# lawfuyang/ToyRenderer

Hardware: AMD Instinct MI355X
Metric: Gmeshlets/s culled (whole node), 100M meshlets (higher is better)
Workload: dtype f32

## Files before the change

### toyrenderer_amd/csrc/k_basepass_as.hip

```cpp
#include <algorithm>
#include <cstdlib>
#include <string>
#include <type_traits>

#if defined(TR_STAMPS) || defined(TR_COUNT_SLOW) || defined(TR_COUNT_PATHS)
__device__ unsigned long long g_stampSums[8];
#define g_pathCount (g_stampSums + 4)
#endif
#include <atomic>
#include <memory>
#include <mutex>
#include <unordered_map>

#include "cull_math.hip.h"
#include "instance_cache.hip.h"
#include "meshlet_exact.hip.h"
#include "trhip_internal.h"

using namespace interop;

namespace
{

constexpr uint32_t kBlock = 256;
constexpr uint32_t kWaves = kBlock / 64;
constexpr uint32_t kBatch = 64;
constexpr uint32_t kSteps = kBatch / 2;
#ifndef TR_RING_SLOTS
#define TR_RING_SLOTS 2
#endif
#ifndef TR_CULL_BATCH
#define TR_CULL_BATCH (TR_RING_SLOTS == 3 ? 30 : 32)
#endif
#ifndef TR_WINDOW_MAP
#define TR_WINDOW_MAP 0
#endif
#ifndef TR_EARLY_PREFETCH
#define TR_EARLY_PREFETCH 1
#endif
#ifndef TR_DEFER
#define TR_DEFER 1
#endif
constexpr uint32_t kCullBatch = TR_CULL_BATCH;
constexpr uint32_t kCullSteps = kCullBatch / 2;
constexpr uint32_t kRingSlots = TR_RING_SLOTS;
static_assert(kCullSteps % kRingSlots == 0 && kCullBatch <= 64, "a batch is a whole number of trips round the ring");
#ifndef TR_CULL_WAVES
#define TR_CULL_WAVES 4
#endif
constexpr uint32_t kCullWaves = TR_CULL_WAVES;
constexpr uint32_t kCullBlock = 64 * kCullWaves;
#ifndef TR_SHORT_PASS_ROUNDS
#define TR_SHORT_PASS_ROUNDS 2
#endif
constexpr uint32_t kShortPassRounds = TR_SHORT_PASS_ROUNDS;
constexpr uint32_t kSlotBytes = 1280;
constexpr uint32_t kDefWords = 5;
constexpr uint32_t kDefStage = 64;
#ifndef TR_DEF_PASS_AT
#define TR_DEF_PASS_AT 32
#endif
constexpr uint32_t kDefPassAt = TR_DEF_PASS_AT;
constexpr uint32_t kDefFromRecord = 0xFFFFFFFFu;
static_assert(kDefPassAt <= kDefStage, "deferred list sizes");

struct RecordInfo
{
    float wxy[8];
    float wz[4];
    float adjxy[6];
    float adjz[3];
    float maxScale;
    uint32_t first;
    uint32_t lastOff;
};
__device__ __forceinline__ uint32_t lastOffOf(uint32_t count) { return count ? 16u * count - 8u : 0u; }
__device__ __forceinline__ uint32_t countOf(uint32_t lastOff) { return (lastOff + 8u) >> 4; }
static_assert(sizeof(RecordInfo) == 96, "RecordInfo layout");

__device__ __forceinline__ cm::M43P worldOf(const RecordInfo& ri)
{
    return { { ri.wxy[0], ri.wxy[1] }, { ri.wxy[2], ri.wxy[3] }, { ri.wxy[4], ri.wxy[5] }, { ri.wxy[6], ri.wxy[7] },
             ri.wz[0], ri.wz[1], ri.wz[2], ri.wz[3] };
}
__device__ __forceinline__ cm::M33P adjugateOf(const RecordInfo& ri)
{
    return { { ri.adjxy[0], ri.adjxy[1] }, { ri.adjxy[2], ri.adjxy[3] }, { ri.adjxy[4], ri.adjxy[5] }, ri.adjz[0], ri.adjz[1], ri.adjz[2] };
}

__device__ __forceinline__ uint32_t listGroupCount(const MeshletCullArgs& a)
{
    return a.listGroups ? a.listGroups[0] : groupCount(a);
}

typedef float v4f __attribute__((ext_vector_type(4)));
template <bool AFTER_READS = false>
__device__ __forceinline__ void issueMeshletLoads(char* slotLds , const MeshletCullStream& stream, uint32_t firstIdx, uint32_t lastOff, uint32_t sub16 ,
                                                  v4f readA = v4f{ 0.f, 0.f, 0.f, 0.f }, uint32_t readB = 0u )
{
#ifdef TR_EXP_NOMEM
    firstIdx &= 63u;
#endif
    const uint32_t idx = firstIdx + (min(sub16, lastOff) >> 4);
    const char* pa = reinterpret_cast<const char*>(stream.sphere) + ((uint64_t)idx << 4);
    const char* pb = reinterpret_cast<const char*>(stream.cone) + ((uint64_t)idx << 2);
    const uint32_t ldsOff = (uint32_t)(uintptr_t)(__attribute__((address_space(3))) char*)slotLds;
#ifndef TR_DMA_POLICY_ID
#define TR_DMA_POLICY_ID 1
#endif
#if TR_DMA_POLICY_ID == 0
#define TR_DMA_POLICY ""
#elif TR_DMA_POLICY_ID == 1
#define TR_DMA_POLICY "nt"
#elif TR_DMA_POLICY_ID == 2
#define TR_DMA_POLICY "sc1"
#elif TR_DMA_POLICY_ID == 3
#define TR_DMA_POLICY "sc0 sc1"
#elif TR_DMA_POLICY_ID == 4
#define TR_DMA_POLICY "sc0 sc1 nt"
#elif TR_DMA_POLICY_ID == 5
#define TR_DMA_POLICY "sc0"
#else
#define TR_DMA_POLICY "sc1 nt"
#endif
    if (AFTER_READS)
        asm volatile("s_mov_b32 m0, %2\n\t"
                     "global_load_lds_dwordx4 %0, off " TR_DMA_POLICY "\n\t"
                     "s_add_u32 m0, %2, 0x400\n\t"
                     "global_load_lds_dword %1, off " TR_DMA_POLICY
                     :: "v"(pa), "v"(pb), "s"(ldsOff), "v"(readA), "v"(readB) : "memory", "m0", "scc");
    else
        asm volatile("s_mov_b32 m0, %2\n\t"
                     "global_load_lds_dwordx4 %0, off " TR_DMA_POLICY "\n\t"
                     "s_add_u32 m0, %2, 0x400\n\t"
                     "global_load_lds_dword %1, off " TR_DMA_POLICY
                     :: "v"(pa), "v"(pb), "s"(ldsOff) : "memory", "m0", "scc");
}
#define TR_WAIT_VMCNT(n) asm volatile("s_waitcnt vmcnt(" #n ")" ::: "memory")

#ifdef TR_STAMPS
#define TR_STAMP(i) do { unsigned long long _t = __builtin_amdgcn_s_memtime(); __builtin_amdgcn_s_waitcnt(0xC07F); stampSum[i] += _t - stampLast; stampLast = _t; } while (0)
#else
#define TR_STAMP(i) do {} while (0)
#endif

#ifndef TR_LK_POLICY_ID
#define TR_LK_POLICY_ID 0
#endif
#if TR_LK_POLICY_ID == 0
#define TR_LK_POLICY ""
#elif TR_LK_POLICY_ID == 1
#define TR_LK_POLICY " sc0"
#elif TR_LK_POLICY_ID == 2
#define TR_LK_POLICY " sc1"
#elif TR_LK_POLICY_ID == 3
#define TR_LK_POLICY " sc0 sc1"
#elif TR_LK_POLICY_ID == 4
#define TR_LK_POLICY " nt"
#else
#define TR_LK_POLICY " sc1 nt"
#endif
#ifndef TR_CULL_WAVES_PER_EU
#define TR_CULL_WAVES_PER_EU 5
#endif
template <bool FRUSTUM, bool OCCLUSION, bool CONE, bool TABLE>
__global__ __launch_bounds__(kCullBlock, TR_CULL_WAVES_PER_EU) void meshletCullKernel(MeshletCullArgs a)
{
#ifdef TR_STAMPS
    unsigned long long stampSum[8] = {0, 0, 0, 0, 0, 0, 0, 0};
    unsigned long long stampLast = __builtin_amdgcn_s_memtime();
    __builtin_amdgcn_s_waitcnt(0xC07F);
#endif
    __shared__ RecordInfo s_recAll[kCullWaves][kCullBatch + 2 * kRingSlots];
    __shared__ uint32_t s_gIdxAll[kCullWaves][kCullBatch];
    __shared__ uint32_t s_quadOff[16];
    __shared__ uint4 s_mipTab[17];
    __shared__ float s_coneTab[cm::kConeTabEntries];
    constexpr bool kDeferred = OCCLUSION && TABLE;
    __shared__ uint2 s_mipBand[kDeferred ? 17 : 1];
    __shared__ uint32_t s_defAll[kCullWaves][kDeferred ? kDefStage * kDefWords : 1u];
    __shared__ __attribute__((aligned(8))) uint32_t s_maskAll[kCullWaves][kCullBatch + 2];
    __shared__ __attribute__((aligned(16))) char s_ring[kCullWaves][kRingSlots][kSlotBytes];

    const uint32_t G = groupCount(a);
    const uint32_t tid = threadIdx.x, lane = tid & 63u, wave = tid >> 6;
    const uint32_t half = lane >> 5, sub = lane & 31u;
    if (a.listGroups && blockIdx.x == 0 && tid == 0) a.listGroups[0] = G;
    const cm::M43 V = cm::loadM43(a.k.m_WorldToView);
    const cm::M43P VP = cm::packM43(V);
    const cm::M33P VR = cm::rot(VP);
    const float coneSlack = cm::coneSlackFactor(V);
    if (!TABLE && G <= gridDim.x * (2u * kCullWaves) * a.shortPassRounds) {
        for (uint32_t g = (blockIdx.x * kCullWaves + wave) * 2u + half; g < G; g += gridDim.x * kCullWaves * 2u) {
            const bool vis = exactMeshletVisible<FRUSTUM, OCCLUSION, CONE>(a, VP, VR, g, sub);
            const unsigned long long b = __ballot(vis);
            if (sub == 0) a.visMask[g] = (uint32_t)(half ? b >> 32 : b);
        }
        return;
    }
    RecordInfo* s_rec = s_recAll[wave];
    uint32_t* s_gIdx = s_gIdxAll[wave];

    if (tid < 16) s_quadOff[tid] = a.hzb.mipOffset[tid];
    if (TABLE && tid >= 1 && tid <= 16) {
        const uint32_t mip = tid - 1u < a.hzb.mips ? tid - 1u : 0u;
        const uint32_t mw = (a.hzb.width >> mip) ? (a.hzb.width >> mip) : 1u, mh = (a.hzb.height >> mip) ? (a.hzb.height >> mip) : 1u;
        s_mipTab[tid] = make_uint4(a.quad.offset[mip], ((mw >> 3) + 1u) * 64u, __float_as_uint(0.5f * (float)mw), __float_as_uint(0.5f * (float)mh));
    }
    if (kDeferred && tid >= 1 && tid <= 16) { const uint32_t d = cm::projMipDelta(a.bands, tid); s_mipBand[tid] = make_uint2(d, 2u * d); }
    const bool nearInRange = a.k.m_NearPlane >= 0x1p-20f && a.k.m_NearPlane <= 0x1p20f;
    if (CONE) for (uint32_t i = tid; i < cm::kConeTabEntries; i += kCullBlock) s_coneTab[i] = cm::coneTableEntry(i);
    if (lane < 2 * kRingSlots) { s_recAll[wave][kCullBatch + lane].first = 0; s_recAll[wave][kCullBatch + lane].lastOff = 0; }
    uint32_t* s_def = s_defAll[wave];
    uint32_t* s_mask = s_maskAll[wave];
    __syncthreads();

    const bool usePerm = a.permHeader != nullptr && a.permHeader[0] == 1u && a.permHeader[1] == G;
#ifndef TR_TEAM_ALL
    const uint32_t teamWaves = kCullWaves, waveInTeam = wave, team = blockIdx.x, teams = gridDim.x;
#else
    const uint32_t teamWaves = gridDim.x * kCullWaves, waveInTeam = blockIdx.x * kCullWaves + wave, team = 0u, teams = 1u;
#endif
    const uint32_t superSize = teamWaves * kCullBatch;
    const uint32_t numSuper = (G + superSize - 1) / superSize;
    auto loadEntry = [&](uint32_t sb_) -> uint4 {
#ifdef TR_BLOCKED_MAP
        const uint64_t e64 = (uint64_t)sb_ * superSize + waveInTeam * kCullBatch + lane;
#else
        const uint64_t e64 = (uint64_t)sb_ * superSize + (lane >> 1) * 2 * teamWaves + 2 * waveInTeam + (lane & 1);
#endif
        if (lane >= kCullBatch || sb_ >= numSuper || e64 >= G) return make_uint4(0xFFFFFFFFu, 0u, 0u, 0u);
        const uint32_t e = (uint32_t)e64;
        if (usePerm) return a.perm[e];
        const MeshletAmplificationData rec = a.records[e];
        return make_uint4(e, rec.m_InstanceConstIdx, rec.m_MeshLOD, rec.m_MeshletGroupOffset);
    };
#ifndef TR_NO_SPLIT_TAIL
    const uint32_t fullRounds = numSuper / teams, left = numSuper - fullRounds * teams;
    uint32_t piecesPer = 1u, stepsPer = kCullSteps;
    if (left) {
        const uint32_t k = std::min(teams / left, kCullSteps / kRingSlots);
        if (k > 1u) {
            stepsPer = ((kCullSteps + k - 1u) / k + kRingSlots - 1u) / kRingSlots * kRingSlots;
            piecesPer = (kCullSteps + stepsPer - 1u) / stepsPer;
        }
    }
#else
    const uint32_t fullRounds = (numSuper + teams - 1u) / teams, left = 0u, piecesPer = 1u, stepsPer = kCullSteps;
#endif
    auto windowOf = [&](uint32_t it, uint32_t& s0, uint32_t& s1) -> uint32_t {
        s0 = 0u; s1 = kCullSteps;
        if (it < fullRounds) {
            uint64_t w = (uint64_t)it * teams + team;
#if TR_WINDOW_MAP
            constexpr uint32_t kCo = TR_CULL_WAVES_PER_EU;
            if (teams % kCo == 0u) {
                const uint32_t perRow = teams / kCo, c = team % perRow, j = team / perRow;
                w = TR_WINDOW_MAP == 2 ? ((uint64_t)c * fullRounds + it) * kCo + j : (uint64_t)it * teams + (uint64_t)c * kCo + j;
            }
#endif
            return w < numSuper ? (uint32_t)w : 0xFFFFFFFFu;
        }
        if (it == fullRounds && left && team < left * piecesPer) {
            s0 = (team % piecesPer) * stepsPer;
            s1 = std::min(s0 + stepsPer, kCullSteps);
            return fullRounds * teams + team / piecesPer;
// ... 276 lines not shown
            TR_STAMP(6);
        };
        if (!primed) {
#pragma unroll
            for (uint32_t k = 0; k + 1 < kRingSlots; ++k)
                issueMeshletLoads(ring + kSlotBytes * k, a.stream, s_rec[2 * (s0 + k) + half].first, s_rec[2 * (s0 + k) + half].lastOff, sub16);
            if (kDefer) {
                const void* p = TABLE ? (const void*)a.quad.base : (const void*)a.hzb.base;
                issueLookup(lk0[kRingSlots - 1u], lk1[kRingSlots - 1u], p, p, 0ull);
            }
            issueMeshletLoads(ring + kSlotBytes * (kRingSlots - 1u), a.stream, s_rec[2 * (s0 + kRingSlots - 1u) + half].first, s_rec[2 * (s0 + kRingSlots - 1u) + half].lastOff, sub16);
        }
#pragma unroll 1
        for (uint32_t s = s0; s < nSteps; s += kRingSlots) {
            step(std::integral_constant<uint32_t, 0>{}, s);
            step(std::integral_constant<uint32_t, 1>{}, s + 1);
            if (kRingSlots == 3) step(std::integral_constant<uint32_t, 2>{}, s + 2);
        }
        if (kDefer) {
            if (kEarly) asm volatile("s_waitcnt vmcnt(0)" : "+v"(lk0[kRingSlots - 1u]), "+v"(lk1[kRingSlots - 1u]) :: "memory");
            else asm volatile("s_waitcnt vmcnt(2)" : "+v"(lk0[kRingSlots - 1u]), "+v"(lk1[kRingSlots - 1u]) :: "memory");
            resolve(2u * nSteps, pVis, pAccept, pPair, pDepth, lk0[kRingSlots - 1u], lk1[kRingSlots - 1u]);
        }
        if (!kPipe) TR_WAIT_VMCNT(0);
        __builtin_amdgcn_fence(__ATOMIC_ACQ_REL, "wavefront");
        __builtin_amdgcn_wave_barrier();
        if (kDeferred && __builtin_expect(batchExact, 0)) {
            for (uint32_t s = s0; s < nSteps; ++s) {
                const uint32_t r = 2 * s + half;
                const uint32_t g = s_gIdx[r];
                const unsigned long long ballot = __ballot(g < G && exactMeshlet(g, sub));
                if (sub == 0) s_mask[r + 2u] = half ? (uint32_t)(ballot >> 32) : (uint32_t)ballot;
            }
            stCount = stAtBatch;
            batchExact = false;
#ifdef TR_COUNT_PATHS
            if (lane == 0) atomicAdd(&g_stampSums[2], 1ull);
#endif
            asm volatile("s_waitcnt vmcnt(0)" ::: "memory");
            __builtin_amdgcn_fence(__ATOMIC_ACQ_REL, "wavefront");
            __builtin_amdgcn_wave_barrier();
        }
        if (kDeferred && __builtin_expect(stAtBatch >= kDefPassAt, 0)) {
            const uint32_t n = stAtBatch < 64u ? stAtBatch : 64u;
            runPass(n);
            stAtBatch -= n;
        }
        {
            const uint32_t g = lane < kCullBatch ? s_gIdx[lane] : 0xFFFFFFFFu;
            if (g < G) a.visMask[g] = s_mask[(lane < kCullBatch ? lane : 0u) + 2u];
        }
        primed = false;
        const uint32_t nStepsN = stepsOf(sbN, s0N, s1N);
        if (nStepsN) {
            const float4* wr = blockAddr(entry);
            q0 = wr[0]; q1 = wr[1]; q2 = wr[2]; q3 = wr[3];
            if (kPipe && usePerm) {
                const bool has = entry.x < G && (lane >> 1) >= s0N && (lane >> 1) < nStepsN;
                uint32_t cnt = entry.w < 32u ? entry.w : 32u;
                if (!has || (uint64_t)entry.z + cnt > a.numMeshlets) cnt = 0u;
                const uint32_t pf = cnt ? entry.z : 0u, pl = lastOffOf(cnt);
#pragma unroll
                for (uint32_t k = 0; k < kRingSlots; ++k) {
                    const int from = (int)((2u * (s0N + k) + half) * 4u);
                    const uint32_t f = (uint32_t)__builtin_amdgcn_ds_bpermute(from, (int)pf), l = (uint32_t)__builtin_amdgcn_ds_bpermute(from, (int)pl);
                    issueMeshletLoads(ring + kSlotBytes * k, a.stream, f, l, sub16);
                }
                primed = true;
            }
        } else if (kPipe) {
            TR_WAIT_VMCNT(0);
        }
    }
    if (kDeferred && stCount) {
        asm volatile("s_waitcnt vmcnt(0)" ::: "memory");
        while (stCount) runPass(stCount < 64u ? stCount : 64u);
    }
#ifdef TR_STAMPS
    if (lane == 0)
        for (int i = 0; i < 8; ++i) atomicAdd(&g_stampSums[i], stampSum[i]);
#endif
}

__device__ __forceinline__ uint32_t waveSum(uint32_t v)
{
    v += (uint32_t)__builtin_amdgcn_update_dpp(0, (int)v, 0x111, 0xf, 0xf, true);
    v += (uint32_t)__builtin_amdgcn_update_dpp(0, (int)v, 0x112, 0xf, 0xf, true);
    v += (uint32_t)__builtin_amdgcn_update_dpp(0, (int)v, 0x114, 0xf, 0xf, true);
    v += (uint32_t)__builtin_amdgcn_update_dpp(0, (int)v, 0x118, 0xf, 0xf, true);
    v += (uint32_t)__builtin_amdgcn_update_dpp(0, (int)v, 0x142, 0xa, 0xf, false);
    v += (uint32_t)__builtin_amdgcn_update_dpp(0, (int)v, 0x143, 0xc, 0xf, false);
    return (uint32_t)__builtin_amdgcn_readlane((int)v, 63);
}

#ifndef TR_SUPER_SHIFT
#define TR_SUPER_SHIFT 8
#endif
constexpr uint32_t kSuperShift = TR_SUPER_SHIFT;
constexpr uint32_t kSuperBatches = 1u << kSuperShift;
constexpr uint32_t kCountThreads = 1024;
constexpr uint32_t kCountWaves = kCountThreads / 64;
__global__ __launch_bounds__(kCountThreads) void visCountKernel(MeshletCullArgs a)
{
    __shared__ uint32_t s_part[kCountWaves];
    const uint32_t G = listGroupCount(a);
    const uint32_t numBatches = (G + kBatch - 1) / kBatch;
    const uint32_t numSupers = (numBatches + kSuperBatches - 1) >> kSuperShift;
    const uint32_t lane = threadIdx.x & 63u, wave = threadIdx.x >> 6;
    constexpr uint32_t kPerWave = kSuperBatches / kCountWaves;
    for (uint32_t sb = blockIdx.x; sb < numSupers; sb += gridDim.x) {
        const uint32_t b0 = (sb << kSuperShift) + wave * kPerWave;
        uint32_t pc[kPerWave];
#pragma unroll
        for (uint32_t i = 0; i < kPerWave; ++i) {
            const uint32_t g = (b0 + i) * kBatch + lane;
            pc[i] = g < G ? (uint32_t)__popc(a.visMask[g]) : 0u;
        }
        uint32_t mine = 0;
#pragma unroll
        for (uint32_t i = 0; i < kPerWave; ++i) {
            pc[i] = waveSum(pc[i]);
            if (lane == 0 && b0 + i < numBatches) a.batchSum[b0 + i] = pc[i];
            mine += pc[i];
        }
        __syncthreads();
        if (lane == 0) s_part[wave] = mine;
        __syncthreads();
        if (threadIdx.x == 0) {
            uint32_t total = 0;
#pragma unroll
            for (uint32_t w = 0; w < kCountWaves; ++w) total += s_part[w];
            a.superSum[sb] = total;
        }
    }
}

__device__ __forceinline__ uint32_t waveInclusiveScan(uint32_t v, uint32_t lane)
{
#pragma unroll
    for (int d = 1; d < 64; d <<= 1) {
        uint32_t n = __shfl_up(v, d);
        if (lane >= (uint32_t)d) v += n;
    }
    return v;
}

__global__ __launch_bounds__(1024) void visSuperScanKernel(MeshletCullArgs a)
{
    __shared__ uint32_t s_wave[16];
    const uint32_t G = listGroupCount(a);
    const uint32_t numBatches = (G + kBatch - 1) / kBatch;
    const uint32_t numSupers = (numBatches + kSuperBatches - 1) >> kSuperShift;
    const uint32_t tid = threadIdx.x, lane = tid & 63u, wave = tid >> 6;
    uint32_t carry = 0;
    for (uint32_t base = 0; base < numSupers; base += 1024u) {
        const uint32_t i = base + tid;
        const uint32_t v = i < numSupers ? a.superSum[i] : 0u;
        const uint32_t inc = waveInclusiveScan(v, lane);
        __syncthreads();
        if (lane == 63) s_wave[wave] = inc;
        __syncthreads();
        uint32_t pre = 0, all = 0;
#pragma unroll
        for (uint32_t w = 0; w < 16; ++w) { if (w < wave) pre += s_wave[w]; all += s_wave[w]; }
        if (i < numSupers) a.superSum[i] = carry + pre + inc - v;
        carry += all;
    }
    if (tid == 0) { a.drawArgs[0] = carry; a.drawArgs[1] = 1; a.drawArgs[2] = 1; }
}

__global__ __launch_bounds__(kBlock) void visExpandKernel(MeshletCullArgs a)
{
    __shared__ uint2 s_mo[kWaves][kBatch];
    const uint32_t G = listGroupCount(a);
    const uint32_t numBatches = (G + kBatch - 1) / kBatch;
    const uint32_t lane = threadIdx.x & 63u, wave = threadIdx.x >> 6;
    const uint32_t half = lane >> 5, sub = lane & 31u;
    const uint32_t bit = 1u << sub, below = bit - 1u;
    uint2* mo = s_mo[wave];
    for (uint32_t batch = blockIdx.x * kWaves + wave; batch < numBatches; batch += gridDim.x * kWaves) {
        const uint32_t g0 = batch * kBatch;
        const uint32_t mask = g0 + lane < G ? a.visMask[g0 + lane] : 0u;
        const uint32_t sb = batch >> kSuperShift;
        uint32_t before = 0;
        for (uint32_t j = (sb << kSuperShift) + lane; j < batch; j += 64u) before += a.batchSum[j];
        before = waveSum(before) + a.superSum[sb];
        const uint32_t pc = (uint32_t)__popc(mask);
        const uint32_t exc = waveInclusiveScan(pc, lane) - pc + before;
        mo[lane] = make_uint2(mask, exc);
        __builtin_amdgcn_fence(__ATOMIC_RELEASE, "wavefront");
        __builtin_amdgcn_wave_barrier();
        __builtin_amdgcn_fence(__ATOMIC_ACQUIRE, "wavefront");
        uint32_t value = ((g0 + half) << 5) | sub;
#pragma unroll 8
        for (uint32_t s = 0; s < kSteps; ++s) {
            const uint2 e = mo[2 * s + half];
            if (e.x & bit) {
                const uint32_t pos = e.y + (uint32_t)__popc(e.x & below);
                if (pos < a.listCapacity) a.visibleList[pos] = value;
            }
            value += 2u << 5;
        }
        __builtin_amdgcn_fence(__ATOMIC_RELEASE, "wavefront");
        __builtin_amdgcn_wave_barrier();
        __builtin_amdgcn_fence(__ATOMIC_ACQUIRE, "wavefront");
    }
}

constexpr uint32_t kCompactTile = 2048;
constexpr uint32_t kCompactThreads = 1024;
constexpr uint32_t kCompactWaves = kCompactThreads / 64;
constexpr uint32_t kCompactMaxTiles = (1u << 19) / kCompactTile;
constexpr uint32_t kStatusStride = 16;
constexpr uint64_t kFlagA = 1ull << 62, kFlagMask = 3ull << 62, kPoison = 1ull << 48;

__global__ __launch_bounds__(kCompactThreads) void visCompactKernel(MeshletCullArgs a, unsigned long long* status, uint32_t* ticket)
{
    __shared__ uint32_t s_mask[kCompactTile];
    __shared__ uint32_t s_off[kCompactTile];
    __shared__ uint32_t s_waveTot[kCompactWaves];
    __shared__ uint32_t s_tile;
    __shared__ unsigned long long s_pre[kCompactMaxTiles / 64u];
    const uint32_t G = listGroupCount(a);
    const uint32_t numTiles = (G + kCompactTile - 1) / kCompactTile;
    const uint32_t tid = threadIdx.x, lane = tid & 63u, wave = tid >> 6;
    for (;;) {
        if (tid == 0) s_tile = atomicAdd(ticket, 1u);
        __syncthreads();
        const uint32_t tile = s_tile;
        if (tile >= numTiles) {
            if (tile == 0 && tid == 0) { a.drawArgs[0] = 0; a.drawArgs[1] = 1; a.drawArgs[2] = 1; }
            return;
        }
        const uint32_t g0 = tile * kCompactTile;
        const uint32_t b = g0 + tid * 2u;
        uint32_t m0 = 0, m1 = 0;
        if (b + 2u <= G) { const uint2 v = *reinterpret_cast<const uint2*>(a.visMask + b); m0 = v.x; m1 = v.y; }
        else if (b < G) m0 = a.visMask[b];
        const uint32_t c0 = (uint32_t)__popc(m0), mine = c0 + (uint32_t)__popc(m1);
        const uint32_t inc = waveInclusiveScan(mine, lane);
        if (lane == 63) s_waveTot[wave] = inc;
        __syncthreads();
        uint32_t pre = 0, total = 0;
#pragma unroll
        for (uint32_t w = 0; w < kCompactWaves; ++w) { const uint32_t x = s_waveTot[w]; if (w < wave) pre += x; total += x; }
        const uint32_t exc = pre + inc - mine;
        *reinterpret_cast<uint2*>(&s_mask[tid * 2u]) = make_uint2(m0, m1);
        *reinterpret_cast<uint2*>(&s_off[tid * 2u]) = make_uint2(exc, exc + c0);
        if (tid == 0) __hip_atomic_store(&status[tile * kStatusStride], kFlagA | (unsigned long long)total, __ATOMIC_RELAXED, __HIP_MEMORY_SCOPE_AGENT);
        if (wave < kCompactMaxTiles / 64u) {
            unsigned long long v = 0;
            if (tid < tile) {
                uint32_t spins = 0;
                for (;;) {
                    v = __hip_atomic_load(&status[tid * kStatusStride], __ATOMIC_RELAXED, __HIP_MEMORY_SCOPE_AGENT);
                    if (v & kFlagMask) { v &= ~kFlagMask; break; }
                    if (++spins > (1u << 22)) { v = kPoison; break; }
                    __builtin_amdgcn_s_sleep(1);
                }
            }
#pragma unroll
            for (int d = 32; d >= 1; d >>= 1) v += __shfl_xor(v, d);
            if (lane == 0) s_pre[wave] = v;
        }
        __syncthreads();
        unsigned long long base = 0;
#pragma unroll
        for (uint32_t w = 0; w < kCompactMaxTiles / 64u; ++w) base += s_pre[w];
        if (tid == 0 && tile == numTiles - 1) {
            const unsigned long long all = base + total;
            const bool bad = (all >> 40) != 0ull;
            a.drawArgs[0] = bad ? 0xFFFFFFFFu : (uint32_t)all;
            a.drawArgs[1] = bad ? 0xFFFFFFFFu : 1u;
            a.drawArgs[2] = bad ? 0xFFFFFFFFu : 1u;
        }
        const uint32_t groupsHere = G - g0 < kCompactTile ? G - g0 : kCompactTile;
#pragma unroll 4
        for (uint32_t slot = tid; slot < groupsHere * 32u; slot += kCompactThreads) {
            const uint32_t g = slot >> 5, sub = slot & 31u;
            const uint32_t mask = s_mask[g];
            if (mask & (1u << sub)) {
                const unsigned long long pos = base + s_off[g] + (uint32_t)__popc(mask & ((1u << sub) - 1u));
                if (pos < a.listCapacity) a.visibleList[pos] = ((g0 + g) << 5) | sub;
            }
        }
        __syncthreads();
    }
}

// ... 212 lines not shown
                if (inSlot > a.slotGroups || inSlot < sentG || runEnd < runBegin || runEnd > a.slotRuns) bad = true;
                if (bad) { status |= 4u; g = 0; runEnd = runBegin; }
                if (a.globalCap && a.records[s] && !bad) {
                    const unsigned long long x = a.recv[(uint64_t)p * slotWords + 2u * s + 1u];
                    if (cutDone[s]) g = 0;
                    else if (counted[s] + x >= a.globalCap) {
                        cutDone[s] = true;
                        const unsigned long long j = a.globalCap - counted[s] - 1ull;
                        if (j < g) {
                            const uint32_t* run = a.recv + (uint64_t)p * slotWords + kSlotHeaderWords + 4ull * runBegin;
                            uint32_t lo = 0, hi = runEnd - runBegin;
                            while (hi - lo > 1u) {
                                const uint32_t mid = (lo + hi) >> 1;
                                if (run[4ull * mid + 3u] <= j) lo = mid; else hi = mid;
                            }
                            g = hi > lo ? run[4ull * lo + 3u] : 0u;
                        }
                    }
                    counted[s] += x;
                }
                uint32_t runs = a.records[s] ? runEnd - runBegin : 0u;
                if (off[s] + g > a.capacity[s]) { g = a.capacity[s] - off[s]; status |= 2u; }
                const uint32_t base = p * slotWords + kSlotHeaderWords;
                s_maskStart[k] = maskRun; s_runStart[k] = runRun;
                s_maskSrc[k] = base + 4u * a.slotRuns + srcG; s_runSrc[k] = base + 4u * runBegin;
                s_dst[k] = off[s]; s_len[k] = g;
                maskRun += g; runRun += runs; ++k;
                off[s] += g;
                runBegin = runEnd;
            }
        }
        s_maskStart[k] = maskRun; s_runStart[k] = runRun;
        if (blockIdx.x == 0)
            for (uint32_t s = 0; s < kMaxPassSlots; ++s)
                if (a.args[s]) {
                    const unsigned long long X = a.globalCap ? counted[s] : off[s];
                    a.args[s][0] = X > 0xFFFFFFFFull ? 0xFFFFFFFFu : (uint32_t)X; a.args[s][1] = 1; a.args[s][2] = 1; a.args[s][3] = off[s];
                    a.args[s][7] = status;
                }
    }
    __syncthreads();
    const uint32_t numSeg = kMaxPassSlots * a.world;
    const uint32_t totalMasks = s_maskStart[numSeg];
    for (uint32_t i = blockIdx.x * 256u + tid; i < totalMasks; i += gridDim.x * 256u) {
        uint32_t lo = 0, hi = numSeg;
        while (hi - lo > 1u) {
            const uint32_t mid = (lo + hi) >> 1;
            if (s_maskStart[mid] <= i) lo = mid; else hi = mid;
        }
        a.masks[lo % kMaxPassSlots][s_dst[lo] + (i - s_maskStart[lo])] = a.recv[(uint64_t)s_maskSrc[lo] + (i - s_maskStart[lo])];
    }
    const uint32_t totalRuns = s_runStart[numSeg];
    for (uint32_t it = blockIdx.x * 256u + (tid & ~63u); it < totalRuns; it += gridDim.x * 256u) {
        const uint32_t i = it + lane;
        uint32_t id = 0, lod = 0, off0 = 0, first = 0, cnt = 0;
        uint32_t* dst = nullptr;
        if (i < totalRuns) {
            uint32_t lo = 0, hi = numSeg;
            while (hi - lo > 1u) {
                const uint32_t mid = (lo + hi) >> 1;
                if (s_runStart[mid] <= i) lo = mid; else hi = mid;
            }
            const uint32_t e = i - s_runStart[lo], runs = s_runStart[lo + 1] - s_runStart[lo], len = s_len[lo];
            const uint4 entry = *reinterpret_cast<const uint4*>(a.recv + (uint64_t)s_runSrc[lo] + 4ull * e);
            uint32_t next = e + 1u < runs ? a.recv[(uint64_t)s_runSrc[lo] + 4ull * (e + 1u) + 3u] : 0xFFFFFFFFu;
            next = next < len ? next : len;
            id = entry.x; lod = entry.y; off0 = entry.z; first = entry.w;
            cnt = first < next ? next - first : 0u;
            dst = a.records[lo % kMaxPassSlots] + 3ull * (s_dst[lo] + first);
        }
        if (cnt <= 8u)
            for (uint32_t j = 0; j < cnt; ++j) { dst[3u * j] = id; dst[3u * j + 1u] = lod; dst[3u * j + 2u] = off0 + 32u * j; }
        unsigned long long big = __ballot(cnt > 8u);
        while (big) {
            const int l = __builtin_ctzll(big);
            big &= big - 1ull;
            const uint32_t bid = __shfl(id, l), blod = __shfl(lod, l), boff = __shfl(off0, l), bcnt = __shfl(cnt, l);
            uint32_t* bdst = (uint32_t*)(((unsigned long long)__shfl((uint32_t)((unsigned long long)dst >> 32), l) << 32) | __shfl((uint32_t)(unsigned long long)dst, l));
            for (uint32_t j = lane; j < bcnt; j += 64u) { bdst[3u * j] = bid; bdst[3u * j + 1u] = blod; bdst[3u * j + 2u] = boff + 32u * j; }
        }
    }
}

void emitListBuild(const trhip::DispatchCtx& ctx, const MeshletCullArgs& a, const char* prefix, bool side, const void* argsBase)
{
    auto emit = [&](const std::string& name, std::function<int(hipStream_t)> fn) {
        if (side) ctx.emitSide(name.c_str(), std::move(fn), { { a.listGroups ? (const void*)a.listGroups : argsBase, false }, { a.visMask, false }, { a.visibleList, true }, { a.drawArgs, true } });
        else ctx.emit(name.c_str(), std::move(fn));
    };
    if (!side && a.recordCapacity <= kCompactMaxTiles * kCompactTile) {
        const uint32_t tiles = (a.recordCapacity + kCompactTile - 1) / kCompactTile;
        const size_t words = (size_t)kCompactMaxTiles * kStatusStride * 2 + 4;
        uint32_t* mem = (uint32_t*)ctx.scratch(words * 4);
        if (mem && ctx.cl->recordClearWords(mem, words, 0, true) == TRHIP_OK) {
            unsigned long long* status = (unsigned long long*)mem;
            uint32_t* ticket = mem + kCompactMaxTiles * kStatusStride * 2;
            uint32_t grid = ctx.computeUnits();
            if (grid > tiles) grid = tiles;
            if (grid == 0) grid = 1;
            emit(std::string(prefix) + "compact", [a, status, ticket, grid](hipStream_t s) {
                TRHIP_LAUNCH(visCompactKernel, dim3(grid), dim3(kCompactThreads), 0, s, a, status, ticket);
                return trhip::launchStatus("visCompactKernel"); });
            return;
        }
    }
    const uint32_t needBlocks = (a.maxBatches + kWaves - 1) / kWaves;
    uint32_t gridSmall = ctx.computeUnits() * 8u;
    if (gridSmall > needBlocks) gridSmall = needBlocks;
    if (gridSmall == 0) gridSmall = 1;
    const std::string p = prefix;
    const uint32_t supers = (a.maxBatches >> kSuperShift) + 1u;
    emit(p + "count", [a, supers](hipStream_t s) {
        TRHIP_LAUNCH(visCountKernel, dim3(supers), dim3(kCountThreads), 0, s, a);
        return trhip::launchStatus("visCountKernel"); });
    emit(p + "scan", [a](hipStream_t s) {
        TRHIP_LAUNCH(visSuperScanKernel, dim3(1), dim3(1024), 0, s, a);
        return trhip::launchStatus("visSuperScanKernel"); });
    emit(p + "expand", [a, gridSmall](hipStream_t s) {
        TRHIP_LAUNCH(visExpandKernel, dim3(gridSmall), dim3(kBlock), 0, s, a);
        return trhip::launchStatus("visExpandKernel"); });
}

template <bool F, bool O, bool C>
void launchCull(const MeshletCullArgs& a, uint32_t grid, bool table, hipStream_t s)
{
    if (O && table) TRHIP_LAUNCH((meshletCullKernel<F, O, C, true>), dim3(grid), dim3(kCullBlock), 0, s, a);
    else TRHIP_LAUNCH((meshletCullKernel<F, O, C, false>), dim3(grid), dim3(kCullBlock), 0, s, a);
}

constexpr uint64_t kStreamBytesPerMeshlet = 20;
__host__ __device__ inline MeshletCullStream meshletStreamLayout(void* mem, uint64_t numMeshlets)
{
    const uint64_t coneAt = (numMeshlets * 16u + 255u) & ~255ull;
    return { reinterpret_cast<const float4*>(mem), reinterpret_cast<const uint32_t*>(reinterpret_cast<char*>(mem) + coneAt) };
}
inline uint64_t meshletStreamBytes(uint64_t numMeshlets) { return ((numMeshlets * 16u + 255u) & ~255ull) + numMeshlets * 4u; }

__global__ __launch_bounds__(256) void meshletStreamKernel(const MeshletData* __restrict__ meshlets, uint64_t n, MeshletCullStream out)
{
    const uint64_t stride = (uint64_t)gridDim.x * 256u;
    for (uint64_t i = (uint64_t)blockIdx.x * 256u + threadIdx.x; i < n; i += stride) {
        const float4* p = reinterpret_cast<const float4*>(meshlets + i);
        const float4 sphere = p[0];
        const uint32_t cone = __float_as_uint(p[1].x);
        const_cast<float4*>(out.sphere)[i] = sphere;
        const_cast<uint32_t*>(out.cone)[i] = cone;
    }
}

int meshletStreamLaunchBuild(trhip_buffer_t* meshlets, hipStream_t s)
{
    const trhip::Stamp from = { meshlets->version };
    if (meshlets->cullStream.current(from)) return TRHIP_OK;
    const uint64_t n = meshlets->byteSize / sizeof(MeshletData);
    const uint64_t blocks = (n + 255u) / 256u;
    TRHIP_LAUNCH(meshletStreamKernel, dim3((uint32_t)(blocks < 65536u ? (blocks ? blocks : 1u) : 65536u)), dim3(256), 0, s,
                       (const MeshletData*)meshlets->ptr, n, meshletStreamLayout(meshlets->cullStream.ptr, n));
    meshlets->cullStream.markBuilt(from);
    return trhip::launchStatus("meshletStreamKernel");
}

int recordASMain(trhip::DispatchCtx& ctx)
{
    const BasePassConstants* k = (const BasePassConstants*)ctx.constants(0, sizeof(BasePassConstants));
    TRHIP_REQUIRE(k, "%s: constant buffer b0 (BasePassConstants, 256 bytes) missing", ctx.shaderName);
    trhip_buffer_t* instances = ctx.buffer(TRHIP_BIND_STRUCTURED_SRV, 0);
    trhip_buffer_t* meshData = ctx.buffer(TRHIP_BIND_STRUCTURED_SRV, 2);
    trhip_buffer_t* meshlets = ctx.buffer(TRHIP_BIND_STRUCTURED_SRV, 4);
    trhip_buffer_t* records = ctx.buffer(TRHIP_BIND_STRUCTURED_SRV, 7);
    trhip_texture_t* hzb = ctx.texture(TRHIP_BIND_TEXTURE_SRV, 8);
    trhip_buffer_t* visMask = ctx.buffer(TRHIP_BIND_STRUCTURED_UAV, 0);
    trhip_buffer_t* visList = ctx.buffer(TRHIP_BIND_STRUCTURED_UAV, 1);
    trhip_buffer_t* drawArgs = ctx.buffer(TRHIP_BIND_STRUCTURED_UAV, 2);
    TRHIP_REQUIRE(instances && meshData && meshlets && records, "%s: needs SRVs t0, t2, t4, t7 (BasePassRenderers.cpp:463-479)", ctx.shaderName);
    TRHIP_REQUIRE(visMask && visList && drawArgs, "%s: needs UAVs u0 (visMask), u1 (visibleList), u2 (drawArgs)", ctx.shaderName);
    TRHIP_REQUIRE(ctx.indirect, "%s: launched by dispatchMeshIndirect (BasePassRenderers.cpp:497-502): use dispatch_indirect", ctx.shaderName);
    TRHIP_REQUIRE(instances->byteSize % sizeof(BasePassInstanceConstants) == 0, "%s: instance buffer size is not a multiple of 144", ctx.shaderName);
    TRHIP_REQUIRE(meshlets->byteSize % sizeof(MeshletData) == 0, "%s: meshlet buffer size is not a multiple of 32", ctx.shaderName);
    TRHIP_REQUIRE(drawArgs->byteSize >= 12, "%s: drawArgs buffer smaller than 12 bytes", ctx.shaderName);

    MeshletCullArgs a;
    memset(&a, 0, sizeof a);
    a.k = *k;
    const bool occlusion = (k->m_CullingFlags & kCullingFlagOcclusionCullingEnable) != 0;
    const bool useTable = occlusion && ctx.variant == 0 && records->byteSize / sizeof(MeshletAmplificationData) >= trhip::tableMinGroups();
    int rc = TRHIP_OK;
    {
        memset(&a.hzb, 0, sizeof a.hzb);
        if (occlusion) {
            TRHIP_REQUIRE(hzb, "%s: occlusion culling enabled but no HZB texture bound at t8", ctx.shaderName);
            TRHIP_REQUIRE(hzb->format == TRHIP_FORMAT_R16_FLOAT, "%s: HZB is not R16_FLOAT", ctx.shaderName);
            TRHIP_REQUIRE(hzb->width == k->m_HZBDimensions.x && hzb->height == k->m_HZBDimensions.y,
                          "%s: m_HZBDimensions %ux%u does not match the HZB texture %ux%u", ctx.shaderName,
                          k->m_HZBDimensions.x, k->m_HZBDimensions.y, hzb->width, hzb->height);
            a.hzb.base = (const _Float16*)hzb->ptr;
            a.hzb.width = hzb->width; a.hzb.height = hzb->height; a.hzb.mips = hzb->mips;
            for (uint32_t m = 0; m < hzb->mips; ++m) a.hzb.mipOffset[m] = (uint32_t)(hzb->mipOffset[m] / 2);
            if (useTable) {
                rc = trhip::hzbQuadEnsure(hzb);
                if (rc != TRHIP_OK) return rc;
                a.quad.base = (const _Float16*)hzb->quad.ptr;
                a.quad.total = hzb->quadTotal;
                for (uint32_t m = 0; m < hzb->mips; ++m) a.quad.offset[m] = hzb->quadOffset[m];
            }
        }
    }
    if (rc != TRHIP_OK) return rc;
    a.meshlets = (const MeshletData*)meshlets->ptr;
    TRHIP_REQUIRE(meshlets->byteSize >= sizeof(MeshletData), "%s: empty meshlet buffer", ctx.shaderName);
    rc = meshlets->cullStream.allocate(meshlets->dev, meshletStreamBytes(meshlets->byteSize / sizeof(MeshletData)));
    if (rc != TRHIP_OK) return rc;
    a.stream = meshletStreamLayout(meshlets->cullStream.ptr, meshlets->byteSize / sizeof(MeshletData));
    a.records = (const MeshletAmplificationData*)records->ptr;
    a.dispatchArgs = (const uint32_t*)((const char*)ctx.argsBuffer->ptr + ctx.argsOffset);
    a.argsWords = (ctx.argsBuffer->byteSize - ctx.argsOffset) >= 16 ? 4u : 3u;
    const uint64_t cap = records->byteSize / sizeof(MeshletAmplificationData);
    a.recordCapacity = cap > 0xFFFFFFFFull ? 0xFFFFFFFFu : (uint32_t)cap;
    TRHIP_REQUIRE(a.recordCapacity <= (1u << 27), "%s: more than 2^27 records cannot be encoded as (g<<5)|lane", ctx.shaderName);
    TRHIP_REQUIRE(visMask->byteSize / 4 >= a.recordCapacity, "%s: visMask holds %llu groups, records buffer %u", ctx.shaderName,
                  (unsigned long long)(visMask->byteSize / 4), a.recordCapacity);
    a.numMeshlets = meshlets->byteSize / sizeof(MeshletData);
    TRHIP_REQUIRE(a.numMeshlets <= (1ull << 32), "%s: more than 2^32 meshlets (m_MeshletDataBufferIdx is 32 bits wide)", ctx.shaderName);
    a.visMask = (uint32_t*)visMask->ptr;
    a.visibleList = (uint32_t*)visList->ptr;
    const uint64_t lcap = visList->byteSize / 4;
    a.listCapacity = lcap > 0xFFFFFFFFull ? 0xFFFFFFFFu : (uint32_t)lcap;
    a.drawArgs = (uint32_t*)drawArgs->ptr;
    if (records->order.ptr && records->order.bytes >= 256 + (uint64_t)a.recordCapacity * 16) {
        a.permHeader = (const uint32_t*)records->order.ptr;
        a.perm = (const uint4*)(a.permHeader + 64);
    }
    rc = trhip::instanceCacheEnsure(instances);
    if (rc != TRHIP_OK) return rc;
    a.numInstances = (uint32_t)(instances->byteSize / sizeof(BasePassInstanceConstants));
    a.cache = instanceCacheLayout(instances->cullCache.ptr, a.numInstances);
    a.maxBatches = (a.recordCapacity + kBatch - 1) / kBatch;
    a.batchSum = (uint32_t*)(a.recordCapacity >= (1u << 19) ? ctx.scratchSide((size_t)a.maxBatches * 4)
                                                            : ctx.scratch((size_t)a.maxBatches * 4));
    TRHIP_REQUIRE(a.batchSum, "%s: scratch allocation failed", ctx.shaderName);
    {
        const size_t supers = (a.maxBatches >> kSuperShift) + 1u;
        a.superSum = (uint32_t*)(a.recordCapacity >= (1u << 19) ? ctx.scratchSide(supers * 4) : ctx.scratch(supers * 4));
        TRHIP_REQUIRE(a.superSum, "%s: scratch allocation failed", ctx.shaderName);
    }

    const uint32_t blocksPerCU = TR_CULL_WAVES_PER_EU;
    uint32_t grid = ctx.computeUnits() * blocksPerCU;
    const uint32_t needBlocks = (a.recordCapacity + kCullBatch * kCullWaves - 1) / (kCullBatch * kCullWaves);
    if (grid > needBlocks) grid = needBlocks;
    if (grid == 0) grid = 1;
    rc = visMask->listCount.allocate(visMask->dev, 256);
    if (rc != TRHIP_OK) return rc;
    a.listGroups = (uint32_t*)visMask->listCount.ptr;
    ctx.cl->use(a.listGroups, ctx.cl->ops.size(), true);
    if (useTable) a.bands = cm::projBands(k->m_P00, k->m_P11, hzb->width, hzb->height);
    static const bool noShortPass = getenv("TRHIP_NO_SHORT_PASS") != nullptr;
    a.shortPassRounds = noShortPass ? 0u : kShortPassRounds;
    const uint32_t flags = k->m_CullingFlags & 7u;
    trhip_texture_t* quadOwner = useTable ? hzb : nullptr;
    const bool table = useTable;
    if (quadOwner) ctx.cl->use(quadOwner->quad.ptr, ctx.cl->ops.size(), false);
    ctx.emit("cull", [a, grid, flags, quadOwner, table, instances, meshData, meshlets](hipStream_t s) {
        if ((const void*)a.meshlets != meshlets->ptr)
            return trhip::fail(TRHIP_ERR_STATE, "basepass_AS_Main: the meshlet buffer was bound to other memory after this command list was recorded: record it again");
        {
            int crc = trhip::instanceCacheLaunchBuild(instances, meshData, s);
            if (crc != TRHIP_OK) return crc;
            crc = meshletStreamLaunchBuild(meshlets, s);
            if (crc != TRHIP_OK) return crc;
        }
        if (quadOwner) {
            int brc = trhip::hzbQuadLaunchBuild(quadOwner, s);
            if (brc != TRHIP_OK) return brc;
        }
        switch (flags) {
        case 0: launchCull<false, false, false>(a, grid, table, s); break;
        case 1: launchCull<true, false, false>(a, grid, table, s); break;
        case 2: launchCull<false, true, false>(a, grid, table, s); break;
        case 3: launchCull<true, true, false>(a, grid, table, s); break;
        case 4: launchCull<false, false, true>(a, grid, table, s); break;
        case 5: launchCull<true, false, true>(a, grid, table, s); break;
        case 6: launchCull<false, true, true>(a, grid, table, s); break;
        default: launchCull<true, true, true>(a, grid, table, s); break;
        }
        return trhip::launchStatus("meshletCullKernel"); });
    emitListBuild(ctx, a, "", a.recordCapacity >= (1u << 19), ctx.argsBuffer->ptr);
    if (ctx.cl->openStats)
        return trhip::statsEmitAS(ctx, a, meshlets, records, instances, meshData, a.recordCapacity >= (1u << 19));
    return TRHIP_OK;
}

int recordPackShard(trhip::DispatchCtx& ctx)
{
    const uint32_t* push = (const uint32_t*)ctx.constants(0, 8);
    trhip_buffer_t* slot = ctx.buffer(TRHIP_BIND_STRUCTURED_UAV, 0);
    trhip_buffer_t* state = ctx.buffer(TRHIP_BIND_STRUCTURED_UAV, 1);
    TRHIP_REQUIRE(push && slot && state, "%s: needs push constants {slotGroups, slotRuns}, UAV u0 (shard slot) and UAV u1 (state words, zeroed once)", ctx.shaderName);
    ShardPackArgs a;
    memset(&a, 0, sizeof a);
    a.slotGroups = push[0];
    a.slotRuns = push[1];
    const uint64_t slotWords = (uint64_t)kSlotHeaderWords + 4ull * a.slotRuns + a.slotGroups;
    TRHIP_REQUIRE(slot->byteSize >= slotWords * 4, "%s: shard slot buffer smaller than 16 + 4 * %u + %u words", ctx.shaderName, a.slotRuns, a.slotGroups);
    const uint64_t maxTiles = (uint64_t)a.slotGroups / kPackTile + kMaxPassSlots + 1u;
    TRHIP_REQUIRE(maxTiles < (1u << 30) && state->byteSize >= maxTiles * 16u, "%s: state buffer u1 smaller than %llu bytes", ctx.shaderName, (unsigned long long)(maxTiles * 16u));
    TRHIP_REQUIRE(((uintptr_t)slot->ptr & 15u) == 0 && ((uintptr_t)state->ptr & 7u) == 0, "%s: u0 / u1 not 16 / 8-byte aligned", ctx.shaderName);
    a.slot = (uint32_t*)slot->ptr;
    a.maxTiles = (uint32_t)maxTiles;
    unsigned long long* halves = (unsigned long long*)state->ptr;
    for (uint32_t s = 0; s < kMaxPassSlots; ++s) {
        trhip_buffer_t* rec = ctx.buffer(TRHIP_BIND_STRUCTURED_SRV, 4 * s);
        trhip_buffer_t* mask = ctx.buffer(TRHIP_BIND_STRUCTURED_SRV, 4 * s + 1);
        trhip_buffer_t* args = ctx.buffer(TRHIP_BIND_STRUCTURED_SRV, 4 * s + 2);
        trhip_buffer_t* draw = ctx.buffer(TRHIP_BIND_STRUCTURED_SRV, 4 * s + 3);
        if (!rec && !mask && !args && !draw) continue;
        TRHIP_REQUIRE(rec && mask && args && draw, "%s: pass slot %u needs t%u..t%u (records, visMask, dispatch args, draw args)", ctx.shaderName, s, 4 * s, 4 * s + 3);
        TRHIP_REQUIRE(args->byteSize >= 12 && draw->byteSize >= 12, "%s: argument buffers smaller than 12 bytes", ctx.shaderName);
        const uint64_t cap = std::min<uint64_t>(rec->byteSize / sizeof(MeshletAmplificationData), mask->byteSize / 4);
        a.records[s] = (const uint32_t*)rec->ptr;
        a.masks[s] = (const uint32_t*)mask->ptr;
        a.dispatchArgs[s] = (const uint32_t*)args->ptr;
        a.drawArgs[s] = (const uint32_t*)draw->ptr;
        a.argsWords[s] = args->byteSize >= 16 ? 4u : 3u;
        a.recordCapacity[s] = cap > 0xFFFFFFFFull ? 0xFFFFFFFFu : (uint32_t)cap;
    }
    a.tileBlocks = (uint32_t)std::min<uint64_t>(maxTiles, (uint64_t)ctx.computeUnits() * 3u);
    const uint32_t maskBlocks = (uint32_t)std::min<uint64_t>(std::max<uint64_t>(((uint64_t)a.slotGroups + 4u * kPackThreads - 1u) / (4u * kPackThreads), 1u), ctx.computeUnits());
    const uint32_t grid = a.tileBlocks + maskBlocks;
    static std::mutex mu;
    static std::unordered_map<void*, std::shared_ptr<std::atomic<uint32_t>>> launches;
    std::shared_ptr<std::atomic<uint32_t>> count;
    {
        std::lock_guard<std::mutex> lock(mu);
        std::shared_ptr<std::atomic<uint32_t>>& c = launches[(void*)halves];
        if (!c) c = std::make_shared<std::atomic<uint32_t>>(0u);
        count = c;
    }
    ctx.emit("main", [a, grid, halves, count](hipStream_t s) {
        ShardPackArgs l = a;
        const uint32_t half = count->fetch_add(1u) & 1u;
        l.status = halves + (size_t)half * a.maxTiles;
        l.statusNext = halves + (size_t)(half ^ 1u) * a.maxTiles;
        TRHIP_LAUNCH(shardPackKernel, dim3(grid), dim3(kPackThreads), 0, s, l);
        return trhip::launchStatus("shardPackKernel"); });
    return TRHIP_OK;
}

int recordUnpackShards(trhip::DispatchCtx& ctx)
{
    const uint32_t* push = (const uint32_t*)ctx.constants(0, 12);
    trhip_buffer_t* recv = ctx.buffer(TRHIP_BIND_STRUCTURED_SRV, 0);
    TRHIP_REQUIRE(push && recv, "%s: needs push constants {world, slotGroups, slotRuns[, globalGroupCapacity]} and SRV t0 (gathered slots)", ctx.shaderName);
    ShardUnpackArgs a;
    memset(&a, 0, sizeof a);
    a.world = push[0];
    a.slotGroups = push[1];
    a.slotRuns = push[2];
    if (const uint32_t* push4 = (const uint32_t*)ctx.constants(0, 16)) a.globalCap = push4[3];
    TRHIP_REQUIRE(a.world >= 1 && a.world <= kMaxRanks, "%s: world size %u outside [1, %u]", ctx.shaderName, a.world, kMaxRanks);
    const uint64_t words = (uint64_t)a.world * (kSlotHeaderWords + 4ull * a.slotRuns + a.slotGroups);
    TRHIP_REQUIRE(words < (1ull << 32), "%s: %u slots of %u groups / %u runs exceed 2^32 words", ctx.shaderName, a.world, a.slotGroups, a.slotRuns);
    TRHIP_REQUIRE(recv->byteSize >= words * 4, "%s: gathered buffer smaller than world x slot", ctx.shaderName);
    TRHIP_REQUIRE(((uintptr_t)recv->ptr & 15u) == 0, "%s: t0 not 16-byte aligned", ctx.shaderName);
    a.recv = (const uint32_t*)recv->ptr;
    MeshletCullArgs lists[kMaxPassSlots];
    uint64_t copyWords = 0;
    for (uint32_t s = 0; s < kMaxPassSlots; ++s) {
        trhip_buffer_t* rec = ctx.buffer(TRHIP_BIND_STRUCTURED_UAV, 4 * s);
        trhip_buffer_t* mask = ctx.buffer(TRHIP_BIND_STRUCTURED_UAV, 4 * s + 1);
// ... 64 lines not shown
```

### toyrenderer_amd/csrc/k_gpuculling.hip

```cpp
#include "cull_math.hip.h"
#include "hzb_quad.hip.h"
#include "instance_cache.hip.h"
#include "trhip_internal.h"

using namespace interop;

namespace
{

constexpr uint32_t kBlock = 256;
constexpr uint32_t kWordSubmit = 1u << 30;
constexpr uint32_t kWordLate = 1u << 31;
constexpr uint32_t kGroupMask = (1u << 27) - 1u;

struct InstanceCullArgs
{
    GPUCullingPassConstants k;
    const BasePassInstanceConstants* instances;
    const uint32_t* ids;
    const MeshData* meshData;
    cm::Hzb hzb;
    MeshletAmplificationData* records;
    uint32_t* dispatchArgs;
    uint32_t* lateCount;
    uint32_t* lateIds;
    const uint32_t* indirectArgs;
    InstanceCullCache cache;
    uint32_t numInstances;
    const uint32_t* shardLate;
    uint32_t directThreads;
    uint32_t maxGroups;
    uint32_t argsWords;
    uint32_t* word;
    uint32_t* localOff;
    uint32_t* blockGroups;
    uint64_t* blockLateSubmit;
    uint32_t* bases;
    uint32_t numBlocks;
    uint32_t* tileHist;
    uint32_t* tileTotal;
    uint16_t* tileOf;
    uint2* lodSel;
    uint32_t* permHeader;
    uint4* perm;
    uint32_t permCapacity;
    uint32_t* lateArgsOut;
    unsigned long long* fusedStatus;
    uint32_t* fusedTicket;
};

struct QuadShare { bool stale = false; };
struct EarlyCullNote { InstanceCullArgs a; size_t scanOp; bool fused; trhip_texture_t* quadOwner = nullptr; std::shared_ptr<QuadShare> share; };

__global__ __launch_bounds__(256) void instanceCacheKernel(const BasePassInstanceConstants* instances, uint32_t n,
                                                           const MeshData* meshData, uint32_t numMeshes, InstanceCullCache c)
{
    const uint32_t i = blockIdx.x * 256u + threadIdx.x;
    if (i >= n) return;
    const BasePassInstanceConstants& inst = instances[i];
    const float4 w0 = *reinterpret_cast<const float4*>(inst.m_WorldMatrix.m[0]);
    const float4 w1 = *reinterpret_cast<const float4*>(inst.m_WorldMatrix.m[1]);
    const float4 w2 = *reinterpret_cast<const float4*>(inst.m_WorldMatrix.m[2]);
    const float4 w3 = *reinterpret_cast<const float4*>(inst.m_WorldMatrix.m[3]);
    const uint32_t meshIdx = inst.m_MeshDataIdx;
    float4 sph = make_float4(0.f, 0.f, 0.f, 0.f);
    uint32_t numLODs = 0;
    uint32_t nm[kMaxNumMeshLODs], mb[kMaxNumMeshLODs];
    float err[kMaxNumMeshLODs];
#pragma unroll
    for (uint32_t l = 0; l < kMaxNumMeshLODs; ++l) { nm[l] = 0; mb[l] = 0; err[l] = 0.f; }
    if (meshIdx < numMeshes) {
        const MeshData& mesh = meshData[meshIdx];
        sph = *reinterpret_cast<const float4*>(&mesh.m_BoundingSphere);
        numLODs = mesh.m_NumLODs;
#pragma unroll
        for (uint32_t l = 0; l < kMaxNumMeshLODs; ++l) {
            nm[l] = mesh.m_MeshLODDatas[l].m_NumMeshlets; mb[l] = mesh.m_MeshLODDatas[l].m_MeshletDataBufferIdx; err[l] = mesh.m_MeshLODDatas[l].m_Error;
        }
    }
    instanceCacheWriteTransformPart(c, i, w0, w1, w2, w3, sph);
    const_cast<float4*>(c.localSphere)[i] = sph;
    const_cast<uint32_t*>(c.numLODs)[i] = numLODs;
#pragma unroll
    for (uint32_t l = 0; l < kMaxNumMeshLODs; ++l) {
        const_cast<uint2&>(c.lod(i, l)) = make_uint2(nm[l], mb[l]);
// ... 308 lines not shown
    const uint32_t tid = threadIdx.x, lane = tid & 63u, wave = tid >> 6;
    const bool binned = n >= kMinBinnedEntries;
    if (binned) {
        uint32_t carry = 0;
        for (uint32_t base = 0; base < kNumTiles; base += kBigThreads) {
            const bool inRange = base + tid < kNumTiles;
            const uint32_t tot = inRange ? a.tileTotal[base + tid] : 0u;
            const uint32_t inc = waveInclusiveScan(tot, lane);
            if (lane == 63) s_wave[wave] = inc;
            __syncthreads();
            uint32_t pre = 0, all = 0;
            for (uint32_t w = 0; w < kBigWaves; ++w) { if (w < wave) pre += s_wave[w]; all += s_wave[w]; }
            if (inRange) s_cursor[base + tid] = carry + pre + inc - tot + a.tileHist[(uint64_t)blockIdx.x * kNumTiles + base + tid];
            carry += all;
            __syncthreads();
        }
    }
    const uint32_t baseG = a.bases[0] + a.blockGroups[blockIdx.x];
    const uint32_t baseL = a.bases[1] + (uint32_t)a.blockLateSubmit[blockIdx.x];
    for (uint32_t e = 0; e < kBigPerThread; ++e) {
        const uint32_t t = blockIdx.x * kBigChunk + e * kBigThreads + tid;
        const uint32_t word = t < n ? a.word[t] : 0u;
        if (word & kWordLate) a.lateIds[baseL + a.localOff[t]] = a.ids[t];
        const bool submit = (word & kWordSubmit) != 0 && !(word & kWordLate);
        const uint32_t groups = word & kGroupMask;
        const uint32_t lod = (word >> 27) & 7u;
        const uint32_t off = submit ? baseG + a.localOff[t] : 0u;
        const bool dropped = submit && off + groups >= a.maxGroups;
        if (dropped && groups != 0 && off < a.maxGroups && a.argsWords > 3) a.dispatchArgs[3] = off;
        const bool emitRec = submit && !dropped;
        const uint32_t id = emitRec ? a.ids[t] : 0u;
        if (emitRec) {
            struct __attribute__((packed, aligned(4))) Quad { uint32_t x, y, z, w; };
            uint32_t* dst = reinterpret_cast<uint32_t*>(a.records + off);
            uint32_t i = 0;
            for (; i + 4u <= groups; i += 4u) {
                const uint32_t o = i * kNumThreadsPerWave;
                *reinterpret_cast<Quad*>(dst + 3u * i) = Quad{ id, lod, o, id };
                *reinterpret_cast<Quad*>(dst + 3u * i + 4u) = Quad{ lod, o + kNumThreadsPerWave, id, lod };
                *reinterpret_cast<Quad*>(dst + 3u * i + 8u) = Quad{ o + 2u * kNumThreadsPerWave, id, lod, o + 3u * kNumThreadsPerWave };
            }
            for (; i < groups; ++i) {
                MeshletAmplificationData rec = { id, lod, i * kNumThreadsPerWave };
                a.records[off + i] = rec;
            }
        }
        const bool place = emitRec && groups != 0 && binned;
        uint32_t p = 0, numMeshlets = 0, mbase = 0;
        if (place) {
            p = atomicAdd(&s_cursor[a.tileOf[t]], groups);
            const uint2 li = a.lodSel[t];
            numMeshlets = li.x; mbase = li.y;
        }
        const uint32_t head = place ? (groups < 4u ? groups : 4u) : 0u;
        const uint32_t j = lane & 3u;
#pragma unroll
        for (uint32_t it = 0; it < 4; ++it) {
            const int src = (int)(it * 16u + (lane >> 2));
            const uint32_t sp = __shfl(p, src), soff = __shfl(off, src), sid = __shfl(id, src);
            const uint32_t sbase = __shfl(mbase, src), snm = __shfl(numMeshlets, src), shead = __shfl(head, src);
            if (j < shead) {
                const uint32_t first = j * kNumThreadsPerWave;
                const uint32_t cnt = snm > first ? (snm - first < kNumThreadsPerWave ? snm - first : kNumThreadsPerWave) : 0u;
                if (sp + j < a.permCapacity) a.perm[sp + j] = make_uint4(soff + j, sid, sbase + first, cnt);
            }
        }
        if (place)
            for (uint32_t i = 4; i < groups; ++i) {
                const uint32_t first = i * kNumThreadsPerWave;
                const uint32_t cnt = numMeshlets > first ? (numMeshlets - first < kNumThreadsPerWave ? numMeshlets - first : kNumThreadsPerWave) : 0u;
                if (p + i < a.permCapacity) a.perm[p + i] = make_uint4(off + i, id, mbase + first, cnt);
            }
    }
}


constexpr uint32_t kFusedMaxEntries = 1u << 17;
constexpr uint32_t kFusedMaxTiles = kFusedMaxEntries / kBlock;
constexpr uint32_t kFusedLateMaxTiles = 4096;
constexpr uint32_t kFusedStatusStride = 16;
constexpr unsigned long long kFusedFlag = 1ull << 63, kFusedPoison = 1ull << 60;

template <int LATE>
__global__ __launch_bounds__(kBlock) void instanceFusedKernel(InstanceCullArgs a, trhip::QuadArgs q)
{
    if (!LATE && blockIdx.x >= a.numBlocks) {
        __shared__ float s_t[9][trhip::kQuadStripCols + 1];
        trhip::hzbQuadStrip(q, blockIdx.x - a.numBlocks, s_t);
        return;
    }
    __shared__ uint32_t s_waveG[kBlock / 64], s_waveL[kBlock / 64], s_waveS[kBlock / 64];
    __shared__ unsigned long long s_preG[kBlock / 64], s_preLS[kBlock / 64];
    __shared__ uint32_t s_tile;
    const uint32_t n = threadCount<LATE>(a);
    const uint32_t numTiles = (n + kBlock - 1) / kBlock < a.numBlocks ? (n + kBlock - 1) / kBlock : a.numBlocks;
    const uint32_t tid = threadIdx.x, lane = tid & 63u, wave = tid >> 6;
    const uint32_t baseX = __hip_atomic_load(&a.dispatchArgs[0], __ATOMIC_RELAXED, __HIP_MEMORY_SCOPE_AGENT);
    const uint32_t baseLate = LATE ? 0u : __hip_atomic_load(a.lateCount, __ATOMIC_RELAXED, __HIP_MEMORY_SCOPE_AGENT);
    if (blockIdx.x >= (numTiles ? numTiles : 1u)) return;
    {
        if (tid == 0) s_tile = atomicAdd(a.fusedTicket, 1u);
        __syncthreads();
        const uint32_t tile = s_tile;
        const uint32_t t = tile * kBlock + tid;
        uint32_t word = 0, tileUnused = 0;
        uint2 lodUnused;
        if (t < n) word = classify<LATE>(a, a.ids[t], &tileUnused, &lodUnused);
        const uint32_t g = (word & kWordSubmit) ? (word & kGroupMask) : 0u;
        const uint32_t late = word >> 31;
        const uint32_t submit = (word >> 30) & 1u;
        const uint32_t incG = waveInclusiveScan(g, lane);
        const uint32_t incL = waveInclusiveScan(late, lane);
        const uint32_t cntS = (uint32_t)__popcll(__ballot(submit != 0));
        if (lane == 63) { s_waveG[wave] = incG; s_waveL[wave] = incL; s_waveS[wave] = cntS; }
        __syncthreads();
        uint32_t baseG = 0, baseL = 0, totG = 0, totL = 0, totS = 0;
#pragma unroll
        for (uint32_t w = 0; w < kBlock / 64; ++w) {
            if (w < wave) { baseG += s_waveG[w]; baseL += s_waveL[w]; }
            totG += s_waveG[w]; totL += s_waveL[w]; totS += s_waveS[w];
        }
        const uint32_t localOff = late ? (baseL + incL - late) : (baseG + incG - g);
        unsigned long long* line = a.fusedStatus + (uint64_t)tile * kFusedStatusStride;
        if (tid == 0 && numTiles != 0) {
            __hip_atomic_store(&line[0], kFusedFlag | (unsigned long long)totG, __ATOMIC_RELAXED, __HIP_MEMORY_SCOPE_AGENT);
            __hip_atomic_store(&line[1], kFusedFlag | ((unsigned long long)totS << 32) | (unsigned long long)totL, __ATOMIC_RELAXED, __HIP_MEMORY_SCOPE_AGENT);
        }
        unsigned long long sumG = 0, sumLS = 0;
        for (uint32_t j = tid; j < tile; j += kBlock) {
            const unsigned long long* pl = a.fusedStatus + (uint64_t)j * kFusedStatusStride;
            unsigned long long v0 = 0, v1 = 0;
            uint32_t spins = 0;
            for (;;) {
                v0 = __hip_atomic_load(&pl[0], __ATOMIC_RELAXED, __HIP_MEMORY_SCOPE_AGENT);
                v1 = __hip_atomic_load(&pl[1], __ATOMIC_RELAXED, __HIP_MEMORY_SCOPE_AGENT);
                if ((v0 & v1 & kFusedFlag) != 0ull) { v0 &= ~kFusedFlag; v1 &= ~kFusedFlag; break; }
                if (++spins > (1u << 22)) { v0 = kFusedPoison; v1 = 0; break; }
                __builtin_amdgcn_s_sleep(1);
            }
            sumG += v0; sumLS += v1;
        }
#pragma unroll
        for (int d = 32; d >= 1; d >>= 1) { sumG += __shfl_xor(sumG, d); sumLS += __shfl_xor(sumLS, d); }
        if (lane == 0) { s_preG[wave] = sumG; s_preLS[wave] = sumLS; }
        __syncthreads();
        unsigned long long preG = 0, preLS = 0;
#pragma unroll
        for (uint32_t w = 0; w < kBlock / 64; ++w) { preG += s_preG[w]; preLS += s_preLS[w]; }
        const uint32_t prefixG = (uint32_t)preG, prefixL = (uint32_t)preLS;
        if (t < n) {
            if (word & kWordLate) {
                a.lateIds[baseLate + prefixL + localOff] = a.ids[t];
            } else if (word & kWordSubmit) {
                const uint32_t groups = word & kGroupMask;
                const uint32_t lod = (word >> 27) & 7u;
                const uint32_t off = baseX + prefixG + localOff;
                if (off + groups >= a.maxGroups) {
                    if (groups != 0 && off < a.maxGroups && a.argsWords > 3) a.dispatchArgs[3] = off;
                } else {
                    const uint32_t id = a.ids[t];
                    for (uint32_t i = 0; i < groups; ++i) {
                        MeshletAmplificationData rec = { id, lod, i * kNumThreadsPerWave };
                        a.records[off + i] = rec;
                    }
                }
            }
        }
        if (tid == 0 && (tile == numTiles - 1u || numTiles == 0)) {
            const unsigned long long allG = preG + totG;
            const uint32_t allL = prefixL + totL, allS = (uint32_t)(preLS >> 32) + totS;
            const uint32_t X = (allG >> 40) ? 0xFFFFFFFFu : baseX + (uint32_t)allG;
            a.bases[0] = baseX;
            a.bases[1] = baseLate;
            a.dispatchArgs[0] = X;
            if (allS != 0) { a.dispatchArgs[1] = 1; a.dispatchArgs[2] = 1; }
            if (a.argsWords > 3 && (X < a.maxGroups || baseX >= a.maxGroups)) a.dispatchArgs[3] = X;
            if (!LATE) {
                const uint32_t lateTotal = baseLate + allL;
                *a.lateCount = lateTotal;
                if (a.lateArgsOut) { a.lateArgsOut[0] = (lateTotal + 63u) / 64u; a.lateArgsOut[1] = 1; a.lateArgsOut[2] = 1; }
            }
            a.permHeader[0] = 0u;
            a.permHeader[1] = X;
        }
    }
}

__global__ void buildLateCullIndirectArgsKernel(const uint32_t* count, uint32_t* args)
{
    args[0] = (count[0] + 63u) / 64u;
    args[1] = 1;
    args[2] = 1;
}

__global__ void shardLateInfoKernel(const uint32_t* counts, uint32_t world, uint32_t rank, uint32_t* info)
{
    uint32_t below = 0, all = 0;
    for (uint32_t p = 0; p < world; ++p) {
        const uint32_t c = counts[p];
        if (p < rank) below += c;
        all += c;
    }
    info[0] = below;
    info[1] = all;
}

int fillHzb(const trhip::DispatchCtx& ctx, trhip_texture_t* tex, const Vector2U& dims, bool occlusion, cm::Hzb* out)
{
    memset(out, 0, sizeof *out);
    if (!occlusion) return TRHIP_OK;
    TRHIP_REQUIRE(tex, "%s: occlusion culling enabled but no HZB texture bound", ctx.shaderName);
    TRHIP_REQUIRE(tex->format == TRHIP_FORMAT_R16_FLOAT, "%s: HZB '%s' is not R16_FLOAT", ctx.shaderName, tex->name.c_str());
    TRHIP_REQUIRE(tex->width == dims.x && tex->height == dims.y,
                  "%s: m_HZBDimensions %ux%u does not match HZB texture %ux%u", ctx.shaderName, dims.x, dims.y, tex->width, tex->height);
    out->base = (const _Float16*)tex->ptr;
    out->width = tex->width; out->height = tex->height; out->mips = tex->mips;
    for (uint32_t k = 0; k < tex->mips; ++k) out->mipOffset[k] = (uint32_t)(tex->mipOffset[k] / 2);
    return TRHIP_OK;
}

std::function<int(hipStream_t)> fusedEarlyLaunch(const InstanceCullArgs& a, trhip_texture_t* quadOwner)
{
    return [a, quadOwner](hipStream_t s) {
        trhip::QuadArgs q;
        memset(&q, 0, sizeof q);
        uint32_t strips = 0;
        if (quadOwner && !quadOwner->quad.current({ quadOwner->version })) {
            q = trhip::quadArgs(quadOwner);
            strips = q.firstStrip[q.mips];
            quadOwner->quad.markBuilt({ quadOwner->version });
        }
        TRHIP_LAUNCH(instanceFusedKernel<0>, dim3(a.numBlocks + strips), dim3(kBlock), 0, s, a, q);
        return trhip::launchStatus("instanceFusedKernel"); };
}

inline uint32_t quadScanStrips(uint32_t all)
{
    static const uint32_t pct = [] { const char* e = getenv("TRHIP_QUAD_SCAN_PERCENT"); const int v = e ? atoi(e) : 50; return (uint32_t)(v < 0 ? 0 : v > 100 ? 100 : v); }();
    return (uint32_t)((uint64_t)all * pct / 100u);
}

std::function<int(hipStream_t)> scanEarlyLaunch(const InstanceCullArgs& a, trhip_texture_t* quadOwner, std::shared_ptr<QuadShare> share)
{
    return [a, quadOwner, share](hipStream_t s) {
        trhip::QuadArgs q;
        memset(&q, 0, sizeof q);
        uint32_t extra = 0, stripEnd = 0;
        if (share) share->stale = false;
        if (quadOwner && !quadOwner->quad.current({ quadOwner->version })) {
            q = trhip::quadArgs(quadOwner);
            stripEnd = share ? quadScanStrips(q.firstStrip[q.mips]) : q.firstStrip[q.mips];
            extra = (stripEnd + kScanStripsPerGroup - 1u) / kScanStripsPerGroup;
            quadOwner->quad.markBuilt({ quadOwner->version });
            if (share) share->stale = true;
        }
        TRHIP_LAUNCH(instanceScanKernel<0>, dim3(1 + kScanTileGroups + extra), dim3(kScanThreads), 0, s, a, q, stripEnd);
        return trhip::launchStatus("instanceScanKernel"); };
}

template <int LATE>
int recordGPUCulling(trhip::DispatchCtx& ctx)
{
    const GPUCullingPassConstants* k = (const GPUCullingPassConstants*)ctx.constants(0, sizeof(GPUCullingPassConstants));
    TRHIP_REQUIRE(k, "%s: constant buffer b0 (GPUCullingPassConstants, 180 bytes) missing", ctx.shaderName);
    trhip_buffer_t* instances = ctx.buffer(TRHIP_BIND_STRUCTURED_SRV, 0);
    trhip_buffer_t* ids = ctx.buffer(TRHIP_BIND_STRUCTURED_SRV, 1);
    trhip_buffer_t* meshData = ctx.buffer(TRHIP_BIND_STRUCTURED_SRV, 2);
    trhip_texture_t* hzb = ctx.texture(TRHIP_BIND_TEXTURE_SRV, 3);
    trhip_buffer_t* records = ctx.buffer(TRHIP_BIND_STRUCTURED_UAV, 0);
    trhip_buffer_t* args = ctx.buffer(TRHIP_BIND_STRUCTURED_UAV, 1);
    trhip_buffer_t* lateCount = ctx.buffer(TRHIP_BIND_STRUCTURED_UAV, 2);
    trhip_buffer_t* lateIds = ctx.buffer(TRHIP_BIND_STRUCTURED_UAV, 3);
    trhip_buffer_t* shardLate = LATE ? ctx.buffer(TRHIP_BIND_STRUCTURED_SRV, 4) : nullptr;
    TRHIP_REQUIRE(!shardLate || shardLate->byteSize >= 8, "%s: shard late info (t4) smaller than 8 bytes", ctx.shaderName);
    TRHIP_REQUIRE(instances && ids && meshData && records && args && lateCount && lateIds,
                  "%s: needs SRVs t0..t2 and UAVs u0..u3 (BasePassRenderers.cpp:351-362)", ctx.shaderName);
    const bool occlusion = (k->m_CullingFlags & kCullingFlagOcclusionCullingEnable) != 0;
    TRHIP_REQUIRE(instances->byteSize % sizeof(BasePassInstanceConstants) == 0, "%s: instance buffer size is not a multiple of 144", ctx.shaderName);
    TRHIP_REQUIRE(meshData->byteSize % sizeof(MeshData) == 0, "%s: mesh data buffer size is not a multiple of 156", ctx.shaderName);
    TRHIP_REQUIRE(records->byteSize >= sizeof(MeshletAmplificationData), "%s: amplification buffer too small", ctx.shaderName);
    TRHIP_REQUIRE(args->byteSize >= 12, "%s: dispatch-arguments buffer smaller than 12 bytes", ctx.shaderName);
    if (LATE) {
        TRHIP_REQUIRE(ctx.indirect, "%s: LATE_CULL=1 is dispatched indirectly (BasePassRenderers.cpp:399)", ctx.shaderName);
        TRHIP_REQUIRE(occlusion, "%s: LATE_CULL=1 without occlusion culling", ctx.shaderName);
        TRHIP_REQUIRE((uint64_t)k->m_NbInstances * 4 <= lateIds->byteSize, "%s: late id buffer smaller than m_NbInstances", ctx.shaderName);
    } else {
        TRHIP_REQUIRE(!ctx.indirect, "%s: LATE_CULL=0 is dispatched directly", ctx.shaderName);
        TRHIP_REQUIRE((uint64_t)k->m_NbInstances * 4 <= ids->byteSize, "%s: m_NbInstances %u exceeds the id buffer", ctx.shaderName, k->m_NbInstances);
        if (occlusion)
            TRHIP_REQUIRE((uint64_t)k->m_NbInstances * 4 <= lateIds->byteSize, "%s: late id buffer smaller than m_NbInstances", ctx.shaderName);
    }
    TRHIP_REQUIRE(lateCount->byteSize >= 4, "%s: late counter buffer too small", ctx.shaderName);

    InstanceCullArgs a;
    memset(&a, 0, sizeof a);
    a.k = *k;
    int rc = fillHzb(ctx, hzb, k->m_HZBDimensions, occlusion, &a.hzb);
    if (rc != TRHIP_OK) return rc;
    a.instances = (const BasePassInstanceConstants*)instances->ptr;
    a.ids = LATE ? (const uint32_t*)lateIds->ptr : (const uint32_t*)ids->ptr;
    a.meshData = (const MeshData*)meshData->ptr;
    a.records = (MeshletAmplificationData*)records->ptr;
    a.dispatchArgs = (uint32_t*)args->ptr;
    a.lateCount = (uint32_t*)lateCount->ptr;
    a.lateIds = (uint32_t*)lateIds->ptr;
    a.indirectArgs = LATE ? (const uint32_t*)((const char*)ctx.argsBuffer->ptr + ctx.argsOffset) : nullptr;
    a.shardLate = shardLate ? (const uint32_t*)shardLate->ptr : nullptr;
    const uint64_t direct = (uint64_t)ctx.gx * kNumThreadsPerWave;
    a.directThreads = direct > 0xFFFFFFFFull ? 0xFFFFFFFFu : (uint32_t)direct;
    const uint64_t cap = records->byteSize / sizeof(MeshletAmplificationData);
    a.maxGroups = cap > 0xFFFFFFFFull ? 0xFFFFFFFFu : (uint32_t)cap;
    a.argsWords = args->byteSize >= 16 ? 4u : 3u;

    const uint32_t nMax = k->m_NbInstances;
    if (nMax == 0) return TRHIP_OK;

    rc = trhip::instanceCacheEnsure(instances);
    if (rc != TRHIP_OK) return rc;
    a.cache = instanceCacheLayout(instances->cullCache.ptr, instances->byteSize / sizeof(BasePassInstanceConstants));
    a.numInstances = (uint32_t)(instances->byteSize / sizeof(BasePassInstanceConstants));
    ctx.emit("instance_cache", [instances, meshData](hipStream_t s) { return trhip::instanceCacheLaunchBuild(instances, meshData, s); });
    static const bool noFused = getenv("TRHIP_NO_FUSED_INSTANCE") != nullptr;
    const bool fusedPath = (nMax <= kFusedMaxEntries || (LATE && (nMax + kBlock - 1) / kBlock <= kFusedLateMaxTiles)) && !noFused;
    a.numBlocks = fusedPath ? (nMax + kBlock - 1) / kBlock : (nMax + kBigChunk - 1) / kBigChunk;
    a.word = (uint32_t*)ctx.scratch((size_t)nMax * 4);
    a.localOff = (uint32_t*)ctx.scratch((size_t)nMax * 4);
    a.blockGroups = (uint32_t*)ctx.scratch((size_t)a.numBlocks * 4);
    a.blockLateSubmit = (uint64_t*)ctx.scratch((size_t)a.numBlocks * 8);
    a.bases = (uint32_t*)ctx.scratch(16);
    a.tileHist = (uint32_t*)ctx.scratch(fusedPath ? 16 : (size_t)a.numBlocks * kNumTiles * 4);
    a.tileTotal = (uint32_t*)ctx.scratch(kNumTiles * 4);
    a.tileOf = (uint16_t*)ctx.scratch((size_t)nMax * 2);
    a.lodSel = (uint2*)ctx.scratch((size_t)nMax * 8);
    TRHIP_REQUIRE(a.word && a.localOff && a.blockGroups && a.blockLateSubmit && a.bases && a.tileHist && a.tileTotal && a.tileOf && a.lodSel, "%s: scratch allocation failed", ctx.shaderName);
    rc = records->order.allocate(records->dev, (uint64_t)kPermHeaderWords * 4 + (uint64_t)a.maxGroups * 16);
    if (rc != TRHIP_OK) return rc;
    a.permHeader = (uint32_t*)records->order.ptr;
    a.perm = (uint4*)(a.permHeader + kPermHeaderWords);
    a.permCapacity = a.maxGroups;
    const bool wantTable = !LATE && occlusion && a.maxGroups >= trhip::tableMinGroups();
    if (wantTable) {
        rc = trhip::hzbQuadEnsure(hzb);
        if (rc != TRHIP_OK) return rc;
    }

    if (fusedPath) {
        const size_t words = (size_t)a.numBlocks * kFusedStatusStride * 2 + 4;
        uint32_t* mem = (uint32_t*)ctx.scratch(words * 4);
        TRHIP_REQUIRE(mem, "%s: scratch allocation failed", ctx.shaderName);
        rc = ctx.cl->recordClearWords(mem, words, 0, true);
        if (rc != TRHIP_OK) return rc;
        a.fusedStatus = (unsigned long long*)mem;
        a.fusedTicket = mem + (size_t)a.numBlocks * kFusedStatusStride * 2;
        trhip_texture_t* quadOwner = wantTable ? hzb : nullptr;
        if (quadOwner) ctx.cl->use(quadOwner->quad.ptr, ctx.cl->ops.size(), true);
        if (LATE) ctx.emit("fused", [a](hipStream_t s) {
            trhip::QuadArgs q;
            memset(&q, 0, sizeof q);
            TRHIP_LAUNCH(instanceFusedKernel<LATE>, dim3(a.numBlocks), dim3(kBlock), 0, s, a, q);
            return trhip::launchStatus("instanceFusedKernel"); });
        else ctx.emit("fused", fusedEarlyLaunch(a, quadOwner));
        if (!LATE && occlusion) ctx.cl->peephole = { ctx.cl->ops.size() - 1, "gpuculling_early", std::make_shared<EarlyCullNote>(EarlyCullNote{ a, ctx.cl->ops.size() - 1, true, quadOwner }) };
        return TRHIP_OK;
    }

    ctx.emit("classify", [a](hipStream_t s) {
        TRHIP_LAUNCH(instanceClassifyKernel<LATE>, dim3(a.numBlocks), dim3(kBigThreads), 0, s, a);
        return trhip::launchStatus("instanceClassifyKernel"); });
    trhip_texture_t* quadOwner = wantTable ? hzb : nullptr;
    std::shared_ptr<QuadShare> share = quadOwner ? std::make_shared<QuadShare>() : nullptr;
    if (quadOwner) ctx.cl->use(quadOwner->quad.ptr, ctx.cl->ops.size(), true);
    if (LATE) ctx.emit("scan", [a](hipStream_t s) {
        trhip::QuadArgs q;
        memset(&q, 0, sizeof q);
        TRHIP_LAUNCH(instanceScanKernel<LATE>, dim3(1 + kScanTileGroups), dim3(kScanThreads), 0, s, a, q, 0u);
        return trhip::launchStatus("instanceScanKernel"); });
    else ctx.emit("scan", scanEarlyLaunch(a, quadOwner, share));
    const size_t scanOp = ctx.cl->ops.size() - 1;
    if (quadOwner) ctx.cl->use(quadOwner->quad.ptr, ctx.cl->ops.size(), true);
    ctx.emit("emit", [a, quadOwner, share](hipStream_t s) {
        trhip::QuadArgs q;
        memset(&q, 0, sizeof q);
        uint32_t extra = 0, stripBegin = 0;
        if (!LATE && quadOwner && share && share->stale) {
            q = trhip::quadArgs(quadOwner);
            stripBegin = quadScanStrips(q.firstStrip[q.mips]);
            extra = (q.firstStrip[q.mips] - stripBegin + kEmitStripsPerGroup - 1u) / kEmitStripsPerGroup;
        }
        TRHIP_LAUNCH(instanceEmitKernel<LATE>, dim3(a.numBlocks + extra), dim3(kBigThreads), 0, s, a, q, stripBegin);
        return trhip::launchStatus("instanceEmitKernel"); });
    if (!LATE && occlusion) ctx.cl->peephole = { ctx.cl->ops.size() - 1, "gpuculling_early", std::make_shared<EarlyCullNote>(EarlyCullNote{ a, scanOp, false, quadOwner, share }) };
    return TRHIP_OK;
}

int recordBuildLateArgs(trhip::DispatchCtx& ctx)
{
    trhip_buffer_t* count = ctx.buffer(TRHIP_BIND_STRUCTURED_SRV, 0);
    trhip_buffer_t* args = ctx.buffer(TRHIP_BIND_STRUCTURED_UAV, 0);
    TRHIP_REQUIRE(count && args, "%s: needs SRV t0 (late count) and UAV u0 (indirect args)", ctx.shaderName);
    TRHIP_REQUIRE(count->byteSize >= 4 && args->byteSize >= 12, "%s: buffers too small", ctx.shaderName);
    TRHIP_REQUIRE(!ctx.indirect && ctx.gx == 1 && ctx.gy == 1 && ctx.gz == 1, "%s: dispatched as 1x1x1", ctx.shaderName);
    const uint32_t* c = (const uint32_t*)count->ptr;
    uint32_t* a = (uint32_t*)args->ptr;
    const trhip_cmdlist_t::Peephole ph = ctx.cl->peephole;
    if (ph.kind && !strcmp(ph.kind, "gpuculling_early") && ph.op != SIZE_MAX && ph.op == ctx.cl->ops.size() - 1) {
        const EarlyCullNote* note = (const EarlyCullNote*)ph.data.get();
        if (note->a.lateCount == c && note->scanOp < ctx.cl->ops.size() && ctx.cl->ops[note->scanOp].lane == 0) {
            InstanceCullArgs fused = note->a;
            fused.lateArgsOut = a;
            const size_t scanOp = note->scanOp;
            if (note->fused) ctx.cl->ops[scanOp].fn = fusedEarlyLaunch(fused, note->quadOwner);
            else ctx.cl->ops[scanOp].fn = scanEarlyLaunch(fused, note->quadOwner, note->share);
            for (size_t i = ctx.cl->useMarks.size(); i-- > 0 && ctx.cl->useMarks[i].op >= ctx.cl->ops.size();) ctx.cl->useMarks[i].op = scanOp;
            ctx.cl->peephole = trhip_cmdlist_t::Peephole();
            return TRHIP_OK;
        }
    }
    ctx.emit("main", [c, a](hipStream_t s) {
        TRHIP_LAUNCH(buildLateCullIndirectArgsKernel, dim3(1), dim3(1), 0, s, c, a);
        return trhip::launchStatus("buildLateCullIndirectArgsKernel"); });
    return TRHIP_OK;
}

trhip::ShaderRegistrar r0("gpuculling_CS_GPUCulling LATE_CULL=0", recordGPUCulling<0>, 0);
trhip::ShaderRegistrar r1("gpuculling_CS_GPUCulling LATE_CULL=1", recordGPUCulling<1>, 1);
trhip::ShaderRegistrar r2("gpuculling_CS_BuildLateCullIndirectArgs", recordBuildLateArgs, 0);

}

namespace trhip
{

int instanceCacheEnsure(trhip_buffer_t* instances)
{
    const uint64_t n = instances->byteSize / sizeof(BasePassInstanceConstants);
    TRHIP_REQUIRE(n >= 1 && n <= 0xFFFFFFFFull, "instance cull cache: instance buffer '%s' size out of range", instances->name.c_str());
    return instances->cullCache.allocate(instances->dev, n * kInstanceCacheBytesPerInstance);
}

int instanceCacheLaunchBuild(trhip_buffer_t* instances, trhip_buffer_t* meshData, hipStream_t s)
{
    const Stamp from = { instances->version, meshData->ptr, meshData->version };
    if (instances->cullCache.current(from)) return TRHIP_OK;
// ... 19 lines not shown
```

### toyrenderer_amd/csrc/k_hzb.hip

```cpp
#include "cull_math.hip.h"
#include "hzb_quad.hip.h"
#include "trhip_internal.h"

using namespace interop;

namespace
{

template <bool MAX>
__global__ __launch_bounds__(256) void minMaxDownsampleKernel(const float* __restrict__ depth, uint32_t W, uint32_t H,
                                                              _Float16* __restrict__ out, uint32_t ow, uint32_t oh)
{
    const uint32_t x = blockIdx.x * 32 + (threadIdx.x & 31), y = blockIdx.y * 8 + (threadIdx.x >> 5);
    if (x >= ow || y >= oh) return;
    const float u = ((float)x + 0.5f) / (float)ow, v = ((float)y + 0.5f) / (float)oh;
    const float fx = cm::fma_(u, (float)W, -0.5f), fy = cm::fma_(v, (float)H, -0.5f);
    int x0 = (int)__builtin_floorf(fx), y0 = (int)__builtin_floorf(fy);
    int x1 = min(max(x0 + 1, 0), (int)W - 1), y1 = min(max(y0 + 1, 0), (int)H - 1);
    x0 = min(max(x0, 0), (int)W - 1);
    y0 = min(max(y0, 0), (int)H - 1);
    const float a = depth[(uint64_t)y0 * W + x0], b = depth[(uint64_t)y0 * W + x1];
    const float c = depth[(uint64_t)y1 * W + x0], d = depth[(uint64_t)y1 * W + x1];
    const float r = MAX ? cm::max_(cm::max_(a, b), cm::max_(c, d))
                        : cm::min_(cm::min_(a, b), cm::min_(c, d));
    out[(uint64_t)y * ow + x] = (_Float16)r;
}

struct SpdArgs
{
    _Float16* base;
    uint32_t width, height, mips;
    uint32_t mipOffset[16];
};

template <bool MAX>
__device__ __forceinline__ float red4(float a, float b, float c, float d)
{
    return MAX ? cm::max_(cm::max_(a, b), cm::max_(c, d)) : cm::min_(cm::min_(a, b), cm::min_(c, d));
}

template <bool MAX>
__global__ __launch_bounds__(256) void spdTileKernel(SpdArgs a, uint32_t lastMip)
{
    __shared__ float s[2][32 * 32];
    const uint32_t tid = threadIdx.x;
    const uint32_t tx = blockIdx.x, ty = blockIdx.y;
    const _Float16* m0 = a.base + a.mipOffset[0];
    {
        const uint32_t px = (tid & 15) * 2, py = (tid >> 4) * 2;
        for (uint32_t dy = 0; dy < 2; ++dy)
            for (uint32_t dx = 0; dx < 2; ++dx) {
                const uint32_t ox = px + dx, oy = py + dy;
                const uint32_t sx = tx * 64 + ox * 2, sy = ty * 64 + oy * 2;
                const float v = red4<MAX>((float)m0[(uint64_t)sy * a.width + sx], (float)m0[(uint64_t)sy * a.width + sx + 1],
                                          (float)m0[(uint64_t)(sy + 1) * a.width + sx], (float)m0[(uint64_t)(sy + 1) * a.width + sx + 1]);
                s[0][oy * 32 + ox] = v;
                if (lastMip >= 1) {
                    const uint32_t mw = a.width >> 1;
                    a.base[a.mipOffset[1] + (uint64_t)(ty * 32 + oy) * mw + tx * 32 + ox] = (_Float16)v;
                }
            }
    }
    __syncthreads();
    uint32_t cur = 0, dim = 32;
    for (uint32_t mip = 2; mip <= 6 && mip <= lastMip; ++mip) {
        const uint32_t od = dim >> 1;
        if (tid < od * od) {
            const uint32_t ox = tid % od, oy = tid / od;
            const float* p = s[cur];
            const float v = red4<MAX>(p[(2 * oy) * dim + 2 * ox], p[(2 * oy) * dim + 2 * ox + 1],
                                      p[(2 * oy + 1) * dim + 2 * ox], p[(2 * oy + 1) * dim + 2 * ox + 1]);
            s[cur ^ 1][oy * od + ox] = v;
            const uint32_t mw = a.width >> mip;
            a.base[a.mipOffset[mip] + (uint64_t)(ty * od + oy) * mw + tx * od + ox] = (_Float16)v;
        }
        __syncthreads();
        cur ^= 1;
        dim = od;
    }
}

template <bool MAX>
__global__ __launch_bounds__(256) void hzbDepthTileKernel(const float* __restrict__ depth, uint32_t W, uint32_t H, SpdArgs a, uint32_t lastMip)
{
    __shared__ float s0[64 * 64];
    __shared__ float s[2][32 * 32];
    const uint32_t tid = threadIdx.x;
    const uint32_t tx = blockIdx.x, ty = blockIdx.y;
    _Float16* m0 = a.base + a.mipOffset[0];
    const uint32_t ow = a.width, oh = a.height;
    {
        const uint32_t lx = tid & 63u, x = tx * 64 + lx;
        const float u = ((float)x + 0.5f) / (float)ow;
        const float fx = cm::fma_(u, (float)W, -0.5f);
        int x0 = (int)__builtin_floorf(fx);
        const int x1 = min(max(x0 + 1, 0), (int)W - 1);
        x0 = min(max(x0, 0), (int)W - 1);
        const int xl = min(x0, (int)W - 2);
        struct __attribute__((packed, aligned(4))) Pair { float a, b; };
        const bool wide = W >= 2u;
        Pair v0[16], v1[16];
        int rowY0, rowY1;
        {
            const uint32_t ly = (tid & 15u) * 4 + (tid >> 6), y = ty * 64 + ly;
            const float v = ((float)y + 0.5f) / (float)oh;
            const float fy = cm::fma_(v, (float)H, -0.5f);
            const int f0 = (int)__builtin_floorf(fy);
            rowY1 = min(max(f0 + 1, 0), (int)H - 1);
            rowY0 = min(max(f0, 0), (int)H - 1);
        }
#pragma unroll
        for (uint32_t it = 0; it < 16; ++it) {
            const int y0 = __builtin_amdgcn_readlane(rowY0, (int)it), y1 = __builtin_amdgcn_readlane(rowY1, (int)it);
            if (wide) {
                v0[it] = *reinterpret_cast<const Pair*>(depth + (uint64_t)y0 * W + xl);
                v1[it] = *reinterpret_cast<const Pair*>(depth + (uint64_t)y1 * W + xl);
            } else {
                v0[it] = { depth[(uint64_t)y0 * W + x0], depth[(uint64_t)y0 * W + x1] };
                v1[it] = { depth[(uint64_t)y1 * W + x0], depth[(uint64_t)y1 * W + x1] };
            }
        }
#pragma unroll
        for (uint32_t it = 0; it < 16; ++it) {
            const uint32_t ly = it * 4 + (tid >> 6), y = ty * 64 + ly;
            const float p = !wide || x0 == xl ? v0[it].a : v0[it].b, q = wide && x1 == xl ? v0[it].a : v0[it].b;
            const float r = !wide || x0 == xl ? v1[it].a : v1[it].b, t = wide && x1 == xl ? v1[it].a : v1[it].b;
            const _Float16 h = (_Float16)red4<MAX>(p, q, r, t);
            m0[(uint64_t)y * ow + x] = h;
            s0[ly * 64 + lx] = (float)h;
        }
    }
    __syncthreads();
    {
        const uint32_t px = (tid & 15) * 2, py = (tid >> 4) * 2;
        for (uint32_t dy = 0; dy < 2; ++dy)
            for (uint32_t dx = 0; dx < 2; ++dx) {
                const uint32_t ox = px + dx, oy = py + dy;
                const float v = red4<MAX>(s0[(2 * oy) * 64 + 2 * ox], s0[(2 * oy) * 64 + 2 * ox + 1],
                                          s0[(2 * oy + 1) * 64 + 2 * ox], s0[(2 * oy + 1) * 64 + 2 * ox + 1]);
                s[0][oy * 32 + ox] = v;
                if (lastMip >= 1) {
                    const uint32_t mw = a.width >> 1;
                    a.base[a.mipOffset[1] + (uint64_t)(ty * 32 + oy) * mw + tx * 32 + ox] = (_Float16)v;
                }
            }
    }
    __syncthreads();
    uint32_t cur = 0, dim = 32;
    for (uint32_t mip = 2; mip <= 6 && mip <= lastMip; ++mip) {
        const uint32_t od = dim >> 1;
        if (tid < od * od) {
            const uint32_t ox = tid % od, oy = tid / od;
            const float* p = s[cur];
            const float v = red4<MAX>(p[(2 * oy) * dim + 2 * ox], p[(2 * oy) * dim + 2 * ox + 1],
                                      p[(2 * oy + 1) * dim + 2 * ox], p[(2 * oy + 1) * dim + 2 * ox + 1]);
            s[cur ^ 1][oy * od + ox] = v;
            const uint32_t mw = a.width >> mip;
            a.base[a.mipOffset[mip] + (uint64_t)(ty * od + oy) * mw + tx * od + ox] = (_Float16)v;
        }
        __syncthreads();
        cur ^= 1;
        dim = od;
    }
}

template <bool MAX>
__global__ __launch_bounds__(256) void spdMipKernel(SpdArgs a, uint32_t mip)
{
    const uint32_t pw = (a.width >> (mip - 1)) ? (a.width >> (mip - 1)) : 1u, ph = (a.height >> (mip - 1)) ? (a.height >> (mip - 1)) : 1u;
    const uint32_t mw = (a.width >> mip) ? (a.width >> mip) : 1u, mh = (a.height >> mip) ? (a.height >> mip) : 1u;
    const uint32_t i = blockIdx.x * 256u + threadIdx.x;
    if (i >= mw * mh) return;
    const uint32_t x = i % mw, y = i / mw;
    const uint32_t x0 = min(2 * x, pw - 1), x1 = min(2 * x + 1, pw - 1);
    const uint32_t y0 = min(2 * y, ph - 1), y1 = min(2 * y + 1, ph - 1);
    const _Float16* p = a.base + a.mipOffset[mip - 1];
    a.base[a.mipOffset[mip] + i] = (_Float16)red4<MAX>((float)p[y0 * pw + x0], (float)p[y0 * pw + x1], (float)p[y1 * pw + x0], (float)p[y1 * pw + x1]);
}

struct MinMaxNote { const float* depth; uint32_t W, H; _Float16* out; uint32_t ow, oh; bool mx; };

template <bool MAX>
__global__ __launch_bounds__(1024) void spdTailKernel(SpdArgs a, uint32_t first)
{
    __shared__ float s[2][64 * 64];
    const uint32_t tid = threadIdx.x;
    uint32_t pw = (a.width >> first) ? (a.width >> first) : 1u, ph = (a.height >> first) ? (a.height >> first) : 1u;
    for (uint32_t i = tid; i < pw * ph; i += 1024) s[0][i] = (float)a.base[a.mipOffset[first] + i];
    __syncthreads();
    uint32_t cur = 0;
    for (uint32_t mip = first + 1; mip < a.mips; ++mip) {
        const uint32_t mw = (a.width >> mip) ? (a.width >> mip) : 1u, mh = (a.height >> mip) ? (a.height >> mip) : 1u;
        const float* p = s[cur];
        for (uint32_t i = tid; i < mw * mh; i += 1024) {
            const uint32_t x = i % mw, y = i / mw;
            const uint32_t x0 = min(2 * x, pw - 1), x1 = min(2 * x + 1, pw - 1);
            const uint32_t y0 = min(2 * y, ph - 1), y1 = min(2 * y + 1, ph - 1);
            const float v = red4<MAX>(p[y0 * pw + x0], p[y0 * pw + x1], p[y1 * pw + x0], p[y1 * pw + x1]);
            s[cur ^ 1][i] = v;
            a.base[a.mipOffset[mip] + i] = (_Float16)v;
        }
        __syncthreads();
        cur ^= 1;
        pw = mw; ph = mh;
    }
}

__global__ __launch_bounds__(256) void hzbQuadBuildKernel(trhip::QuadArgs a)
{
    __shared__ float s_t[9][trhip::kQuadStripCols + 1];
    trhip::hzbQuadStrip(a, blockIdx.x, s_t);
}


int recordMinMaxDownsample(trhip::DispatchCtx& ctx)
{
    const MinMaxDownsampleConsts* k = (const MinMaxDownsampleConsts*)ctx.constants(0, sizeof(MinMaxDownsampleConsts));
    TRHIP_REQUIRE(k, "%s: push constants (MinMaxDownsampleConsts, 12 bytes) missing", ctx.shaderName);
    trhip_texture_t* src = ctx.texture(TRHIP_BIND_TEXTURE_SRV, 0);
    uint32_t mip = 0;
    trhip_texture_t* dst = ctx.texture(TRHIP_BIND_TEXTURE_UAV, 0, &mip);
    TRHIP_REQUIRE(src && dst, "%s: needs Texture_SRV t0 (depth) and Texture_UAV u0 (HZB)", ctx.shaderName);
    TRHIP_REQUIRE(src->format == TRHIP_FORMAT_R32_FLOAT, "%s: depth source must be R32_FLOAT", ctx.shaderName);
    TRHIP_REQUIRE(dst->format == TRHIP_FORMAT_R16_FLOAT, "%s: HZB must be R16_FLOAT", ctx.shaderName);
    TRHIP_REQUIRE(k->m_OutputDimensions.x == dst->mipW(mip) && k->m_OutputDimensions.y == dst->mipH(mip),
                  "%s: m_OutputDimensions %ux%u does not match HZB mip %u (%ux%u)", ctx.shaderName,
                  k->m_OutputDimensions.x, k->m_OutputDimensions.y, mip, dst->mipW(mip), dst->mipH(mip));
    TRHIP_REQUIRE(!ctx.indirect, "%s: dispatched directly", ctx.shaderName);
    TRHIP_REQUIRE(ctx.gx >= (dst->mipW(mip) + 7) / 8 && ctx.gy >= (dst->mipH(mip) + 7) / 8,
                  "%s: dispatch %ux%u groups of 8x8 does not cover %ux%u (BasePassRenderers.cpp:533)", ctx.shaderName,
                  ctx.gx, ctx.gy, dst->mipW(mip), dst->mipH(mip));
    const float* depth = (const float*)src->mipPtr(0);
    _Float16* out = (_Float16*)dst->mipPtr(mip);
    const uint32_t W = src->width, H = src->height, ow = dst->mipW(mip), oh = dst->mipH(mip);
    const bool mx = k->m_bDownsampleMax != 0;
    ctx.emit("main", [=](hipStream_t s) {
        dim3 grid((ow + 31) / 32, (oh + 7) / 8);
        if (mx) TRHIP_LAUNCH(minMaxDownsampleKernel<true>, grid, dim3(256), 0, s, depth, W, H, out, ow, oh);
        else TRHIP_LAUNCH(minMaxDownsampleKernel<false>, grid, dim3(256), 0, s, depth, W, H, out, ow, oh);
        return trhip::launchStatus("minMaxDownsampleKernel"); });
    ctx.cl->peephole = { ctx.cl->ops.size() - 1, "minmaxdownsample", std::make_shared<MinMaxNote>(MinMaxNote{ depth, W, H, out, ow, oh, mx }) };
    return TRHIP_OK;
}

int recordSPD(trhip::DispatchCtx& ctx)
{
    const SPDConstants* k = (const SPDConstants*)ctx.constants(0, sizeof(SPDConstants));
    TRHIP_REQUIRE(k, "%s: push constants (SPDConstants, 32 bytes) missing", ctx.shaderName);
    uint32_t mip0 = 0;
    trhip_texture_t* tex = ctx.texture(TRHIP_BIND_TEXTURE_UAV, 2, &mip0);
    TRHIP_REQUIRE(tex, "%s: needs Texture_UAV u2 = HZB mip 0 (FFXHelpers.cpp:71)", ctx.shaderName);
    TRHIP_REQUIRE(mip0 == 0, "%s: u2 must be mip 0", ctx.shaderName);
    TRHIP_REQUIRE(tex->format == TRHIP_FORMAT_R16_FLOAT, "%s: HZB must be R16_FLOAT", ctx.shaderName);
    TRHIP_REQUIRE(k->mips == tex->mips - 1, "%s: SPDConstants.mips %u != HZB mips-1 %u (FFXHelpers.cpp:63-64)", ctx.shaderName, k->mips, tex->mips - 1);
    for (uint32_t i = 1; i < tex->mips; ++i) {
        uint32_t m = 0;
        trhip_texture_t* t = ctx.texture(TRHIP_BIND_TEXTURE_UAV, 2 + i, &m);
        TRHIP_REQUIRE(t == tex && m == i, "%s: UAV u%u must be HZB mip %u (FFXHelpers.cpp:76-81)", ctx.shaderName, 2 + i, i);
    }
    TRHIP_REQUIRE(!ctx.indirect, "%s: dispatched directly", ctx.shaderName);
    if (trhip_buffer_t* counter = ctx.buffer(TRHIP_BIND_STRUCTURED_UAV, 0)) ctx.cl->forgetUse(counter->ptr, ctx.cl->ops.size());
    const bool mx = ctx.variant == 2;
    SpdArgs a;
    memset(&a, 0, sizeof a);
    a.base = (_Float16*)tex->ptr;
    a.width = tex->width; a.height = tex->height; a.mips = tex->mips;
    for (uint32_t i = 0; i < tex->mips; ++i) a.mipOffset[i] = (uint32_t)(tex->mipOffset[i] / 2);
    if (tex->mips <= 1) return TRHIP_OK;

    uint32_t first = 0;
    const bool tiled = (tex->width % 64 == 0) && (tex->height % 64 == 0);
    const trhip_cmdlist_t::Peephole ph = ctx.cl->peephole;
    const MinMaxNote* note = (ph.kind && !strcmp(ph.kind, "minmaxdownsample") && ph.op == ctx.cl->ops.size() - 1 && ph.op != SIZE_MAX) ? (const MinMaxNote*)ph.data.get() : nullptr;
    const bool fuse = tiled && note && note->out == a.base + a.mipOffset[0] && note->ow == tex->width && note->oh == tex->height && note->mx == mx
                      && ctx.cl->ops.back().lane == 0;
    if (fuse) {
        const MinMaxNote n = *note;
        const uint32_t lastMip = tex->mips - 1 < 6 ? tex->mips - 1 : 6;
        ctx.cl->ops.pop_back();
        ctx.emit("depth_tile", [a, n, lastMip, mx](hipStream_t s) {
            dim3 grid(a.width / 64, a.height / 64);
            if (mx) TRHIP_LAUNCH(hzbDepthTileKernel<true>, grid, dim3(256), 0, s, n.depth, n.W, n.H, a, lastMip);
            else TRHIP_LAUNCH(hzbDepthTileKernel<false>, grid, dim3(256), 0, s, n.depth, n.W, n.H, a, lastMip);
            return trhip::launchStatus("hzbDepthTileKernel"); });
        first = lastMip;
    } else if (tiled) {
        const uint32_t lastMip = tex->mips - 1 < 6 ? tex->mips - 1 : 6;
        ctx.emit("tile", [a, lastMip, mx](hipStream_t s) {
            dim3 grid(a.width / 64, a.height / 64);
            if (mx) TRHIP_LAUNCH(spdTileKernel<true>, grid, dim3(256), 0, s, a, lastMip);
            else TRHIP_LAUNCH(spdTileKernel<false>, grid, dim3(256), 0, s, a, lastMip);
            return trhip::launchStatus("spdTileKernel"); });
        first = lastMip;
    }
    while ((uint64_t)tex->mipW(first) * tex->mipH(first) > 64 * 64 && first + 1 < tex->mips) {
        const uint32_t mip = first + 1;
        const uint32_t texels = tex->mipW(mip) * tex->mipH(mip);
        ctx.emit("mip", [a, mip, texels, mx](hipStream_t s) {
            if (mx) TRHIP_LAUNCH(spdMipKernel<true>, dim3((texels + 255u) / 256u), dim3(256), 0, s, a, mip);
            else TRHIP_LAUNCH(spdMipKernel<false>, dim3((texels + 255u) / 256u), dim3(256), 0, s, a, mip);
            return trhip::launchStatus("spdMipKernel"); });
        first = mip;
    }
    if (first + 1 < tex->mips) {
        ctx.emit("tail", [a, first, mx](hipStream_t s) {
            if (mx) TRHIP_LAUNCH(spdTailKernel<true>, dim3(1), dim3(1024), 0, s, a, first);
            else TRHIP_LAUNCH(spdTailKernel<false>, dim3(1), dim3(1024), 0, s, a, first);
            return trhip::launchStatus("spdTailKernel"); });
    }
    return TRHIP_OK;
}

}

namespace trhip
{

int hzbQuadEnsure(trhip_texture_t* tex)
{
    TRHIP_REQUIRE(tex && tex->ptr && tex->format == TRHIP_FORMAT_R16_FLOAT && tex->mips <= 16, "footprint-min table: needs a bound R16_FLOAT texture");
    uint64_t total = 0;
    for (uint32_t k = 0; k < tex->mips; ++k) {
        tex->quadOffset[k] = (uint32_t)total;
        total += (uint64_t)((tex->mipW(k) >> 3) + 1) * ((tex->mipH(k) >> 3) + 1) * 64u;
    }
    TRHIP_REQUIRE(total < (1ull << 31), "footprint-min table: HZB %ux%u too large", tex->width, tex->height);
    tex->quadTotal = (uint32_t)total;
    return tex->quad.allocate(tex->dev, total * 2);
}

int hzbQuadLaunchBuild(trhip_texture_t* tex, hipStream_t s)
{
    const Stamp from = { tex->version };
    if (tex->quad.current(from)) return TRHIP_OK;
    const QuadArgs a = quadArgs(tex);
    TRHIP_LAUNCH(hzbQuadBuildKernel, dim3(a.firstStrip[a.mips]), dim3(256), 0, s, a);
    tex->quad.markBuilt(from);
    return launchStatus("hzbQuadBuildKernel");
}

}

namespace
{

trhip::ShaderRegistrar r0("minmaxdownsample_CS_Main", recordMinMaxDownsample, 0);
trhip::ShaderRegistrar r1("ffx_spd_downsample_pass_CS FFX_SPD_OPTION_DOWNSAMPLE_FILTER=1", recordSPD, 1);
trhip::ShaderRegistrar r2("ffx_spd_downsample_pass_CS FFX_SPD_OPTION_DOWNSAMPLE_FILTER=2", recordSPD, 2);

}
```

### toyrenderer_amd/csrc/trhip_core.cpp

```cpp
#include "trhip_internal.h"
#include "r11g11b10.hip.h"

#include <chrono>
#include <cmath>
#include <cstdlib>

#include <algorithm>
#include <memory>

namespace trhip
{

static thread_local char tl_error[1024] = "";

int fail(int code, const char* fmt, ...)
{
    va_list ap;
    va_start(ap, fmt);
    vsnprintf(tl_error, sizeof tl_error, fmt, ap);
    va_end(ap);
    return code;
}

int hipfail(hipError_t e, const char* what)
{
    return fail(TRHIP_ERR_HIP, "HIP error %d (%s) in %s", (int)e, hipGetErrorString(e), what);
}

struct ShaderEntry { std::string name; RecordFn fn; int variant; };
static std::vector<ShaderEntry>& shaders()
{
    static std::vector<ShaderEntry> s;
    return s;
}

void registerShader(const char* name, RecordFn fn, int variant)
{
    shaders().push_back({ name, fn, variant });
}

static const ShaderEntry* findShader(const char* name)
{
    for (const ShaderEntry& e : shaders())
        if (e.name == name) return &e;
    return nullptr;
}

trhip_buffer_t* DispatchCtx::buffer(uint32_t type, uint32_t slot) const
{
    for (uint32_t i = 0; i < numBindings; ++i)
        if (bindings[i].type == type && bindings[i].slot == slot)
            return (trhip_buffer_t*)bindings[i].resource;
    return nullptr;
}

trhip_texture_t* DispatchCtx::texture(uint32_t type, uint32_t slot, uint32_t* baseMip) const
{
    for (uint32_t i = 0; i < numBindings; ++i)
        if (bindings[i].type == type && bindings[i].slot == slot) {
            if (baseMip) *baseMip = bindings[i].baseMip;
            return (trhip_texture_t*)bindings[i].resource;
        }
    return nullptr;
}

const void* DispatchCtx::constants(uint32_t slot, size_t bytes) const
{
    for (uint32_t i = 0; i < numBindings; ++i) {
        if (bindings[i].slot != slot) continue;
        if (bindings[i].type == TRHIP_BIND_CONSTANT_BUFFER) {
            trhip_buffer_t* b = (trhip_buffer_t*)bindings[i].resource;
            if (!b || !b->isVolatileConstant || b->shadow.size() < bytes) return nullptr;
            return b->shadow.data();
        }
        if (bindings[i].type == TRHIP_BIND_PUSH_CONSTANTS) {
            if (!push || pushBytes < bytes) return nullptr;
            return push;
        }
    }
    return nullptr;
}

void DispatchCtx::emit(const char* kernelName, std::function<int(hipStream_t)> fn) const
{
    std::string n = std::string(shaderName) + "#" + kernelName;
    cl->ops.push_back({ std::move(n), std::move(fn) });
}

void DispatchCtx::emitSide(const char* kernelName, std::function<int(hipStream_t)> fn, std::initializer_list<Op::Access> touched) const
{
// ... 39 lines not shown
    (void)hipEventCreate(&e);
    return e;
}

int trhip_device_t::drainProfile()
{
    for (ProfilePending& p : pending) {
        float ms = 0;
        TRHIP_HIP(hipEventSynchronize(p.e1));
        TRHIP_HIP(hipEventElapsedTime(&ms, p.e0, p.e1));
        auto it = accum.find(p.name);
        if (it == accum.end()) { accumOrder.push_back(p.name); it = accum.emplace(p.name, ProfileAccum{}).first; }
        it->second.launches += 1;
        it->second.totalMs += ms;
        eventPool.push_back(p.e0);
        eventPool.push_back(p.e1);
    }
    pending.clear();
    return TRHIP_OK;
}

static void* arenaAlloc(std::vector<trhip_cmdlist_t::ScratchBlock>& arena, int deviceIndex, size_t bytes)
{
    bytes = (bytes + 255) & ~size_t(255);
    if (bytes == 0) bytes = 256;
    for (trhip_cmdlist_t::ScratchBlock& b : arena)
        if (b.bytes - b.used >= bytes) { void* p = (char*)b.ptr + b.used; b.used += bytes; return p; }
    size_t blockBytes = std::max(bytes, size_t(1) << 20);
    void* p = nullptr;
    if (hipSetDevice(deviceIndex) != hipSuccess || hipMalloc(&p, blockBytes) != hipSuccess) return nullptr;
    arena.push_back({ p, blockBytes, bytes });
    return p;
}

void* trhip_cmdlist_t::scratchAlloc(size_t bytes) { return arenaAlloc(scratch, dev->index, bytes); }
void* trhip_cmdlist_t::scratchAllocSide(size_t bytes) { return arenaAlloc(sideScratch, dev->index, bytes); }

int trhip_device_t::syncAll()
{
    TRHIP_HIP(hipStreamSynchronize(stream));
    if (sideStream) TRHIP_HIP(hipStreamSynchronize(sideStream));
    return TRHIP_OK;
}

int trhip::DerivedData::allocate(const trhip_device_t* dev, uint64_t size)
{
    if (ptr) return size <= bytes ? TRHIP_OK : fail(TRHIP_ERR_STATE, "derived data of %llu bytes asked to grow to %llu", (unsigned long long)bytes, (unsigned long long)size);
    TRHIP_HIP(hipSetDevice(dev->index));
    void* p = nullptr;
    TRHIP_HIP(hipMalloc(&p, (size_t)size));
    ptr = p;
    bytes = size;
    return TRHIP_OK;
}

void trhip::freeDerived(trhip_device_t* dev, std::initializer_list<DerivedData*> all)
{
    bool any = false;
    for (const DerivedData* d : all) any |= d->ptr != nullptr;
    if (!any) return;
    (void)hipSetDevice(dev->index);
    (void)dev->syncAll();
    for (const DerivedData* d : all)
        if (d->ptr) (void)hipFree(d->ptr);
}

void trhip_cmdlist_t::resetRecording()
{
    ops.clear();
    for (trhip_buffer_t* b : heldBuffers) trhip_buffer_release(b);
    for (trhip_texture_t* t : heldTextures) trhip_texture_release(t);
    heldBuffers.clear();
    heldTextures.clear();
    markers.clear();
    openStats = nullptr;
    statsHostCS = 0;
    useMarks.clear();
    openClearBatch.reset();
    openClearOp = SIZE_MAX;
    firstClearBatch.reset();
    firstClearOp = SIZE_MAX;
    clearedTo.clear();
    peephole = Peephole();
    for (ScratchBlock& b : scratch) b.used = 0;
    for (ScratchBlock& b : sideScratch) b.used = 0;
}

namespace
{
struct ClearKernelArgs { void* ptr[trhip_cmdlist_t::ClearBatch::kMax]; uint64_t words[trhip_cmdlist_t::ClearBatch::kMax]; uint32_t value[trhip_cmdlist_t::ClearBatch::kMax]; uint32_t count; };

__global__ __launch_bounds__(256) void multiClearKernel(ClearKernelArgs a)
{
    const uint64_t stride = (uint64_t)gridDim.x * 256u;
    for (uint32_t k = 0; k < a.count; ++k) {
        uint32_t* p = (uint32_t*)a.ptr[k];
        const uint32_t v = a.value[k];
        for (uint64_t i = (uint64_t)blockIdx.x * 256u + threadIdx.x; i < a.words[k]; i += stride) p[i] = v;
    }
}
}

int trhip_cmdlist_t::recordClearWords(void* ptr, uint64_t words, uint32_t value, bool fresh)
{
    if (words == 0) return TRHIP_OK;
    if (fresh && firstClearBatch && firstClearBatch->count < ClearBatch::kMax) {
        ClearBatch& f = *firstClearBatch;
        f.ptr[f.count] = ptr; f.words[f.count] = words; f.value[f.count] = value;
        ++f.count;
        return TRHIP_OK;
    }
    if (!(openClearBatch && openClearOp == ops.size() - 1 && openClearBatch->count < ClearBatch::kMax)) {
        openClearBatch = std::make_shared<ClearBatch>();
        std::shared_ptr<ClearBatch> b = openClearBatch;
        const uint32_t cus = dev->computeUnits;
        ops.push_back({ "", [b, cus](hipStream_t s) {
            ClearKernelArgs a;
            uint64_t most = 0;
            a.count = b->count;
            for (uint32_t k = 0; k < b->count; ++k) { a.ptr[k] = b->ptr[k]; a.words[k] = b->words[k]; a.value[k] = b->value[k]; most = std::max(most, b->words[k]); }
            uint64_t grid = (most + 1023u) / 1024u;
            if (grid > (uint64_t)cus * 8u) grid = (uint64_t)cus * 8u;
            if (grid == 0) grid = 1;
            TRHIP_LAUNCH(multiClearKernel, dim3((uint32_t)grid), dim3(256), 0, s, a);
            return trhip::launchStatus("multiClearKernel"); } });
        ops.back().kind = "clear_buffer";
        openClearOp = ops.size() - 1;
        if (!firstClearBatch) { firstClearBatch = openClearBatch; firstClearOp = openClearOp; }
    }
    ClearBatch& b = *openClearBatch;
    b.ptr[b.count] = ptr; b.words[b.count] = words; b.value[b.count] = value;
    ++b.count;
    return TRHIP_OK;
}

void trhip_cmdlist_t::hold(trhip_buffer_t* b, bool write, size_t op) { if (b) { use(b->ptr, op == SIZE_MAX ? ops.size() : op, write, &b->version); trhip_buffer_retain(b); heldBuffers.push_back(b); } }
void trhip_cmdlist_t::hold(trhip_texture_t* t, bool write) { if (t) { use(t->ptr, ops.size(), write, &t->version); trhip_texture_retain(t); heldTextures.push_back(t); } }

extern "C" {

const char* trhip_last_error(void) { return tl_error; }
uint32_t trhip_abi_version(void) { return TRHIP_ABI_VERSION; }
uint32_t trhip_shader_count(void) { return (uint32_t)shaders().size(); }
const char* trhip_shader_name(uint32_t i) { return i < shaders().size() ? shaders()[i].name.c_str() : nullptr; }
int trhip_shader_exists(const char* name) { return name && findShader(name) ? 1 : 0; }

static int deviceCreate(int index, void* stream, bool external, trhip_device* out)
{
    if (!out) return fail(TRHIP_ERR_INVALID, "out is null");
    int n = 0;
    if (hipGetDeviceCount(&n) != hipSuccess || n <= 0)
        return fail(TRHIP_ERR_NO_DEVICE, "no HIP device visible (this back end has no CPU fallback)");
    if (index < 0 || index >= n) return fail(TRHIP_ERR_INVALID, "device index %d out of range (%d devices)", index, n);
    TRHIP_HIP(hipSetDevice(index));
    hipDeviceProp_t props;
    TRHIP_HIP(hipGetDeviceProperties(&props, index));
    auto dev = std::make_unique<trhip_device_t>();
    dev->index = index;
    dev->computeUnits = (uint32_t)props.multiProcessorCount;
    dev->waveSize = (uint32_t)props.warpSize;
    dev->totalMem = (uint64_t)props.totalGlobalMem;
    if (dev->waveSize != 64)
        return fail(TRHIP_ERR_INVALID, "wave size %u: the kernels are written for wave64 (gfx950)", dev->waveSize);
    if (external) {
        dev->stream = (hipStream_t)stream;
        dev->ownsStream = false;
    } else {
        TRHIP_HIP(hipStreamCreateWithFlags(&dev->stream, hipStreamNonBlocking));
        dev->ownsStream = true;
    }
    if (!getenv("TRHIP_NO_SIDE_STREAM")) {
        int lowest = 0, highest = 0;
        TRHIP_HIP(hipDeviceGetStreamPriorityRange(&lowest, &highest));
        TRHIP_HIP(hipStreamCreateWithPriority(&dev->sideStream, hipStreamNonBlocking, highest));
        TRHIP_HIP(hipEventCreateWithFlags(&dev->evFork, hipEventDisableTiming));
        for (hipEvent_t& e : dev->runDone) TRHIP_HIP(hipEventCreateWithFlags(&e, hipEventDisableTiming));
    }
    *out = dev.release();
    return TRHIP_OK;
}

int trhip_device_create(int device_index, trhip_device* out) { return deviceCreate(device_index, nullptr, false, out); }
int trhip_device_create_on_stream(int device_index, void* s, trhip_device* out) { return deviceCreate(device_index, s, true, out); }

void trhip_device_destroy(trhip_device dev)
{
    if (!dev) return;
    (void)hipSetDevice(dev->index);
    (void)dev->syncAll();
    (void)dev->drainProfile();
    for (hipEvent_t e : dev->eventPool) (void)hipEventDestroy(e);
    if (dev->sideStream) { (void)hipStreamSynchronize(dev->sideStream); (void)hipStreamDestroy(dev->sideStream); }
    if (dev->evFork) (void)hipEventDestroy(dev->evFork);
    for (hipEvent_t e : dev->runDone) if (e) (void)hipEventDestroy(e);
    if (dev->ownsStream) (void)hipStreamDestroy(dev->stream);
    delete dev;
}

int trhip_device_wait_idle(trhip_device dev)
{
    if (!dev) return fail(TRHIP_ERR_INVALID, "device is null");
    TRHIP_HIP(hipSetDevice(dev->index));
    return dev->syncAll();
}

int trhip_device_join_side_stream(trhip_device dev)
{
    if (!dev) return fail(TRHIP_ERR_INVALID, "device is null");
    TRHIP_HIP(hipSetDevice(dev->index));
    std::lock_guard<std::mutex> lock(dev->mutex);
    if (dev->sideStream && dev->sideRunCounter > dev->mainWaitedUpTo) {
        TRHIP_HIP(hipStreamWaitEvent(dev->stream, dev->runDone[dev->sideRunCounter % trhip_device_t::kSideRuns], 0));
        dev->mainWaitedUpTo = dev->sideRunCounter;
    }
    return TRHIP_OK;
}
// ... 207 lines not shown
    if (off + bytes > b->byteSize) return fail(TRHIP_ERR_INVALID, "buffer_upload(%s): range exceeds the buffer", b->name.c_str());
    int rc = syncCopy(b->dev, (char*)b->ptr + off, src, bytes, hipMemcpyHostToDevice);
    b->version.fetch_add(1);
    return rc;
}

int trhip_buffer_mark_written(trhip_buffer b)
{
    if (!b) return fail(TRHIP_ERR_INVALID, "buffer_mark_written: null argument");
    b->version.fetch_add(1);
    return TRHIP_OK;
}

int trhip_texture_mark_written(trhip_texture t)
{
    if (!t) return fail(TRHIP_ERR_INVALID, "texture_mark_written: null argument");
    t->version.fetch_add(1);
    return TRHIP_OK;
}

int trhip_buffer_download(trhip_buffer b, uint64_t off, void* dst, uint64_t bytes)
{
    if (!b || !dst) return fail(TRHIP_ERR_INVALID, "buffer_download: null argument");
    if (!b->ptr) return fail(TRHIP_ERR_STATE, "buffer_download(%s): no memory bound", b->name.c_str());
    if (off + bytes > b->byteSize) return fail(TRHIP_ERR_INVALID, "buffer_download(%s): range exceeds the buffer", b->name.c_str());
    return syncCopy(b->dev, dst, (char*)b->ptr + off, bytes, hipMemcpyDeviceToHost);
}

int trhip_texture_upload(trhip_texture t, uint32_t mip, const void* src, uint64_t bytes)
{
    if (!t || !src || mip >= t->mips) return fail(TRHIP_ERR_INVALID, "texture_upload: bad argument");
    if (!t->ptr) return fail(TRHIP_ERR_STATE, "texture_upload(%s): no memory bound", t->name.c_str());
    uint64_t need = (uint64_t)t->mipW(mip) * t->mipH(mip) * t->texelBytes;
    if (bytes != need) return fail(TRHIP_ERR_INVALID, "texture_upload(%s): mip %u is %llu bytes, got %llu", t->name.c_str(), mip, (unsigned long long)need, (unsigned long long)bytes);
    int rc = syncCopy(t->dev, t->mipPtr(mip), src, bytes, hipMemcpyHostToDevice);
    t->version.fetch_add(1);
    return rc;
}

int trhip_texture_download(trhip_texture t, uint32_t mip, void* dst, uint64_t bytes)
{
    if (!t || !dst || mip >= t->mips) return fail(TRHIP_ERR_INVALID, "texture_download: bad argument");
    if (!t->ptr) return fail(TRHIP_ERR_STATE, "texture_download(%s): no memory bound", t->name.c_str());
    uint64_t need = (uint64_t)t->mipW(mip) * t->mipH(mip) * t->texelBytes;
    if (bytes != need) return fail(TRHIP_ERR_INVALID, "texture_download(%s): mip %u is %llu bytes, got %llu", t->name.c_str(), mip, (unsigned long long)need, (unsigned long long)bytes);
    return syncCopy(t->dev, dst, t->mipPtr(mip), bytes, hipMemcpyDeviceToHost);
}

int trhip_cmd_create(trhip_device dev, trhip_cmdlist* out)
{
    if (!dev || !out) return fail(TRHIP_ERR_INVALID, "cmd_create: null argument");
    auto cl = std::make_unique<trhip_cmdlist_t>();
    cl->dev = dev;
    *out = cl.release();
    return TRHIP_OK;
}

void trhip_cmd_release(trhip_cmdlist cl)
{
    if (!cl) return;
    (void)hipSetDevice(cl->dev->index);
    (void)cl->dev->syncAll();
    cl->resetRecording();
    for (auto& b : cl->scratch) (void)hipFree(b.ptr);
    for (auto& b : cl->sideScratch) (void)hipFree(b.ptr);
    delete cl;
}

int trhip_cmd_open(trhip_cmdlist cl)
{
    if (!cl) return fail(TRHIP_ERR_INVALID, "cmdlist is null");
    if (cl->open) return fail(TRHIP_ERR_STATE, "cmd_open: already open");
    cl->resetRecording();
    cl->open = true;
    return TRHIP_OK;
}

int trhip_cmd_close(trhip_cmdlist cl)
{
    if (!cl) return fail(TRHIP_ERR_INVALID, "cmdlist is null");
    if (!cl->open) return fail(TRHIP_ERR_STATE, "cmd_close: not open");
    if (!cl->markers.empty()) return fail(TRHIP_ERR_STATE, "cmd_close: %zu marker(s) still open", cl->markers.size());
    if (cl->openStats) return fail(TRHIP_ERR_STATE, "cmd_close: a pipeline statistics query is still open");
    cl->open = false;
    std::stable_sort(cl->useMarks.begin(), cl->useMarks.end(), [](const trhip_cmdlist_t::UseMark& a, const trhip_cmdlist_t::UseMark& b) { return a.op < b.op; });
    return TRHIP_OK;
}

#define TRHIP_RECORDING(cl)                                                                  \
    do {                                                                                     \
        if (!(cl)) return fail(TRHIP_ERR_INVALID, "cmdlist is null");                        \
        if (!(cl)->open) return fail(TRHIP_ERR_STATE, "command list is not open");           \
    } while (0)

int trhip_cmd_write_buffer(trhip_cmdlist cl, trhip_buffer buf, uint64_t off, const void* src, uint64_t bytes)
{
    TRHIP_RECORDING(cl);
    if (!buf || !src) return fail(TRHIP_ERR_INVALID, "write_buffer: null argument");
    if (off + bytes > buf->byteSize) return fail(TRHIP_ERR_INVALID, "write_buffer(%s): %llu+%llu exceeds %llu bytes", buf->name.c_str(), (unsigned long long)off, (unsigned long long)bytes, (unsigned long long)buf->byteSize);
    if (buf->isVolatileConstant) {
        memcpy(buf->shadow.data() + off, src, (size_t)bytes);
        return TRHIP_OK;
    }
    if (!buf->ptr) return fail(TRHIP_ERR_STATE, "write_buffer(%s): no memory bound", buf->name.c_str());
    auto staged = std::make_shared<std::vector<uint8_t>>((const uint8_t*)src, (const uint8_t*)src + bytes);
    void* dst = (char*)buf->ptr + off;
    cl->hold(buf, true);
    cl->ops.push_back({ "", [staged, dst](hipStream_t s) {
        TRHIP_HIP(hipMemcpyAsync(dst, staged->data(), staged->size(), hipMemcpyHostToDevice, s));
        return (int)TRHIP_OK; } });
    cl->ops.back().kind = "write_buffer";
    return TRHIP_OK;
}

int trhip_cmd_clear_buffer_u32(trhip_cmdlist cl, trhip_buffer buf, uint32_t value)
{
    TRHIP_RECORDING(cl);
    if (!buf) return fail(TRHIP_ERR_INVALID, "clear_buffer: null buffer");
    if (!buf->ptr) return fail(TRHIP_ERR_STATE, "clear_buffer(%s): no memory bound", buf->name.c_str());
    if (buf->byteSize % 4) return fail(TRHIP_ERR_INVALID, "clear_buffer(%s): size not a multiple of 4", buf->name.c_str());
    if (cl->stillClearedTo(buf->ptr, value)) return TRHIP_OK;
    const bool hoist = !cl->usedSoFar(buf->ptr) && cl->firstClearBatch && cl->firstClearBatch->count < trhip_cmdlist_t::ClearBatch::kMax;
    const bool merges = cl->openClearBatch && cl->openClearOp == cl->ops.size() - 1 && cl->openClearBatch->count < trhip_cmdlist_t::ClearBatch::kMax;
    cl->hold(buf, true, hoist ? cl->firstClearOp : merges ? cl->openClearOp : cl->ops.size());
    int rc = cl->recordClearWords(buf->ptr, buf->byteSize / 4, value, hoist);
    if (rc == TRHIP_OK) cl->clearedTo[buf->ptr] = { value, cl->useMarks.size() };
    return rc;
}

int trhip_cmd_clear_texture_f32(trhip_cmdlist cl, trhip_texture tex, float value)
{
    TRHIP_RECORDING(cl);
    if (!tex) return fail(TRHIP_ERR_INVALID, "clear_texture: null texture");
    if (!tex->ptr) return fail(TRHIP_ERR_STATE, "clear_texture(%s): no memory bound", tex->name.c_str());
    if (tex->format == TRHIP_FORMAT_RG32_UINT || tex->format == TRHIP_FORMAT_RGBA32_UINT || tex->format == TRHIP_FORMAT_R8_UINT)
        return fail(TRHIP_ERR_INVALID, "clear_texture_f32(%s): RG32_UINT / RGBA32_UINT / R8_UINT are cleared with clear_texture_u32", tex->name.c_str());
    if (tex->format == TRHIP_FORMAT_RGBA8_UNORM)
        return fail(TRHIP_ERR_INVALID, "clear_texture_f32(%s): an RGBA8_UNORM texture has no clear: postprocess_PS_PostProcess writes every texel", tex->name.c_str());
    void* p = tex->ptr;
    cl->hold(tex, true);
    if (tex->format == TRHIP_FORMAT_R32_FLOAT || tex->format == TRHIP_FORMAT_R11G11B10_FLOAT) {
        uint32_t bits;
        memcpy(&bits, &value, 4);
        if (tex->format == TRHIP_FORMAT_R11G11B10_FLOAT) bits = trhip::packR11G11B10(value, value, value);
        size_t n = (size_t)(tex->totalBytes / 4);
        cl->ops.push_back({ "", [p, n, bits](hipStream_t s) { TRHIP_HIP(hipMemsetD32Async((hipDeviceptr_t)p, (int)bits, n, s)); return (int)TRHIP_OK; } });
        cl->ops.back().kind = "clear_texture";
    } else if (tex->format == TRHIP_FORMAT_R8_UNORM) {
        const float sat = value != value ? 0.0f : value < 0.0f ? 0.0f : value > 1.0f ? 1.0f : value;
        const int byte = (int)std::nearbyint(sat * 255.0f);
        size_t n = (size_t)tex->totalBytes;
        cl->ops.push_back({ "", [p, n, byte](hipStream_t s) { TRHIP_HIP(hipMemsetAsync(p, byte, n, s)); return (int)TRHIP_OK; } });
        cl->ops.back().kind = "clear_texture";
    } else {
        _Float16 h = (_Float16)value;
        uint16_t bits;
        memcpy(&bits, &h, 2);
        size_t n = (size_t)(tex->totalBytes / 2);
        cl->ops.push_back({ "", [p, n, bits](hipStream_t s) { TRHIP_HIP(hipMemsetD16Async((hipDeviceptr_t)p, bits, n, s)); return (int)TRHIP_OK; } });
        cl->ops.back().kind = "clear_texture";
    }
    return TRHIP_OK;
}

int trhip_cmd_clear_texture_u32(trhip_cmdlist cl, trhip_texture tex, uint32_t value)
{
    TRHIP_RECORDING(cl);
    if (!tex) return fail(TRHIP_ERR_INVALID, "clear_texture: null texture");
    if (!tex->ptr) return fail(TRHIP_ERR_STATE, "clear_texture(%s): no memory bound", tex->name.c_str());
    if (tex->format == TRHIP_FORMAT_RGBA8_UNORM)
        return fail(TRHIP_ERR_INVALID, "clear_texture_u32(%s): an RGBA8_UNORM texture has no clear: postprocess_PS_PostProcess writes every texel", tex->name.c_str());
    if (tex->format != TRHIP_FORMAT_RG32_UINT && tex->format != TRHIP_FORMAT_RGBA32_UINT && tex->format != TRHIP_FORMAT_R8_UINT)
        return fail(TRHIP_ERR_INVALID, "clear_texture_u32(%s): needs an RG32_UINT, RGBA32_UINT or R8_UINT texture", tex->name.c_str());
    void* p = tex->ptr;
    cl->hold(tex, true);
    if (tex->format == TRHIP_FORMAT_R8_UINT) {
        const int byte = (int)(value & 0xFFu);
        const size_t bytes = (size_t)tex->totalBytes;
        cl->ops.push_back({ "", [p, bytes, byte](hipStream_t s) { TRHIP_HIP(hipMemsetAsync(p, byte, bytes, s)); return (int)TRHIP_OK; } });
        cl->ops.back().kind = "clear_texture";
        return TRHIP_OK;
    }
    const size_t n = (size_t)(tex->totalBytes / 4);
    cl->ops.push_back({ "", [p, n, value](hipStream_t s) { TRHIP_HIP(hipMemsetD32Async((hipDeviceptr_t)p, (int)value, n, s)); return (int)TRHIP_OK; } });
    cl->ops.back().kind = "clear_texture";
    return TRHIP_OK;
}

int trhip_cmd_copy_buffer(trhip_cmdlist cl, trhip_buffer dst, uint64_t dstOff, trhip_buffer src, uint64_t srcOff, uint64_t bytes)
{
    TRHIP_RECORDING(cl);
    if (!dst || !src) return fail(TRHIP_ERR_INVALID, "copy_buffer: null buffer");
    if (!dst->ptr || !src->ptr) return fail(TRHIP_ERR_STATE, "copy_buffer: a buffer has no memory bound");
    if (dstOff + bytes > dst->byteSize || srcOff + bytes > src->byteSize) return fail(TRHIP_ERR_INVALID, "copy_buffer(%s <- %s): range exceeds a buffer", dst->name.c_str(), src->name.c_str());
    void* d = (char*)dst->ptr + dstOff;
    const void* sp = (const char*)src->ptr + srcOff;
    cl->hold(dst, true); cl->hold(src, false);
    cl->ops.push_back({ "", [d, sp, bytes](hipStream_t s) { TRHIP_HIP(hipMemcpyAsync(d, sp, (size_t)bytes, hipMemcpyDeviceToDevice, s)); return (int)TRHIP_OK; } });
    cl->ops.back().kind = "copy_buffer";
    return TRHIP_OK;
}

int trhip_cmd_host_callback(trhip_cmdlist cl, trhip_host_fn fn, void* user)
{
    TRHIP_RECORDING(cl);
    if (!fn) return fail(TRHIP_ERR_INVALID, "host_callback: null function");
    cl->ops.push_back({ "", [fn, user](hipStream_t s) { fn(user, (void*)s); return (int)TRHIP_OK; } });
    cl->ops.back().kind = "host_callback";
    return TRHIP_OK;
}

int trhip_cmd_copy_texture(trhip_cmdlist cl, trhip_texture dst, trhip_texture src)
{
    TRHIP_RECORDING(cl);
    if (!dst || !src) return fail(TRHIP_ERR_INVALID, "copy_texture: null texture");
    if (!dst->ptr || !src->ptr) return fail(TRHIP_ERR_STATE, "copy_texture: a texture has no memory bound");
    if (dst->width != src->width || dst->height != src->height || dst->mips != src->mips || dst->format != src->format)
        return fail(TRHIP_ERR_INVALID, "copy_texture(%s <- %s): descriptions differ", dst->name.c_str(), src->name.c_str());
    void* d = dst->ptr;
    const void* sp = src->ptr;
    const uint64_t bytes = src->totalBytes;
    cl->hold(dst, true); cl->hold(src, false);
    cl->ops.push_back({ "", [d, sp, bytes](hipStream_t s) { TRHIP_HIP(hipMemcpyAsync(d, sp, (size_t)bytes, hipMemcpyDeviceToDevice, s)); return (int)TRHIP_OK; } });
    cl->ops.back().kind = "copy_texture";
    return TRHIP_OK;
}

static int recordDispatch(trhip_cmdlist cl, const char* name, const trhip_binding* b, uint32_t nb, const void* push, uint32_t pushBytes,
                          bool indirect, trhip_buffer args, uint32_t argsOff, uint32_t gx, uint32_t gy, uint32_t gz)
{
    TRHIP_RECORDING(cl);
    if (!name) return fail(TRHIP_ERR_INVALID, "dispatch: shader name is null");
    const ShaderEntry* e = findShader(name);
    if (!e) return fail(TRHIP_ERR_UNKNOWN_SHADER, "dispatch: unknown shader '%s'", name);
    if (nb && !b) return fail(TRHIP_ERR_INVALID, "dispatch(%s): bindings is null", name);
    if (indirect) {
        if (!args || !args->ptr) return fail(TRHIP_ERR_INVALID, "dispatch_indirect(%s): no argument buffer", name);
        if (argsOff % 4 || argsOff + 12 > args->byteSize) return fail(TRHIP_ERR_INVALID, "dispatch_indirect(%s): bad argument offset %u", name, argsOff);
        cl->hold(args, false);
    } else if (gx == 0 || gy == 0 || gz == 0) {
        return fail(TRHIP_ERR_INVALID, "dispatch(%s): zero group count (Graphic.cpp:944)", name);
    }
    for (uint32_t i = 0; i < nb; ++i) {
        switch (b[i].type) {
        case TRHIP_BIND_CONSTANT_BUFFER: case TRHIP_BIND_STRUCTURED_SRV: case TRHIP_BIND_STRUCTURED_UAV: {
            trhip_buffer_t* r = (trhip_buffer_t*)b[i].resource;
            if (!r) return fail(TRHIP_ERR_INVALID, "dispatch(%s): binding %u has no buffer", name, i);
            if (b[i].type != TRHIP_BIND_CONSTANT_BUFFER && !r->ptr) return fail(TRHIP_ERR_STATE, "dispatch(%s): buffer '%s' has no memory bound", name, r->name.c_str());
            if (b[i].type == TRHIP_BIND_STRUCTURED_UAV && !r->canHaveUAVs) return fail(TRHIP_ERR_INVALID, "dispatch(%s): buffer '%s' bound as UAV without canHaveUAVs", name, r->name.c_str());
            cl->hold(r, b[i].type == TRHIP_BIND_STRUCTURED_UAV);
            break; }
        case TRHIP_BIND_TEXTURE_SRV: case TRHIP_BIND_TEXTURE_UAV: {
            trhip_texture_t* t = (trhip_texture_t*)b[i].resource;
            if (!t) return fail(TRHIP_ERR_INVALID, "dispatch(%s): binding %u has no texture", name, i);
            if (!t->ptr) return fail(TRHIP_ERR_STATE, "dispatch(%s): texture '%s' has no memory bound", name, t->name.c_str());
            if (b[i].type == TRHIP_BIND_TEXTURE_UAV && b[i].baseMip >= t->mips) return fail(TRHIP_ERR_INVALID, "dispatch(%s): UAV mip %u out of range", name, b[i].baseMip);
            cl->hold(t, b[i].type == TRHIP_BIND_TEXTURE_UAV);
            break; }
        case TRHIP_BIND_PUSH_CONSTANTS: case TRHIP_BIND_SAMPLER: break;
        default: return fail(TRHIP_ERR_INVALID, "dispatch(%s): binding %u has unknown type %u", name, i, b[i].type);
        }
    }
    DispatchCtx ctx{ cl, e->name.c_str(), e->variant, b, nb, push, pushBytes, indirect, args, argsOff, gx, gy, gz };
    int rc = e->fn(ctx);
    if (rc != TRHIP_OK || !cl->openStats) return rc;
    const uint32_t threads = statsCSThreads(name);
    if (!threads) return TRHIP_OK;
    if (!indirect) { cl->statsHostCS += (uint64_t)gx * gy * gz * threads; return TRHIP_OK; }
    return statsEmitIndirectCS(cl, args, argsOff, threads);
}

int trhip_cmd_dispatch(trhip_cmdlist cl, const char* name, const trhip_binding* b, uint32_t nb, const void* push, uint32_t pushBytes,
                       uint32_t gx, uint32_t gy, uint32_t gz)
{
    return recordDispatch(cl, name, b, nb, push, pushBytes, false, nullptr, 0, gx, gy, gz);
}

int trhip_cmd_dispatch_indirect(trhip_cmdlist cl, const char* name, const trhip_binding* b, uint32_t nb, const void* push, uint32_t pushBytes,
                                trhip_buffer args, uint32_t argsOff)
{
    return recordDispatch(cl, name, b, nb, push, pushBytes, true, args, argsOff, 0, 0, 0);
}

int trhip_cmd_begin_timer(trhip_cmdlist cl, trhip_timer t)
{
    TRHIP_RECORDING(cl);
    if (!t) return fail(TRHIP_ERR_INVALID, "timer is null");
    cl->ops.push_back({ "", [t](hipStream_t s) { TRHIP_HIP(hipEventRecord(t->e0, s)); t->began = true; t->ended = false; return (int)TRHIP_OK; } });
    cl->ops.back().kind = "timer";
    return TRHIP_OK;
}

int trhip_cmd_end_timer(trhip_cmdlist cl, trhip_timer t)
{
    TRHIP_RECORDING(cl);
    if (!t) return fail(TRHIP_ERR_INVALID, "timer is null");
    cl->ops.push_back({ "", [t](hipStream_t s) { TRHIP_HIP(hipEventRecord(t->e1, s)); t->ended = true; return (int)TRHIP_OK; } });
    cl->ops.back().kind = "timer";
    return TRHIP_OK;
}

int trhip_cmd_begin_pipeline_stats(trhip_cmdlist cl, trhip_pipeline_stats q)
{
    TRHIP_RECORDING(cl);
    if (!q) return fail(TRHIP_ERR_INVALID, "pipeline statistics query is null");
    if (q->dev != cl->dev) return fail(TRHIP_ERR_INVALID, "begin_pipeline_stats: the query belongs to another device");
    if (cl->openStats) return fail(TRHIP_ERR_STATE, "begin_pipeline_stats: this command list already has a query open");
    cl->openStats = q;
    cl->statsHostCS = 0;
    cl->peephole = trhip_cmdlist_t::Peephole();
    cl->use(q->counters, cl->ops.size(), true);
    cl->ops.push_back({ "", [q](hipStream_t s) {
        TRHIP_HIP(hipMemsetAsync(q->counters, 0, sizeof(trhip_pipeline_statistics), s));
        q->began = true; q->ended = false;
        return (int)TRHIP_OK; } });
    cl->ops.back().kind = "pipeline_stats";
    return TRHIP_OK;
}

int trhip_cmd_end_pipeline_stats(trhip_cmdlist cl, trhip_pipeline_stats q)
{
    TRHIP_RECORDING(cl);
    if (!q) return fail(TRHIP_ERR_INVALID, "pipeline statistics query is null");
    if (cl->openStats != q) return fail(TRHIP_ERR_STATE, "end_pipeline_stats: the query is not open in this command list");
    const uint64_t hostCS = cl->statsHostCS;
    cl->openStats = nullptr;
    cl->statsHostCS = 0;
    cl->peephole = trhip_cmdlist_t::Peephole();
    cl->use(q->counters, cl->ops.size(), true);
    cl->ops.push_back({ "", [q, hostCS](hipStream_t s) {
        if (hostCS) {
            int rc = statsLaunchAdd(q->counters + kStatCS, hostCS, s);
            if (rc != TRHIP_OK) return rc;
        }
        TRHIP_HIP(hipEventRecord(q->done, s));
        q->ended = true;
        return (int)TRHIP_OK; } });
    cl->ops.back().kind = "pipeline_stats";
    return TRHIP_OK;
}

int trhip_cmd_begin_marker(trhip_cmdlist cl, const char* name)
{
    TRHIP_RECORDING(cl);
    cl->markers.push_back(name ? name : "");
    return TRHIP_OK;
}

int trhip_cmd_end_marker(trhip_cmdlist cl)
{
    TRHIP_RECORDING(cl);
    if (cl->markers.empty()) return fail(TRHIP_ERR_STATE, "end_marker without begin_marker");
    cl->markers.pop_back();
    return TRHIP_OK;
}

int trhip_queue_execute(trhip_device dev, const trhip_cmdlist* lists, uint32_t n)
{
    if (!dev || (n && !lists)) return fail(TRHIP_ERR_INVALID, "queue_execute: null argument");
    TRHIP_HIP(hipSetDevice(dev->index));
    std::lock_guard<std::mutex> lock(dev->mutex);
    bool inRun = false;
    std::vector<Op::Access> runTouched;
    auto endRun = [&]() -> int {
        if (!inRun) return TRHIP_OK;
        inRun = false;
        const uint64_t id = ++dev->sideRunCounter;
        const uint32_t slot = (uint32_t)(id % trhip_device_t::kSideRuns);
        if (id > trhip_device_t::kSideRuns && id - trhip_device_t::kSideRuns > dev->mainWaitedUpTo) {
            TRHIP_HIP(hipStreamWaitEvent(dev->stream, dev->runDone[slot], 0));
            dev->mainWaitedUpTo = id - trhip_device_t::kSideRuns;
        }
        TRHIP_HIP(hipEventRecord(dev->runDone[slot], dev->sideStream));
        for (const Op::Access& t : runTouched) (t.write ? dev->sideWriter : dev->sideReader)[t.ptr] = id;
        runTouched.clear();
        return TRHIP_OK;
    };
    auto ownerOf = [&](const void* ptr, bool write) -> uint64_t {
        uint64_t need = 0;
        auto w = dev->sideWriter.find(ptr);
        if (w != dev->sideWriter.end()) need = w->second;
        if (write) {
            auto r = dev->sideReader.find(ptr);
            if (r != dev->sideReader.end() && r->second > need) need = r->second;
        }
        return need;
    };
    auto waitForRun = [&](uint64_t need) -> int {
        if (need <= dev->mainWaitedUpTo) return TRHIP_OK;
        TRHIP_HIP(hipStreamWaitEvent(dev->stream, dev->runDone[need % trhip_device_t::kSideRuns], 0));
        dev->mainWaitedUpTo = need;
        return TRHIP_OK;
    };
    auto nextIsSide = [&](uint32_t li, size_t oi) -> bool {
        if (!dev->sideStream) return false;
        for (++oi; li < n; ++li, oi = 0)
            if (lists[li] && oi < lists[li]->ops.size()) return lists[li]->ops[oi].lane == 1;
        return false;
    };
    for (uint32_t i = 0; i < n; ++i) {
        trhip_cmdlist_t* cl = lists[i];
        if (!cl) return fail(TRHIP_ERR_INVALID, "queue_execute: list %u is null", i);
        if (cl->open) return fail(TRHIP_ERR_STATE, "queue_execute: list %u is still open", i);
        if (cl->dev != dev) return fail(TRHIP_ERR_INVALID, "queue_execute: list %u belongs to another device", i);
        size_t mark = 0;
// ... 212 lines not shown
```

### toyrenderer_amd/csrc/trhip_internal.h

```cpp
#pragma once

#include <hip/hip_runtime.h>

#include <atomic>
#include <cstdarg>
#include <cstdint>
#include <cstdio>
#include <cstdlib>
#include <cstring>
#include <functional>
#include <map>
#include <memory>
#include <mutex>
#include <string>
#include <unordered_map>
#include <vector>

#include <hip/hip_ext.h>

#include "../../include/trhip.h"
#include "ShaderInterop.h"

namespace trhip
{

int fail(int code, const char* fmt, ...) __attribute__((format(printf, 2, 3)));
int hipfail(hipError_t e, const char* what);

#define TRHIP_HIP(expr)                                                        \
    do {                                                                       \
        hipError_t _e = (expr);                                                \
        if (_e != hipSuccess) return ::trhip::hipfail(_e, #expr);              \
    } while (0)

#define TRHIP_REQUIRE(cond, ...)                                               \
    do {                                                                       \
        if (!(cond)) return ::trhip::fail(TRHIP_ERR_INVALID, __VA_ARGS__);     \
    } while (0)

struct ProfilePending { std::string name; hipEvent_t e0, e1; };
struct ProfileAccum { uint64_t launches = 0; double totalMs = 0; };

}

struct trhip_device_t
{
    int index = 0;
    hipStream_t stream = nullptr;
    bool ownsStream = false;
    uint32_t computeUnits = 0;
    uint32_t waveSize = 0;
    uint64_t totalMem = 0;

    static constexpr uint32_t kSideRuns = 16;
    hipStream_t sideStream = nullptr;
    hipEvent_t evFork = nullptr;
    bool forkSignalled = false;
    hipEvent_t runDone[kSideRuns] = {};
    uint64_t sideRunCounter = 0;
    uint64_t mainWaitedUpTo = 0;
    std::unordered_map<const void*, uint64_t> sideWriter;
    std::unordered_map<const void*, uint64_t> sideReader;
    int syncAll();

    std::mutex mutex;
    bool profiling = false;
    std::string profileFilter;
    std::vector<trhip::ProfilePending> pending;
    std::vector<hipEvent_t> eventPool;
    std::map<std::string, trhip::ProfileAccum> accum;
    std::vector<std::string> accumOrder;

    hipEvent_t acquireEvent();
    int drainProfile();
};

struct trhip_heap_t
{
    trhip_device_t* dev = nullptr;
    void* base = nullptr;
    uint64_t bytes = 0;
    std::atomic<int> rc{1};
};

namespace trhip
{

struct Stamp
{
    uint64_t version = 0;
    const void* other = nullptr;
    uint64_t otherVersion = 0;
    bool operator==(const Stamp& s) const { return version == s.version && other == s.other && otherVersion == s.otherVersion; }
};

struct DerivedData
{
    void* ptr = nullptr;
    uint64_t bytes = 0;
    Stamp built;

    int allocate(const trhip_device_t* dev, uint64_t size);
    bool current(const Stamp& s) const { return built == s; }
    void markBuilt(const Stamp& s) { built = s; }
// ... 47 lines not shown
};

struct trhip_timer_t
{
    trhip_device_t* dev = nullptr;
    hipEvent_t e0 = nullptr, e1 = nullptr;
    bool began = false, ended = false;
};

struct MeshletCullArgs;

struct trhip_pipeline_stats_t
{
    trhip_device_t* dev = nullptr;
    unsigned long long* counters = nullptr;
    hipEvent_t done = nullptr;
    bool began = false, ended = false;
};

namespace trhip
{

enum : uint32_t { kStatCS = 10, kStatAS = 11, kStatMS = 12, kStatMSPrim = 13, kStatWords = 14 };

struct Op
{
    std::string name;
    std::function<int(hipStream_t)> fn;
    const char* kind = "dispatch";
    uint8_t lane = 0;
    struct Access { const void* ptr; bool write; };
    std::vector<Access> touched;
};

}

struct trhip_cmdlist_t
{
    trhip_device_t* dev = nullptr;
    bool open = false;
    std::vector<trhip::Op> ops;
    std::vector<trhip_buffer_t*> heldBuffers;
    std::vector<trhip_texture_t*> heldTextures;
    std::vector<std::string> markers;
    trhip_pipeline_stats_t* openStats = nullptr;
    uint64_t statsHostCS = 0;

    struct ScratchBlock { void* ptr; size_t bytes; size_t used; };
    std::vector<ScratchBlock> scratch;

    struct ClearBatch { static constexpr uint32_t kMax = 32; void* ptr[kMax]; uint64_t words[kMax]; uint32_t value[kMax]; uint32_t count = 0; };
    std::shared_ptr<ClearBatch> openClearBatch;
    size_t openClearOp = SIZE_MAX;
    std::shared_ptr<ClearBatch> firstClearBatch;
    size_t firstClearOp = SIZE_MAX;
    struct ClearedTo { uint32_t value; size_t marks; };
    std::unordered_map<const void*, ClearedTo> clearedTo;
    bool stillClearedTo(const void* ptr, uint32_t value) const
    {
        auto it = clearedTo.find(ptr);
        if (it == clearedTo.end() || it->second.value != value) return false;
        for (size_t i = it->second.marks; i < useMarks.size(); ++i)
            if (useMarks[i].ptr == ptr && useMarks[i].write) return false;
        return true;
    }
    int recordClearWords(void* ptr, uint64_t words, uint32_t value, bool fresh = false);
    bool usedSoFar(const void* ptr) const { for (const UseMark& m : useMarks) if (m.ptr == ptr) return true; return false; }

    struct UseMark { size_t op; const void* ptr; bool write; std::atomic<uint64_t>* version; };
    std::vector<UseMark> useMarks;
    void use(const void* ptr, size_t op, bool write, std::atomic<uint64_t>* version = nullptr)
    {
        if (!ptr) return;
        useMarks.push_back({ op, ptr, write, version });
    }
    void forgetUse(const void* ptr, size_t op)
    {
        for (size_t i = useMarks.size(); i-- > 0 && useMarks[i].op >= op;)
            if (useMarks[i].op == op && useMarks[i].ptr == ptr) useMarks.erase(useMarks.begin() + (ptrdiff_t)i);
    }

    struct Peephole { size_t op = SIZE_MAX; const char* kind = nullptr; std::shared_ptr<void> data; } peephole;

    void* scratchAlloc(size_t bytes);
    void* scratchAllocSide(size_t bytes);
    std::vector<ScratchBlock> sideScratch;
    void resetRecording();
    void hold(trhip_buffer_t* b, bool write, size_t op = SIZE_MAX);
    void hold(trhip_texture_t* t, bool write);
};

namespace trhip
{

struct DispatchCtx
{
    trhip_cmdlist_t* cl;
    const char* shaderName;
    int variant;
    const trhip_binding* bindings; uint32_t numBindings;
    const void* push; uint32_t pushBytes;
    bool indirect; trhip_buffer_t* argsBuffer; uint32_t argsOffset;
    uint32_t gx, gy, gz;

    trhip_buffer_t* buffer(uint32_t type, uint32_t slot) const;
    trhip_texture_t* texture(uint32_t type, uint32_t slot, uint32_t* baseMip = nullptr) const;
    const void* constants(uint32_t slot, size_t bytes) const;
    uint32_t computeUnits() const { return cl->dev->computeUnits; }
    void* scratch(size_t bytes) const { return cl->scratchAlloc(bytes); }
    void* scratchSide(size_t bytes) const { return cl->dev->sideStream ? cl->scratchAllocSide(bytes) : cl->scratchAlloc(bytes); }
    void emit(const char* kernelName, std::function<int(hipStream_t)> fn) const;
    void emitSide(const char* kernelName, std::function<int(hipStream_t)> fn, std::initializer_list<Op::Access> touched) const;
};

int hzbQuadEnsure(trhip_texture_t* tex);
int hzbQuadLaunchBuild(trhip_texture_t* tex, hipStream_t s);

int instanceCacheEnsure(trhip_buffer_t* instances);
int instanceCacheLaunchBuild(trhip_buffer_t* instances, trhip_buffer_t* meshData, hipStream_t s);

inline uint32_t tableMinGroups()
{
    static const uint32_t v = [] { const char* e = getenv("TRHIP_TABLE_MIN_GROUPS"); return e ? (uint32_t)strtoul(e, nullptr, 0) : (1u << 17); }();
    return v;
}

uint32_t statsCSThreads(const char* shaderName);
int statsLaunchAdd(unsigned long long* counter, uint64_t value, hipStream_t s);
int statsEmitIndirectCS(trhip_cmdlist_t* cl, trhip_buffer_t* args, uint32_t argsOffset, uint32_t threads);
int statsEmitAS(const DispatchCtx& ctx, const ::MeshletCullArgs& a, trhip_buffer_t* meshlets, trhip_buffer_t* records,
                trhip_buffer_t* instances, trhip_buffer_t* meshData, bool side);

using RecordFn = int (*)(DispatchCtx&);
void registerShader(const char* name, RecordFn fn, int variant);

struct ShaderRegistrar
{
    ShaderRegistrar(const char* name, RecordFn fn, int variant = 0) { registerShader(name, fn, variant); }
};

struct LaunchTap { hipStream_t onStream = nullptr; hipEvent_t stopEvent = nullptr; int launches = 0; };
extern thread_local LaunchTap* g_launchTap;
#define TRHIP_LAUNCH(kernel, grid, block, shmem, stream, ...)                                                       \
    do {                                                                                                            \
        trhip::LaunchTap* tap_ = trhip::g_launchTap;                                                                \
        if (tap_ && tap_->onStream == (stream) && ++tap_->launches)                                              \
            hipExtLaunchKernelGGL(kernel, grid, block, shmem, stream, nullptr, tap_->stopEvent, 0, __VA_ARGS__);    \
        else                                                                                                        \
            hipLaunchKernelGGL(kernel, grid, block, shmem, stream, __VA_ARGS__);                                    \
    } while (0)

inline int launchStatus(const char* what)
{
    hipError_t e = hipGetLastError();
    return e == hipSuccess ? TRHIP_OK : hipfail(e, what);
}

}
```

Before: 123.3.

## Carry meshlet list build into later dispatches and host it in spare blocks

Instead of emitting the count/scan/expand list-build kernels right after the meshlet cull, the command list now carries the pending list build forward. Later dispatches (HZB downsample, late culling, late AS) run its stages inside extra grid rows of their own kernels, and any other command flushes the carried work first. The list-build device code moves into a shared header so several kernels can call it. This is meant to remove separate small kernel launches and let the list build overlap with independent work, at the cost of more complex recording logic and dependency hazards.

```diff
diff --git a/toyrenderer_amd/csrc/k_basepass_as.hip b/toyrenderer_amd/csrc/k_basepass_as.hip
--- a/toyrenderer_amd/csrc/k_basepass_as.hip
+++ b/toyrenderer_amd/csrc/k_basepass_as.hip
@@ -1,6 +1,7 @@
 #include <algorithm>
 #include <cstdlib>
 #include <string>
+#include <tuple>
 #include <type_traits>
 
 #if defined(TR_STAMPS) || defined(TR_COUNT_SLOW) || defined(TR_COUNT_PATHS)
@@ -163,9 +164,11 @@
 #ifndef TR_CULL_WAVES_PER_EU
 #define TR_CULL_WAVES_PER_EU 5
 #endif
-template <bool FRUSTUM, bool OCCLUSION, bool CONE, bool TABLE>
-__global__ __launch_bounds__(kCullBlock, TR_CULL_WAVES_PER_EU) void meshletCullKernel(MeshletCullArgs a)
-{
+template <bool FRUSTUM, bool OCCLUSION, bool CONE, bool TABLE, typename... Host>
+__global__ __launch_bounds__(kCullBlock, TR_CULL_WAVES_PER_EU) void meshletCullKernel(MeshletCullArgs a, Host... host)
+{
+    constexpr bool HOST = sizeof...(Host) != 0;
+    static_assert(!HOST || !TABLE, "the deferred mode never hosts");
 #ifdef TR_STAMPS
     unsigned long long stampSum[8] = {0, 0, 0, 0, 0, 0, 0, 0};
     unsigned long long stampLast = __builtin_amdgcn_s_memtime();
@@ -182,6 +185,12 @@
     __shared__ __attribute__((aligned(8))) uint32_t s_maskAll[kCullWaves][kCullBatch + 2];
     __shared__ __attribute__((aligned(16))) char s_ring[kCullWaves][kRingSlots][kSlotBytes];
 
+    if constexpr (HOST) {
+        if (blockIdx.y != 0) {
+            trhip::listWorkRun<kCullBlock, trhip::kListExpand>(std::get<0>(std::tie(host...)), (blockIdx.y - 1u) * gridDim.x + blockIdx.x, (gridDim.y - 1u) * gridDim.x, s_ring);
+            return;
+        }
+    }
     const uint32_t G = groupCount(a);
     const uint32_t tid = threadIdx.x, lane = tid & 63u, wave = tid >> 6;
     const uint32_t half = lane >> 5, sub = lane & 31u;
@@ -624,129 +633,39 @@
 #endif
 }
 
-__device__ __forceinline__ uint32_t waveSum(uint32_t v)
-{
-    v += (uint32_t)__builtin_amdgcn_update_dpp(0, (int)v, 0x111, 0xf, 0xf, true);
-    v += (uint32_t)__builtin_amdgcn_update_dpp(0, (int)v, 0x112, 0xf, 0xf, true);
-    v += (uint32_t)__builtin_amdgcn_update_dpp(0, (int)v, 0x114, 0xf, 0xf, true);
-    v += (uint32_t)__builtin_amdgcn_update_dpp(0, (int)v, 0x118, 0xf, 0xf, true);
-    v += (uint32_t)__builtin_amdgcn_update_dpp(0, (int)v, 0x142, 0xa, 0xf, false);
-    v += (uint32_t)__builtin_amdgcn_update_dpp(0, (int)v, 0x143, 0xc, 0xf, false);
-    return (uint32_t)__builtin_amdgcn_readlane((int)v, 63);
-}
-
+using trhip::waveSum;
+using trhip::waveInclusiveScan;
 #ifndef TR_SUPER_SHIFT
 #define TR_SUPER_SHIFT 8
 #endif
-constexpr uint32_t kSuperShift = TR_SUPER_SHIFT;
-constexpr uint32_t kSuperBatches = 1u << kSuperShift;
+static_assert(trhip::kSuperShift == TR_SUPER_SHIFT, "one super size for the list build");
+using trhip::kSuperShift;
+using trhip::kSuperBatches;
+static_assert(kBatch == trhip::kListBatch && kSteps == trhip::kListSteps, "one batch size for the cull's list build");
 constexpr uint32_t kCountThreads = 1024;
 constexpr uint32_t kCountWaves = kCountThreads / 64;
+
+__device__ __forceinline__ trhip::ListBuildArgs listArgsOf(const MeshletCullArgs& a)
+{
+    return { a.visMask, a.listGroups, a.batchSum, a.superSum, a.visibleList, a.listCapacity, a.drawArgs };
+}
+
 __global__ __launch_bounds__(kCountThreads) void visCountKernel(MeshletCullArgs a)
 {
     __shared__ uint32_t s_part[kCountWaves];
-    const uint32_t G = listGroupCount(a);
-    const uint32_t numBatches = (G + kBatch - 1) / kBatch;
-    const uint32_t numSupers = (numBatches + kSuperBatches - 1) >> kSuperShift;
-    const uint32_t lane = threadIdx.x & 63u, wave = threadIdx.x >> 6;
-    constexpr uint32_t kPerWave = kSuperBatches / kCountWaves;
-    for (uint32_t sb = blockIdx.x; sb < numSupers; sb += gridDim.x) {
-        const uint32_t b0 = (sb << kSuperShift) + wave * kPerWave;
-        uint32_t pc[kPerWave];
-#pragma unroll
-        for (uint32_t i = 0; i < kPerWave; ++i) {
-            const uint32_t g = (b0 + i) * kBatch + lane;
-            pc[i] = g < G ? (uint32_t)__popc(a.visMask[g]) : 0u;
-        }
-        uint32_t mine = 0;
-#pragma unroll
-        for (uint32_t i = 0; i < kPerWave; ++i) {
-            pc[i] = waveSum(pc[i]);
-            if (lane == 0 && b0 + i < numBatches) a.batchSum[b0 + i] = pc[i];
-            mine += pc[i];
-        }
-        __syncthreads();
-        if (lane == 0) s_part[wave] = mine;
-        __syncthreads();
-        if (threadIdx.x == 0) {
-            uint32_t total = 0;
-#pragma unroll
-            for (uint32_t w = 0; w < kCountWaves; ++w) total += s_part[w];
-            a.superSum[sb] = total;
-        }
-    }
-}
-
-__device__ __forceinline__ uint32_t waveInclusiveScan(uint32_t v, uint32_t lane)
-{
-#pragma unroll
-    for (int d = 1; d < 64; d <<= 1) {
-        uint32_t n = __shfl_up(v, d);
-        if (lane >= (uint32_t)d) v += n;
-    }
-    return v;
+    trhip::visCountBlocks<kCountThreads>(listArgsOf(a), listGroupCount(a), blockIdx.x, gridDim.x, s_part);
 }
 
 __global__ __launch_bounds__(1024) void visSuperScanKernel(MeshletCullArgs a)
 {
     __shared__ uint32_t s_wave[16];
-    const uint32_t G = listGroupCount(a);
-    const uint32_t numBatches = (G + kBatch - 1) / kBatch;
-    const uint32_t numSupers = (numBatches + kSuperBatches - 1) >> kSuperShift;
-    const uint32_t tid = threadIdx.x, lane = tid & 63u, wave = tid >> 6;
-    uint32_t carry = 0;
-    for (uint32_t base = 0; base < numSupers; base += 1024u) {
-        const uint32_t i = base + tid;
-        const uint32_t v = i < numSupers ? a.superSum[i] : 0u;
-        const uint32_t inc = waveInclusiveScan(v, lane);
-        __syncthreads();
-        if (lane == 63) s_wave[wave] = inc;
-        __syncthreads();
-        uint32_t pre = 0, all = 0;
-#pragma unroll
-        for (uint32_t w = 0; w < 16; ++w) { if (w < wave) pre += s_wave[w]; all += s_wave[w]; }
-        if (i < numSupers) a.superSum[i] = carry + pre + inc - v;
-        carry += all;
-    }
-    if (tid == 0) { a.drawArgs[0] = carry; a.drawArgs[1] = 1; a.drawArgs[2] = 1; }
-}
-
-__global__ __launch_bounds__(kBlock) void visExpandKernel(MeshletCullArgs a)
-{
-    __shared__ uint2 s_mo[kWaves][kBatch];
-    const uint32_t G = listGroupCount(a);
-    const uint32_t numBatches = (G + kBatch - 1) / kBatch;
-    const uint32_t lane = threadIdx.x & 63u, wave = threadIdx.x >> 6;
-    const uint32_t half = lane >> 5, sub = lane & 31u;
-    const uint32_t bit = 1u << sub, below = bit - 1u;
-    uint2* mo = s_mo[wave];
-    for (uint32_t batch = blockIdx.x * kWaves + wave; batch < numBatches; batch += gridDim.x * kWaves) {
-        const uint32_t g0 = batch * kBatch;
-        const uint32_t mask = g0 + lane < G ? a.visMask[g0 + lane] : 0u;
-        const uint32_t sb = batch >> kSuperShift;
-        uint32_t before = 0;
-        for (uint32_t j = (sb << kSuperShift) + lane; j < batch; j += 64u) before += a.batchSum[j];
-        before = waveSum(before) + a.superSum[sb];
-        const uint32_t pc = (uint32_t)__popc(mask);
-        const uint32_t exc = waveInclusiveScan(pc, lane) - pc + before;
-        mo[lane] = make_uint2(mask, exc);
-        __builtin_amdgcn_fence(__ATOMIC_RELEASE, "wavefront");
-        __builtin_amdgcn_wave_barrier();
-        __builtin_amdgcn_fence(__ATOMIC_ACQUIRE, "wavefront");
-        uint32_t value = ((g0 + half) << 5) | sub;
-#pragma unroll 8
-        for (uint32_t s = 0; s < kSteps; ++s) {
-            const uint2 e = mo[2 * s + half];
-            if (e.x & bit) {
-                const uint32_t pos = e.y + (uint32_t)__popc(e.x & below);
-                if (pos < a.listCapacity) a.visibleList[pos] = value;
-            }
-            value += 2u << 5;
-        }
-        __builtin_amdgcn_fence(__ATOMIC_RELEASE, "wavefront");
-        __builtin_amdgcn_wave_barrier();
-        __builtin_amdgcn_fence(__ATOMIC_ACQUIRE, "wavefront");
-    }
+    trhip::visSuperScanBlock(listArgsOf(a), listGroupCount(a), s_wave);
+}
+
+__global__ __launch_bounds__(kBlock) void visExpandKernel(MeshletCullArgs a, uint32_t first16, uint32_t end16)
+{
+    __shared__ uint2 s_mo[kWaves * kBatch];
+    trhip::visExpandBlocks<kBlock>(listArgsOf(a), listGroupCount(a), first16, end16, blockIdx.x, gridDim.x, s_mo);
 }
 
 constexpr uint32_t kCompactTile = 2048;
@@ -1125,6 +1044,41 @@
     }
 }
 
+template <typename Emit>
+void emitListKernels(Emit&& emit, const MeshletCullArgs& a, uint32_t computeUnits, const std::string& p, uint32_t stage, uint32_t first16)
+{
+    const uint32_t needBlocks = (a.maxBatches + kWaves - 1) / kWaves;
+    uint32_t gridSmall = computeUnits * 8u;
+    if (gridSmall > needBlocks) gridSmall = needBlocks;
+    if (gridSmall == 0) gridSmall = 1;
+    const uint32_t supers = (a.maxBatches >> kSuperShift) + 1u;
+    if (stage == 0) emit(p + "count", [a, supers](hipStream_t s) {
+        TRHIP_LAUNCH(visCountKernel, dim3(supers), dim3(kCountThreads), 0, s, a);
+        return trhip::launchStatus("visCountKernel"); });
+    if (stage <= 1) emit(p + "scan", [a](hipStream_t s) {
+        TRHIP_LAUNCH(visSuperScanKernel, dim3(1), dim3(1024), 0, s, a);
+        return trhip::launchStatus("visSuperScanKernel"); });
+    if (first16 < 65536u) emit(p + "expand", [a, gridSmall, first16](hipStream_t s) {
+        TRHIP_LAUNCH(visExpandKernel, dim3(gridSmall), dim3(kBlock), 0, s, a, first16, 65536u);
+        return trhip::launchStatus("visExpandKernel"); });
+}
+
+int flushCarriedList(trhip_cmdlist_t* cl, const trhip_cmdlist_t::ListCarry& c)
+{
+    MeshletCullArgs a;
+    memset(&a, 0, sizeof a);
+    a.visMask = const_cast<uint32_t*>(c.l.visMask);
+    a.listGroups = const_cast<uint32_t*>(c.l.groups);
+    a.batchSum = c.l.batchSum; a.superSum = c.l.superSum;
+    a.visibleList = c.l.visibleList; a.listCapacity = c.l.listCapacity;
+    a.drawArgs = c.l.drawArgs;
+    a.maxBatches = c.maxBatches;
+    const trhip::DispatchCtx ctx{ cl, c.shader.c_str(), 0, nullptr, 0, nullptr, 0, false, nullptr, 0, 0, 0, 0 };
+    emitListKernels([&](const std::string& name, std::function<int(hipStream_t)> fn) { ctx.emit(name.c_str(), std::move(fn)); },
+                    a, ctx.computeUnits(), "", c.stage, c.stage == 2 ? c.given16 : 0u);
+    return TRHIP_OK;
+}
+
 void emitListBuild(const trhip::DispatchCtx& ctx, const MeshletCullArgs& a, const char* prefix, bool side, const void* argsBase)
 {
     auto emit = [&](const std::string& name, std::function<int(hipStream_t)> fn) {
@@ -1147,27 +1101,14 @@
             return;
         }
     }
-    const uint32_t needBlocks = (a.maxBatches + kWaves - 1) / kWaves;
-    uint32_t gridSmall = ctx.computeUnits() * 8u;
-    if (gridSmall > needBlocks) gridSmall = needBlocks;
-    if (gridSmall == 0) gridSmall = 1;
-    const std::string p = prefix;
-    const uint32_t supers = (a.maxBatches >> kSuperShift) + 1u;
-    emit(p + "count", [a, supers](hipStream_t s) {
-        TRHIP_LAUNCH(visCountKernel, dim3(supers), dim3(kCountThreads), 0, s, a);
-        return trhip::launchStatus("visCountKernel"); });
-    emit(p + "scan", [a](hipStream_t s) {
-        TRHIP_LAUNCH(visSuperScanKernel, dim3(1), dim3(1024), 0, s, a);
-        return trhip::launchStatus("visSuperScanKernel"); });
-    emit(p + "expand", [a, gridSmall](hipStream_t s) {
-        TRHIP_LAUNCH(visExpandKernel, dim3(gridSmall), dim3(kBlock), 0, s, a);
-        return trhip::launchStatus("visExpandKernel"); });
+    emitListKernels(emit, a, ctx.computeUnits(), prefix, 0, 0);
 }
 
 template <bool F, bool O, bool C>
-void launchCull(const MeshletCullArgs& a, uint32_t grid, bool table, hipStream_t s)
-{
-    if (O && table) TRHIP_LAUNCH((meshletCullKernel<F, O, C, true>), dim3(grid), dim3(kCullBlock), 0, s, a);
+void launchCull(const MeshletCullArgs& a, uint32_t grid, bool table, const trhip::ListWork& hosted, uint32_t extra, hipStream_t s)
+{
+    if (extra) TRHIP_LAUNCH((meshletCullKernel<F, O, C, false, trhip::ListWork>), dim3(grid, 1u + (extra + grid - 1u) / grid), dim3(kCullBlock), 0, s, a, hosted);
+    else if (O && table) TRHIP_LAUNCH((meshletCullKernel<F, O, C, true>), dim3(grid), dim3(kCullBlock), 0, s, a);
     else TRHIP_LAUNCH((meshletCullKernel<F, O, C, false>), dim3(grid), dim3(kCullBlock), 0, s, a);
 }
 
@@ -1278,12 +1219,14 @@
     a.numInstances = (uint32_t)(instances->byteSize / sizeof(BasePassInstanceConstants));
     a.cache = instanceCacheLayout(instances->cullCache.ptr, a.numInstances);
     a.maxBatches = (a.recordCapacity + kBatch - 1) / kBatch;
-    a.batchSum = (uint32_t*)(a.recordCapacity >= (1u << 19) ? ctx.scratchSide((size_t)a.maxBatches * 4)
-                                                            : ctx.scratch((size_t)a.maxBatches * 4));
+    const bool carried = ctx.variant == 0 && a.recordCapacity >= trhip::inlineListMinGroups();
+    const bool sideBuild = !carried && a.recordCapacity >= (1u << 19);
+    a.batchSum = (uint32_t*)(sideBuild ? ctx.scratchSide((size_t)a.maxBatches * 4)
+                                       : ctx.scratch((size_t)a.maxBatches * 4));
     TRHIP_REQUIRE(a.batchSum, "%s: scratch allocation failed", ctx.shaderName);
     {
         const size_t supers = (a.maxBatches >> kSuperShift) + 1u;
-        a.superSum = (uint32_t*)(a.recordCapacity >= (1u << 19) ? ctx.scratchSide(supers * 4) : ctx.scratch(supers * 4));
+        a.superSum = (uint32_t*)(sideBuild ? ctx.scratchSide(supers * 4) : ctx.scratch(supers * 4));
         TRHIP_REQUIRE(a.superSum, "%s: scratch allocation failed", ctx.shaderName);
     }
 
@@ -1303,7 +1246,11 @@
     trhip_texture_t* quadOwner = useTable ? hzb : nullptr;
     const bool table = useTable;
     if (quadOwner) ctx.cl->use(quadOwner->quad.ptr, ctx.cl->ops.size(), false);
-    ctx.emit("cull", [a, grid, flags, quadOwner, table, instances, meshData, meshlets](hipStream_t s) {
+    uint32_t extra = 0;
+    trhip::ListWork hosted;
+    memset(&hosted, 0, sizeof hosted);
+    if (ctx.variant == 1 && !table) hosted = ctx.cl->takeListWork(trhip_cmdlist_t::kWideHost, kCullWaves, &extra);
+    ctx.emit("cull", [a, grid, flags, quadOwner, table, hosted, extra, instances, meshData, meshlets](hipStream_t s) {
         if ((const void*)a.meshlets != meshlets->ptr)
             return trhip::fail(TRHIP_ERR_STATE, "basepass_AS_Main: the meshlet buffer was bound to other memory after this command list was recorded: record it again");
         {
@@ -1317,17 +1264,27 @@
             if (brc != TRHIP_OK) return brc;
         }
         switch (flags) {
-        case 0: launchCull<false, false, false>(a, grid, table, s); break;
-        case 1: launchCull<true, false, false>(a, grid, table, s); break;
-        case 2: launchCull<false, true, false>(a, grid, table, s); break;
-        case 3: launchCull<true, true, false>(a, grid, table, s); break;
-        case 4: launchCull<false, false, true>(a, grid, table, s); break;
-        case 5: launchCull<true, false, true>(a, grid, table, s); break;
-        case 6: launchCull<false, true, true>(a, grid, table, s); break;
-        default: launchCull<true, true, true>(a, grid, table, s); break;
+        case 0: launchCull<false, false, false>(a, grid, table, hosted, extra, s); break;
+        case 1: launchCull<true, false, false>(a, grid, table, hosted, extra, s); break;
+        case 2: launchCull<false, true, false>(a, grid, table, hosted, extra, s); break;
+        case 3: launchCull<true, true, false>(a, grid, table, hosted, extra, s); break;
+        case 4: launchCull<false, false, true>(a, grid, table, hosted, extra, s); break;
+        case 5: launchCull<true, false, true>(a, grid, table, hosted, extra, s); break;
+        case 6: launchCull<false, true, true>(a, grid, table, hosted, extra, s); break;
+        default: launchCull<true, true, true>(a, grid, table, hosted, extra, s); break;
         }
         return trhip::launchStatus("meshletCullKernel"); });
-    emitListBuild(ctx, a, "", a.recordCapacity >= (1u << 19), ctx.argsBuffer->ptr);
+    if (carried) {
+        auto c = std::make_unique<trhip_cmdlist_t::ListCarry>();
+        c->l = { a.visMask, a.listGroups, a.batchSum, a.superSum, a.visibleList, a.listCapacity, a.drawArgs };
+        c->maxBatches = a.maxBatches;
+        c->shader = ctx.shaderName;
+        c->visMask = visMask; c->visibleList = visList; c->drawArgs = drawArgs;
+        c->flush = flushCarriedList;
+        ctx.cl->listCarry = std::move(c);
+    } else {
+        emitListBuild(ctx, a, "", a.recordCapacity >= (1u << 19), ctx.argsBuffer->ptr);
+    }
     if (ctx.cl->openStats)
         return trhip::statsEmitAS(ctx, a, meshlets, records, instances, meshData, a.recordCapacity >= (1u << 19));
     return TRHIP_OK;
diff --git a/toyrenderer_amd/csrc/k_gpuculling.hip b/toyrenderer_amd/csrc/k_gpuculling.hip
--- a/toyrenderer_amd/csrc/k_gpuculling.hip
+++ b/toyrenderer_amd/csrc/k_gpuculling.hip
@@ -1,6 +1,7 @@
 #include "cull_math.hip.h"
 #include "hzb_quad.hip.h"
 #include "instance_cache.hip.h"
+#include "list_build.hip.h"
 #include "trhip_internal.h"
 
 using namespace interop;
@@ -475,16 +476,21 @@
 constexpr unsigned long long kFusedFlag = 1ull << 63, kFusedPoison = 1ull << 60;
 
 template <int LATE>
-__global__ __launch_bounds__(kBlock) void instanceFusedKernel(InstanceCullArgs a, trhip::QuadArgs q)
+__global__ __launch_bounds__(kBlock) void instanceFusedKernel(InstanceCullArgs a, trhip::QuadArgs q, trhip::ListWork hosted)
 {
     if (!LATE && blockIdx.x >= a.numBlocks) {
         __shared__ float s_t[9][trhip::kQuadStripCols + 1];
         trhip::hzbQuadStrip(q, blockIdx.x - a.numBlocks, s_t);
         return;
     }
-    __shared__ uint32_t s_waveG[kBlock / 64], s_waveL[kBlock / 64], s_waveS[kBlock / 64];
-    __shared__ unsigned long long s_preG[kBlock / 64], s_preLS[kBlock / 64];
-    __shared__ uint32_t s_tile;
+    __shared__ uint2 s_lds[LATE ? (kBlock / 64) * trhip::kListBatch : 16];
+    if (LATE && blockIdx.x >= a.numBlocks) {
+        trhip::listWorkRun<kBlock, trhip::kListExpand>(hosted, blockIdx.x - a.numBlocks, gridDim.x - a.numBlocks, s_lds);
+        return;
+    }
+    unsigned long long* const s_preG = (unsigned long long*)s_lds, * const s_preLS = s_preG + kBlock / 64;
+    uint32_t* const s_waveG = (uint32_t*)(s_preLS + kBlock / 64), * const s_waveL = s_waveG + kBlock / 64, * const s_waveS = s_waveL + kBlock / 64;
+    uint32_t& s_tile = s_waveS[kBlock / 64];
     const uint32_t n = threadCount<LATE>(a);
     const uint32_t numTiles = (n + kBlock - 1) / kBlock < a.numBlocks ? (n + kBlock - 1) / kBlock : a.numBlocks;
     const uint32_t tid = threadIdx.x, lane = tid & 63u, wave = tid >> 6;
@@ -623,7 +629,7 @@
             strips = q.firstStrip[q.mips];
             quadOwner->quad.markBuilt({ quadOwner->version });
         }
-        TRHIP_LAUNCH(instanceFusedKernel<0>, dim3(a.numBlocks + strips), dim3(kBlock), 0, s, a, q);
+        TRHIP_LAUNCH(instanceFusedKernel<0>, dim3(a.numBlocks + strips), dim3(kBlock), 0, s, a, q, trhip::ListWork{});
         return trhip::launchStatus("instanceFusedKernel"); };
 }
 
@@ -747,11 +753,15 @@
         a.fusedTicket = mem + (size_t)a.numBlocks * kFusedStatusStride * 2;
         trhip_texture_t* quadOwner = wantTable ? hzb : nullptr;
         if (quadOwner) ctx.cl->use(quadOwner->quad.ptr, ctx.cl->ops.size(), true);
-        if (LATE) ctx.emit("fused", [a](hipStream_t s) {
-            trhip::QuadArgs q;
-            memset(&q, 0, sizeof q);
-            TRHIP_LAUNCH(instanceFusedKernel<LATE>, dim3(a.numBlocks), dim3(kBlock), 0, s, a, q);
-            return trhip::launchStatus("instanceFusedKernel"); });
+        if (LATE) {
+            uint32_t extra = 0;
+            const trhip::ListWork hosted = ctx.cl->takeListWork(trhip_cmdlist_t::kWideHost, kBlock / 64, &extra);
+            ctx.emit("fused", [a, hosted, extra](hipStream_t s) {
+                trhip::QuadArgs q;
+                memset(&q, 0, sizeof q);
+                TRHIP_LAUNCH(instanceFusedKernel<LATE>, dim3(a.numBlocks + extra), dim3(kBlock), 0, s, a, q, hosted);
+                return trhip::launchStatus("instanceFusedKernel"); });
+        }
         else ctx.emit("fused", fusedEarlyLaunch(a, quadOwner));
         if (!LATE && occlusion) ctx.cl->peephole = { ctx.cl->ops.size() - 1, "gpuculling_early", std::make_shared<EarlyCullNote>(EarlyCullNote{ a, ctx.cl->ops.size() - 1, true, quadOwner }) };
         return TRHIP_OK;
diff --git a/toyrenderer_amd/csrc/k_hzb.hip b/toyrenderer_amd/csrc/k_hzb.hip
--- a/toyrenderer_amd/csrc/k_hzb.hip
+++ b/toyrenderer_amd/csrc/k_hzb.hip
@@ -1,5 +1,6 @@
 #include "cull_math.hip.h"
 #include "hzb_quad.hip.h"
+#include "list_build.hip.h"
 #include "trhip_internal.h"
 
 using namespace interop;
@@ -81,10 +82,15 @@
 }
 
 template <bool MAX>
-__global__ __launch_bounds__(256) void hzbDepthTileKernel(const float* __restrict__ depth, uint32_t W, uint32_t H, SpdArgs a, uint32_t lastMip)
+__global__ __launch_bounds__(256) void hzbDepthTileKernel(const float* __restrict__ depth, uint32_t W, uint32_t H, SpdArgs a, uint32_t lastMip, trhip::ListWork hosted)
 {
     __shared__ float s0[64 * 64];
     __shared__ float s[2][32 * 32];
+    if (blockIdx.y >= a.height / 64) {
+        const uint32_t tilesY = a.height / 64;
+        trhip::listWorkRun<256, trhip::kListCount | trhip::kListExpand>(hosted, (blockIdx.y - tilesY) * gridDim.x + blockIdx.x, (gridDim.y - tilesY) * gridDim.x, s0);
+        return;
+    }
     const uint32_t tid = threadIdx.x;
     const uint32_t tx = blockIdx.x, ty = blockIdx.y;
     _Float16* m0 = a.base + a.mipOffset[0];
@@ -181,9 +187,13 @@
 struct MinMaxNote { const float* depth; uint32_t W, H; _Float16* out; uint32_t ow, oh; bool mx; };
 
 template <bool MAX>
-__global__ __launch_bounds__(1024) void spdTailKernel(SpdArgs a, uint32_t first)
+__global__ __launch_bounds__(1024) void spdTailKernel(SpdArgs a, uint32_t first, trhip::ListWork hosted)
 {
     __shared__ float s[2][64 * 64];
+    if (blockIdx.x >= 1) {
+        trhip::listWorkRun<1024, trhip::kListScan | trhip::kListExpand>(hosted, blockIdx.x - 1, gridDim.x - 1, s);
+        return;
+    }
     const uint32_t tid = threadIdx.x;
     uint32_t pw = (a.width >> first) ? (a.width >> first) : 1u, ph = (a.height >> first) ? (a.height >> first) : 1u;
     for (uint32_t i = tid; i < pw * ph; i += 1024) s[0][i] = (float)a.base[a.mipOffset[first] + i];
@@ -278,10 +288,13 @@
         const MinMaxNote n = *note;
         const uint32_t lastMip = tex->mips - 1 < 6 ? tex->mips - 1 : 6;
         ctx.cl->ops.pop_back();
-        ctx.emit("depth_tile", [a, n, lastMip, mx](hipStream_t s) {
-            dim3 grid(a.width / 64, a.height / 64);
-            if (mx) TRHIP_LAUNCH(hzbDepthTileKernel<true>, grid, dim3(256), 0, s, n.depth, n.W, n.H, a, lastMip);
-            else TRHIP_LAUNCH(hzbDepthTileKernel<false>, grid, dim3(256), 0, s, n.depth, n.W, n.H, a, lastMip);
+        uint32_t extra = 0;
+        const trhip::ListWork hosted = ctx.cl->takeListWork(trhip_cmdlist_t::kTileHost, 4, &extra);
+        const uint32_t extraRows = (extra + a.width / 64 - 1) / (a.width / 64);
+        ctx.emit("depth_tile", [a, n, lastMip, mx, hosted, extraRows](hipStream_t s) {
+            dim3 grid(a.width / 64, a.height / 64 + extraRows);
+            if (mx) TRHIP_LAUNCH(hzbDepthTileKernel<true>, grid, dim3(256), 0, s, n.depth, n.W, n.H, a, lastMip, hosted);
+            else TRHIP_LAUNCH(hzbDepthTileKernel<false>, grid, dim3(256), 0, s, n.depth, n.W, n.H, a, lastMip, hosted);
             return trhip::launchStatus("hzbDepthTileKernel"); });
         first = lastMip;
     } else if (tiled) {
@@ -303,9 +316,11 @@
         first = mip;
     }
     if (first + 1 < tex->mips) {
-        ctx.emit("tail", [a, first, mx](hipStream_t s) {
-            if (mx) TRHIP_LAUNCH(spdTailKernel<true>, dim3(1), dim3(1024), 0, s, a, first);
-            else TRHIP_LAUNCH(spdTailKernel<false>, dim3(1), dim3(1024), 0, s, a, first);
+        uint32_t extra = 0;
+        const trhip::ListWork hosted = ctx.cl->takeListWork(trhip_cmdlist_t::kTailHost, 16, &extra);
+        ctx.emit("tail", [a, first, mx, hosted, extra](hipStream_t s) {
+            if (mx) TRHIP_LAUNCH(spdTailKernel<true>, dim3(1 + extra), dim3(1024), 0, s, a, first, hosted);
+            else TRHIP_LAUNCH(spdTailKernel<false>, dim3(1 + extra), dim3(1024), 0, s, a, first, hosted);
             return trhip::launchStatus("spdTailKernel"); });
     }
     return TRHIP_OK;
diff --git a/toyrenderer_amd/csrc/list_build.hip.h b/toyrenderer_amd/csrc/list_build.hip.h
--- /dev/null
+++ b/toyrenderer_amd/csrc/list_build.hip.h
@@ -0,0 +1,166 @@
+#pragma once
+
+#include <hip/hip_runtime.h>
+
+#include <cstdint>
+
+namespace trhip
+{
+
+#ifndef TR_SUPER_SHIFT
+#define TR_SUPER_SHIFT 8
+#endif
+constexpr uint32_t kListBatch = 64;
+constexpr uint32_t kListSteps = kListBatch / 2;
+constexpr uint32_t kSuperShift = TR_SUPER_SHIFT;
+constexpr uint32_t kSuperBatches = 1u << kSuperShift;
+
+struct ListBuildArgs
+{
+    const uint32_t* visMask;
+    const uint32_t* groups;
+    uint32_t* batchSum;
+    uint32_t* superSum;
+    uint32_t* visibleList; uint32_t listCapacity;
+    uint32_t* drawArgs;
+};
+
+enum : uint32_t { kListNone = 0, kListCount = 1, kListScan = 2, kListExpand = 4 };
+struct ListWork
+{
+    ListBuildArgs l;
+    uint32_t phase;
+    uint32_t first16, end16;
+};
+
+__device__ __forceinline__ uint32_t waveSum(uint32_t v)
+{
+    v += (uint32_t)__builtin_amdgcn_update_dpp(0, (int)v, 0x111, 0xf, 0xf, true);
+    v += (uint32_t)__builtin_amdgcn_update_dpp(0, (int)v, 0x112, 0xf, 0xf, true);
+    v += (uint32_t)__builtin_amdgcn_update_dpp(0, (int)v, 0x114, 0xf, 0xf, true);
+    v += (uint32_t)__builtin_amdgcn_update_dpp(0, (int)v, 0x118, 0xf, 0xf, true);
+    v += (uint32_t)__builtin_amdgcn_update_dpp(0, (int)v, 0x142, 0xa, 0xf, false);
+    v += (uint32_t)__builtin_amdgcn_update_dpp(0, (int)v, 0x143, 0xc, 0xf, false);
+    return (uint32_t)__builtin_amdgcn_readlane((int)v, 63);
+}
+
+__device__ __forceinline__ uint32_t waveInclusiveScan(uint32_t v, uint32_t lane)
+{
+#pragma unroll
+    for (int d = 1; d < 64; d <<= 1) {
+        uint32_t n = __shfl_up(v, d);
+        if (lane >= (uint32_t)d) v += n;
+    }
+    return v;
+}
+
+template <uint32_t kThreads>
+__device__ __forceinline__ void visCountBlocks(const ListBuildArgs& l, uint32_t G, uint32_t block, uint32_t blocks, uint32_t* s_part)
+{
+    constexpr uint32_t kW = kThreads / 64, kPerWave = kSuperBatches / kW, kChunk = 16;
+    static_assert(kPerWave >= kChunk && kPerWave % kChunk == 0, "a wave's share of a super is whole chunks");
+    const uint32_t numBatches = (G + kListBatch - 1) / kListBatch;
+    const uint32_t numSupers = (numBatches + kSuperBatches - 1) >> kSuperShift;
+    const uint32_t lane = threadIdx.x & 63u, wave = threadIdx.x >> 6;
+    for (uint32_t sb = block; sb < numSupers; sb += blocks) {
+        uint32_t mine = 0;
+        for (uint32_t c = 0; c < kPerWave; c += kChunk) {
+            const uint32_t b0 = (sb << kSuperShift) + wave * kPerWave + c;
+            uint32_t pc[kChunk];
+#pragma unroll
+            for (uint32_t i = 0; i < kChunk; ++i) {
+                const uint32_t g = (b0 + i) * kListBatch + lane;
+                pc[i] = g < G ? (uint32_t)__popc(l.visMask[g]) : 0u;
+            }
+#pragma unroll
+            for (uint32_t i = 0; i < kChunk; ++i) {
+                pc[i] = waveSum(pc[i]);
+                if (lane == 0 && b0 + i < numBatches) l.batchSum[b0 + i] = pc[i];
+                mine += pc[i];
+            }
+        }
+        __syncthreads();
+        if (lane == 0) s_part[wave] = mine;
+        __syncthreads();
+        if (threadIdx.x == 0) {
+            uint32_t total = 0;
+#pragma unroll
+            for (uint32_t w = 0; w < kW; ++w) total += s_part[w];
+            l.superSum[sb] = total;
+        }
+    }
+}
+
+__device__ __forceinline__ void visSuperScanBlock(const ListBuildArgs& l, uint32_t G, uint32_t* s_wave)
+{
+    const uint32_t numBatches = (G + kListBatch - 1) / kListBatch;
+    const uint32_t numSupers = (numBatches + kSuperBatches - 1) >> kSuperShift;
+    const uint32_t tid = threadIdx.x, lane = tid & 63u, wave = tid >> 6;
+    uint32_t carry = 0;
+    for (uint32_t base = 0; base < numSupers; base += 1024u) {
+        const uint32_t i = base + tid;
+        const uint32_t v = i < numSupers ? l.superSum[i] : 0u;
+        const uint32_t inc = waveInclusiveScan(v, lane);
+        __syncthreads();
+        if (lane == 63) s_wave[wave] = inc;
+        __syncthreads();
+        uint32_t pre = 0, all = 0;
+#pragma unroll
+        for (uint32_t w = 0; w < 16; ++w) { if (w < wave) pre += s_wave[w]; all += s_wave[w]; }
+        if (i < numSupers) l.superSum[i] = carry + pre + inc - v;
+        carry += all;
+    }
+    if (tid == 0) { l.drawArgs[0] = carry; l.drawArgs[1] = 1; l.drawArgs[2] = 1; }
+}
+
+template <uint32_t kThreads>
+__device__ __forceinline__ void visExpandBlocks(const ListBuildArgs& l, uint32_t G, uint32_t first16, uint32_t end16, uint32_t block, uint32_t blocks, uint2* s_mo)
+{
+    constexpr uint32_t kW = kThreads / 64;
+    const uint32_t numBatches = (G + kListBatch - 1) / kListBatch;
+    const uint32_t batchFirst = (uint32_t)(((uint64_t)numBatches * first16) >> 16), batchEnd = (uint32_t)(((uint64_t)numBatches * end16) >> 16);
+    const uint32_t lane = threadIdx.x & 63u, wave = threadIdx.x >> 6;
+    const uint32_t half = lane >> 5, sub = lane & 31u;
+    const uint32_t bit = 1u << sub, below = bit - 1u;
+    uint2* mo = s_mo + wave * kListBatch;
+    for (uint32_t batch = batchFirst + block * kW + wave; batch < batchEnd; batch += blocks * kW) {
+        const uint32_t g0 = batch * kListBatch;
+        const uint32_t mask = g0 + lane < G ? l.visMask[g0 + lane] : 0u;
+        const uint32_t sb = batch >> kSuperShift;
+        uint32_t before = 0;
+        for (uint32_t j = (sb << kSuperShift) + lane; j < batch; j += 64u) before += l.batchSum[j];
+        before = waveSum(before) + l.superSum[sb];
+        const uint32_t pc = (uint32_t)__popc(mask);
+        const uint32_t exc = waveInclusiveScan(pc, lane) - pc + before;
+        mo[lane] = make_uint2(mask, exc);
+        __builtin_amdgcn_fence(__ATOMIC_RELEASE, "wavefront");
+        __builtin_amdgcn_wave_barrier();
+        __builtin_amdgcn_fence(__ATOMIC_ACQUIRE, "wavefront");
+        uint32_t value = ((g0 + half) << 5) | sub;
+#pragma unroll 8
+        for (uint32_t s = 0; s < kListSteps; ++s) {
+            const uint2 e = mo[2 * s + half];
+            if (e.x & bit) {
+                const uint32_t pos = e.y + (uint32_t)__popc(e.x & below);
+                if (pos < l.listCapacity) l.visibleList[pos] = value;
+            }
+            value += 2u << 5;
+        }
+        __builtin_amdgcn_fence(__ATOMIC_RELEASE, "wavefront");
+        __builtin_amdgcn_wave_barrier();
+        __builtin_amdgcn_fence(__ATOMIC_ACQUIRE, "wavefront");
+    }
+}
+
+template <uint32_t kThreads, uint32_t kPhases>
+__device__ __forceinline__ void listWorkRun(const ListWork& w, uint32_t block, uint32_t blocks, void* lds)
+{
+    const uint32_t G = w.l.groups[0];
+    if ((kPhases & kListCount) && w.phase == kListCount) visCountBlocks<kThreads>(w.l, G, block, blocks, (uint32_t*)lds);
+    if constexpr ((kPhases & kListScan) != 0 && kThreads == 1024) {
+        if (w.phase == kListScan && block == 0) visSuperScanBlock(w.l, G, (uint32_t*)lds);
+    }
+    if ((kPhases & kListExpand) && w.phase == kListExpand) visExpandBlocks<kThreads>(w.l, G, w.first16, w.end16, block, blocks, (uint2*)lds);
+}
+
+}
diff --git a/toyrenderer_amd/csrc/trhip_core.cpp b/toyrenderer_amd/csrc/trhip_core.cpp
--- a/toyrenderer_amd/csrc/trhip_core.cpp
+++ b/toyrenderer_amd/csrc/trhip_core.cpp
@@ -6,6 +6,7 @@
 #include <cstdlib>
 
 #include <algorithm>
+#include <array>
 #include <memory>
 
 namespace trhip
@@ -211,6 +212,7 @@
     firstClearOp = SIZE_MAX;
     clearedTo.clear();
     peephole = Peephole();
+    listCarry.reset();
     for (ScratchBlock& b : scratch) b.used = 0;
     for (ScratchBlock& b : sideScratch) b.used = 0;
 }
@@ -261,6 +263,79 @@
     b.ptr[b.count] = ptr; b.words[b.count] = words; b.value[b.count] = value;
     ++b.count;
     return TRHIP_OK;
+}
+
+uint32_t trhip::listSliceEnd16(uint32_t slice)
+{
+    static const std::array<uint32_t, 4> ends = [] {
+        double f[4] = { 0.29, 0.17, 0.36, 0.18 };
+        if (const char* e = getenv("TRHIP_LIST_SLICES")) {
+            for (double& v : f) v = 0.0;
+            char* end = nullptr;
+            for (int i = 0; i < 4 && *e; ++i) {
+                const double v = strtod(e, &end);
+                if (end == e) break;
+                f[i] = v < 0.0 ? 0.0 : v;
+                e = *end == ',' ? end + 1 : end;
+            }
+        }
+        std::array<uint32_t, 4> r{};
+        double sum = 0.0;
+        for (int i = 0; i < 4; ++i) {
+            sum += f[i];
+            r[i] = sum >= 0.99999 ? 65536u : (uint32_t)(sum * 65536.0);
+        }
+        return r; }();
+    return slice < 4 ? ends[slice] : ends[3];
+}
+
+trhip::ListWork trhip_cmdlist_t::takeListWork(ListHost host, uint32_t waves, uint32_t* extraBlocks)
+{
+    trhip::ListWork w;
+    memset(&w, 0, sizeof w);
+    *extraBlocks = 0;
+    if (!listCarry) return w;
+    ListCarry& c = *listCarry;
+    uint32_t blocks = 0;
+    if (c.stage == 0 && host == kTileHost) {
+        w.phase = trhip::kListCount;
+        blocks = (c.maxBatches >> trhip::kSuperShift) + 1u;
+        c.stage = 1;
+    } else if (c.stage == 1 && host == kTailHost) {
+        w.phase = trhip::kListScan;
+        blocks = 1;
+        c.stage = 2;
+    } else if (c.stage == 2 && c.slice < 4) {
+        const uint32_t end16 = std::max(trhip::listSliceEnd16(c.slice++), c.given16);
+        if (end16 == c.given16) return w;
+        w.phase = trhip::kListExpand;
+        w.first16 = c.given16; w.end16 = end16;
+        c.given16 = end16;
+        const uint64_t batches = (((uint64_t)c.maxBatches * (end16 - w.first16)) >> 16) + 1u;
+        blocks = (uint32_t)std::min<uint64_t>((batches + waves - 1u) / waves, (uint64_t)dev->computeUnits * 32u / waves);
+        if (blocks == 0) blocks = 1;
+    } else {
+        return w;
+    }
+    w.l = c.l;
+    *extraBlocks = blocks;
+    use(c.l.groups, ops.size(), false);
+    hold(c.visMask, false);
+    if (w.phase != trhip::kListCount) hold(c.drawArgs, true);
+    if (w.phase == trhip::kListExpand) hold(c.visibleList, true);
+    if (c.stage == 2 && c.given16 >= 65536u) listCarry.reset();
+    return w;
+}
+
+int trhip_cmdlist_t::flushListCarry()
+{
+    if (!listCarry) return TRHIP_OK;
+    const std::unique_ptr<ListCarry> c = std::move(listCarry);
+    use(c->l.groups, ops.size(), false);
+    hold(c->visMask, false);
+    hold(c->drawArgs, true);
+    hold(c->visibleList, true);
+    return c->flush(this, *c);
 }
 
 void trhip_cmdlist_t::hold(trhip_buffer_t* b, bool write, size_t op) { if (b) { use(b->ptr, op == SIZE_MAX ? ops.size() : op, write, &b->version); trhip_buffer_retain(b); heldBuffers.push_back(b); } }
@@ -634,6 +709,7 @@
     if (!cl->open) return fail(TRHIP_ERR_STATE, "cmd_close: not open");
     if (!cl->markers.empty()) return fail(TRHIP_ERR_STATE, "cmd_close: %zu marker(s) still open", cl->markers.size());
     if (cl->openStats) return fail(TRHIP_ERR_STATE, "cmd_close: a pipeline statistics query is still open");
+    if (int rc = cl->flushListCarry(); rc != TRHIP_OK) return rc;
     cl->open = false;
     std::stable_sort(cl->useMarks.begin(), cl->useMarks.end(), [](const trhip_cmdlist_t::UseMark& a, const trhip_cmdlist_t::UseMark& b) { return a.op < b.op; });
     return TRHIP_OK;
@@ -643,6 +719,12 @@
     do {                                                                                     \
         if (!(cl)) return fail(TRHIP_ERR_INVALID, "cmdlist is null");                        \
         if (!(cl)->open) return fail(TRHIP_ERR_STATE, "command list is not open");           \
+    } while (0)
+#define TRHIP_RECORDING_NO_HOST(cl)                                                          \
+    do {                                                                                     \
+        TRHIP_RECORDING(cl);                                                                 \
+        int flushed_ = (cl)->flushListCarry();                                               \
+        if (flushed_ != TRHIP_OK) return flushed_;                                           \
     } while (0)
 
 int trhip_cmd_write_buffer(trhip_cmdlist cl, trhip_buffer buf, uint64_t off, const void* src, uint64_t bytes)
@@ -655,6 +737,7 @@
         return TRHIP_OK;
     }
     if (!buf->ptr) return fail(TRHIP_ERR_STATE, "write_buffer(%s): no memory bound", buf->name.c_str());
+    if (int rc = cl->flushListCarry(); rc != TRHIP_OK) return rc;
     auto staged = std::make_shared<std::vector<uint8_t>>((const uint8_t*)src, (const uint8_t*)src + bytes);
     void* dst = (char*)buf->ptr + off;
     cl->hold(buf, true);
@@ -673,7 +756,11 @@
     if (buf->byteSize % 4) return fail(TRHIP_ERR_INVALID, "clear_buffer(%s): size not a multiple of 4", buf->name.c_str());
     if (cl->stillClearedTo(buf->ptr, value)) return TRHIP_OK;
     const bool hoist = !cl->usedSoFar(buf->ptr) && cl->firstClearBatch && cl->firstClearBatch->count < trhip_cmdlist_t::ClearBatch::kMax;
-    const bool merges = cl->openClearBatch && cl->openClearOp == cl->ops.size() - 1 && cl->openClearBatch->count < trhip_cmdlist_t::ClearBatch::kMax;
+    bool merges = cl->openClearBatch && cl->openClearOp == cl->ops.size() - 1 && cl->openClearBatch->count < trhip_cmdlist_t::ClearBatch::kMax;
+    if (!hoist && !merges && cl->listCarry) {
+        if (int rc = cl->flushListCarry(); rc != TRHIP_OK) return rc;
+        merges = false;
+    }
     cl->hold(buf, true, hoist ? cl->firstClearOp : merges ? cl->openClearOp : cl->ops.size());
     int rc = cl->recordClearWords(buf->ptr, buf->byteSize / 4, value, hoist);
     if (rc == TRHIP_OK) cl->clearedTo[buf->ptr] = { value, cl->useMarks.size() };
@@ -682,7 +769,7 @@
 
 int trhip_cmd_clear_texture_f32(trhip_cmdlist cl, trhip_texture tex, float value)
 {
-    TRHIP_RECORDING(cl);
+    TRHIP_RECORDING_NO_HOST(cl);
     if (!tex) return fail(TRHIP_ERR_INVALID, "clear_texture: null texture");
     if (!tex->ptr) return fail(TRHIP_ERR_STATE, "clear_texture(%s): no memory bound", tex->name.c_str());
     if (tex->format == TRHIP_FORMAT_RG32_UINT || tex->format == TRHIP_FORMAT_RGBA32_UINT || tex->format == TRHIP_FORMAT_R8_UINT)
@@ -717,7 +804,7 @@
 
 int trhip_cmd_clear_texture_u32(trhip_cmdlist cl, trhip_texture tex, uint32_t value)
 {
-    TRHIP_RECORDING(cl);
+    TRHIP_RECORDING_NO_HOST(cl);
     if (!tex) return fail(TRHIP_ERR_INVALID, "clear_texture: null texture");
     if (!tex->ptr) return fail(TRHIP_ERR_STATE, "clear_texture(%s): no memory bound", tex->name.c_str());
     if (tex->format == TRHIP_FORMAT_RGBA8_UNORM)
@@ -741,7 +828,7 @@
 
 int trhip_cmd_copy_buffer(trhip_cmdlist cl, trhip_buffer dst, uint64_t dstOff, trhip_buffer src, uint64_t srcOff, uint64_t bytes)
 {
-    TRHIP_RECORDING(cl);
+    TRHIP_RECORDING_NO_HOST(cl);
     if (!dst || !src) return fail(TRHIP_ERR_INVALID, "copy_buffer: null buffer");
     if (!dst->ptr || !src->ptr) return fail(TRHIP_ERR_STATE, "copy_buffer: a buffer has no memory bound");
     if (dstOff + bytes > dst->byteSize || srcOff + bytes > src->byteSize) return fail(TRHIP_ERR_INVALID, "copy_buffer(%s <- %s): range exceeds a buffer", dst->name.c_str(), src->name.c_str());
@@ -755,7 +842,7 @@
 
 int trhip_cmd_host_callback(trhip_cmdlist cl, trhip_host_fn fn, void* user)
 {
-    TRHIP_RECORDING(cl);
+    TRHIP_RECORDING_NO_HOST(cl);
     if (!fn) return fail(TRHIP_ERR_INVALID, "host_callback: null function");
     cl->ops.push_back({ "", [fn, user](hipStream_t s) { fn(user, (void*)s); return (int)TRHIP_OK; } });
     cl->ops.back().kind = "host_callback";
@@ -764,7 +851,7 @@
 
 int trhip_cmd_copy_texture(trhip_cmdlist cl, trhip_texture dst, trhip_texture src)
 {
-    TRHIP_RECORDING(cl);
+    TRHIP_RECORDING_NO_HOST(cl);
     if (!dst || !src) return fail(TRHIP_ERR_INVALID, "copy_texture: null texture");
     if (!dst->ptr || !src->ptr) return fail(TRHIP_ERR_STATE, "copy_texture: a texture has no memory bound");
     if (dst->width != src->width || dst->height != src->height || dst->mips != src->mips || dst->format != src->format)
@@ -813,6 +900,17 @@
         default: return fail(TRHIP_ERR_INVALID, "dispatch(%s): binding %u has unknown type %u", name, i, b[i].type);
         }
     }
+    if (cl->listCarry) {
+        static const char* const hosts[] = { "minmaxdownsample_CS_Main", "ffx_spd_downsample_pass_CS FFX_SPD_OPTION_DOWNSAMPLE_FILTER=1",
+                                             "ffx_spd_downsample_pass_CS FFX_SPD_OPTION_DOWNSAMPLE_FILTER=2", "gpuculling_CS_GPUCulling LATE_CULL=1",
+                                             "basepass_AS_Main LATE_CULL=1" };
+        bool host = false;
+        for (const char* h : hosts) host |= e->name == h;
+        if (!host) {
+            int frc = cl->flushListCarry();
+            if (frc != TRHIP_OK) return frc;
+        }
+    }
     DispatchCtx ctx{ cl, e->name.c_str(), e->variant, b, nb, push, pushBytes, indirect, args, argsOff, gx, gy, gz };
     int rc = e->fn(ctx);
     if (rc != TRHIP_OK || !cl->openStats) return rc;
@@ -836,7 +934,7 @@
 
 int trhip_cmd_begin_timer(trhip_cmdlist cl, trhip_timer t)
 {
-    TRHIP_RECORDING(cl);
+    TRHIP_RECORDING_NO_HOST(cl);
     if (!t) return fail(TRHIP_ERR_INVALID, "timer is null");
     cl->ops.push_back({ "", [t](hipStream_t s) { TRHIP_HIP(hipEventRecord(t->e0, s)); t->began = true; t->ended = false; return (int)TRHIP_OK; } });
     cl->ops.back().kind = "timer";
@@ -845,7 +943,7 @@
 
 int trhip_cmd_end_timer(trhip_cmdlist cl, trhip_timer t)
 {
-    TRHIP_RECORDING(cl);
+    TRHIP_RECORDING_NO_HOST(cl);
     if (!t) return fail(TRHIP_ERR_INVALID, "timer is null");
     cl->ops.push_back({ "", [t](hipStream_t s) { TRHIP_HIP(hipEventRecord(t->e1, s)); t->ended = true; return (int)TRHIP_OK; } });
     cl->ops.back().kind = "timer";
@@ -854,7 +952,7 @@
 
 int trhip_cmd_begin_pipeline_stats(trhip_cmdlist cl, trhip_pipeline_stats q)
 {
-    TRHIP_RECORDING(cl);
+    TRHIP_RECORDING_NO_HOST(cl);
     if (!q) return fail(TRHIP_ERR_INVALID, "pipeline statistics query is null");
     if (q->dev != cl->dev) return fail(TRHIP_ERR_INVALID, "begin_pipeline_stats: the query belongs to another device");
     if (cl->openStats) return fail(TRHIP_ERR_STATE, "begin_pipeline_stats: this command list already has a query open");
@@ -872,7 +970,7 @@
 
 int trhip_cmd_end_pipeline_stats(trhip_cmdlist cl, trhip_pipeline_stats q)
 {
-    TRHIP_RECORDING(cl);
+    TRHIP_RECORDING_NO_HOST(cl);
     if (!q) return fail(TRHIP_ERR_INVALID, "pipeline statistics query is null");
     if (cl->openStats != q) return fail(TRHIP_ERR_STATE, "end_pipeline_stats: the query is not open in this command list");
     const uint64_t hostCS = cl->statsHostCS;
diff --git a/toyrenderer_amd/csrc/trhip_internal.h b/toyrenderer_amd/csrc/trhip_internal.h
--- a/toyrenderer_amd/csrc/trhip_internal.h
+++ b/toyrenderer_amd/csrc/trhip_internal.h
@@ -20,6 +20,7 @@
 
 #include "../../include/trhip.h"
 #include "ShaderInterop.h"
+#include "list_build.hip.h"
 
 namespace trhip
 {
@@ -233,6 +234,22 @@
 
     struct Peephole { size_t op = SIZE_MAX; const char* kind = nullptr; std::shared_ptr<void> data; } peephole;
 
+    struct ListCarry
+    {
+        trhip::ListBuildArgs l;
+        uint32_t maxBatches = 0;
+        uint32_t stage = 0;
+        uint32_t given16 = 0;
+        uint32_t slice = 0;
+        std::string shader;
+        trhip_buffer_t *visMask = nullptr, *visibleList = nullptr, *drawArgs = nullptr;
+        int (*flush)(trhip_cmdlist_t* cl, const ListCarry& c) = nullptr;
+    };
+    std::unique_ptr<ListCarry> listCarry;
+    enum ListHost { kTileHost, kTailHost, kWideHost };
+    trhip::ListWork takeListWork(ListHost host, uint32_t waves, uint32_t* extraBlocks);
+    int flushListCarry();
+
     void* scratchAlloc(size_t bytes);
     void* scratchAllocSide(size_t bytes);
     std::vector<ScratchBlock> sideScratch;
@@ -301,6 +318,17 @@
             hipLaunchKernelGGL(kernel, grid, block, shmem, stream, __VA_ARGS__);                                    \
     } while (0)
 
+inline uint32_t inlineListMinGroups()
+{
+    static const uint32_t v = [] {
+        if (getenv("TRHIP_NO_INLINE_LIST")) return 0xFFFFFFFFu;
+        const char* e = getenv("TRHIP_INLINE_LIST_MIN_GROUPS");
+        return e ? (uint32_t)strtoul(e, nullptr, 0) : (1u << 19); }();
+    return v;
+}
+
+uint32_t listSliceEnd16(uint32_t slice);
+
 inline int launchStatus(const char* what)
 {
     hipError_t e = hipGetLastError();
```

Result: slower. 115.1 (-6.7%).
